# CityU-AIM-Group/SCAN

Hardware: AMD Instinct MI355X
Metric: train images/sec (whole node), VGG16 C2F 1024x2048 (higher is better)
Workload: dtype f32 (fp32 storage, fp32 multiply, fp32 accumulate -- the reference's arithmetic; the convolutions run it on the bf16 matrix cores as bf16x6: every fp32 operand cut into 3 bf16 pieces = all 24 significand bits, 6 bf16 MFMAs per product)

## Files before the change

### include/scan_hip.h

```cpp
#ifndef SCAN_HIP_H
#define SCAN_HIP_H

#include <stdint.h>

#ifdef __cplusplus
extern "C" {
#endif

#define SCAN_MAX_LEVELS 5

typedef struct {
  int32_t n_levels;
  int32_t n_images;
  int32_t h[SCAN_MAX_LEVELS];
  int32_t w[SCAN_MAX_LEVELS];
  int64_t row_off[SCAN_MAX_LEVELS + 1];
} scan_pyramid_t;

const char* scan_last_error(void);
int scan_abi_version(void);

#define SCAN_TUNE_UNKNOWN (-2147483647 - 1)
int scan_tune(const char* key, int value);
int scan_tune_get(const char* key);
int scan_tune_default(const char* key);
const char* scan_tune_key(int index);

int scan_mfma_sustained_bf16(double seconds, int32_t random, double* tflops, void* stream);

int scan_comm_standin(float* buf, int64_t n_floats, double traffic, int32_t wgs, double gbps, void* stream);

int scan_conv3x3_bf16x3_instance(const scan_pyramid_t* d, int32_t Nout);
int scan_conv1x1_bf16x6_instance(const scan_pyramid_t* yd, int32_t Nout, int32_t Csw);

int scan_sigmoid_focal_loss_forward(const float* logits, const int32_t* targets, int64_t M, int32_t C,
                                    float gamma, float alpha, float* losses, float* loss_sum, void* stream);
int scan_sigmoid_focal_loss_backward(const float* logits, const int32_t* targets, const float* d_losses,
                                     float d_scale, int64_t M, int32_t C, float gamma, float alpha,
                                     float* d_logits, void* stream);

int scan_iou_loss_forward(const float* pred, const float* target, const float* weight, int64_t P,
                          float* out2, void* stream);
int scan_iou_loss_backward(const float* pred, const float* target, const float* weight, int64_t P,
                           const float* g_num_dev, float* d_pred, void* stream);

int scan_bce_logits_forward(const float* logits, const float* targets, float const_target,
                            const float* weight, int64_t w_stride, int64_t M, float* out2, void* stream);
int scan_bce_logits_backward(const float* logits, const float* targets, float const_target,
                             const float* weight, int64_t w_stride, int64_t M, const float* g_dev,
                             float* d_logits, void* stream);

int scan_cka_bce_forward(const float* logits, const float* act, int64_t M, int32_t Cf, float target, float* out,
                         void* stream);
int scan_cka_bce_backward(const float* logits, const float* act, int64_t M, int32_t Cf, float target,
                          const float* g_dev, float* d_logits, void* stream);
int scan_cka_bce_forward_loss(const float* logits, const float* act, int64_t M, int32_t Cf, float target, float* out,
                              void* stream);
int scan_cka_bce_backward_loss(const float* logits, const float* act, int64_t M, int32_t Cf, float target,
                               const float* g_loss, const float* sums, float* d_logits, void* stream);

int scan_scale(const float* x, float alpha, float* y, int64_t n, void* stream);
int scan_copy_cols(const float* src, int32_t ld_src, float* dst, int32_t ld_dst, int64_t M, int32_t ncols, int32_t ztail,
                   void* stream);
int scan_paradigm_update(float* P, const float* pb, int32_t K, int32_t C, int32_t T, int32_t it, void* stream);

int scan_dynconv_softmax_forward(const float* feat, const float* kernels, int64_t M, int32_t C, int32_t K,
                                 float* logits, float* probs, void* stream);
int64_t scan_dynconv_ws_floats(int64_t M, int32_t C, int32_t K);
int scan_dynconv_softmax_backward(const float* feat, const float* kernels, const float* probs,
                                  const float* d_logits_in, const float* d_probs, int64_t M, int32_t C,
                                  int32_t K, float* d_feat, float* d_kernels, float* ws, void* stream);

int scan_softmax_focal_forward(const float* logits, const int64_t* labels, int64_t M, int32_t K, float gamma,
                               float* loss_sum, void* stream);
int scan_softmax_focal_backward(const float* logits, const int64_t* labels, int64_t M, int32_t K, float gamma,
                                float d_scale, float* d_logits, void* stream);

#define SCAN_NMS_PANEL 8192
#define SCAN_NMS_MAX 262144
int64_t scan_nms_ws_bytes(int64_t n);
int scan_nms(const float* dets, const float* scores, const float* labels, int64_t n, float thr, int32_t rule_ge,
             int64_t* keep_out, int32_t* num_keep_out, void* workspace, void* stream);

int scan_conv2d_forward(const float* x, const scan_pyramid_t* xd, int32_t Cin_s, const float* w, const float* bias,
                        float* y, const scan_pyramid_t* yd, int32_t Cout, int32_t Cout_s, int32_t ksize,
                        int32_t stride, int32_t relu, void* stream);
int scan_conv2d_dgrad(const float* dy, const scan_pyramid_t* yd, int32_t Cout_s, const float* wt, float* dx,
                      const scan_pyramid_t* xd, int32_t Cin, int32_t Cin_s, int32_t ksize, int32_t stride,
                      const float* mask, void* stream);
int64_t scan_conv2d_wgrad_ws_floats(const scan_pyramid_t* yd, int32_t Cin_s, int32_t Cout, int32_t ksize);
int scan_conv2d_wgrad(const float* x, const scan_pyramid_t* xd, int32_t Cin_s, const float* dy,
                      const scan_pyramid_t* yd, int32_t Cout, int32_t Cout_s, int32_t ksize, int32_t stride,
                      float* dw, int32_t accumulate, float* ws, void* stream);
int scan_weight_split(const float* w, int32_t O, int32_t T, int32_t Cs, int32_t mode, void* wh, void* wl,
                      int32_t Csw, void* stream);
int scan_conv3x3_bf16x3(const float* x, const scan_pyramid_t* d, int32_t Cs, const void* wh, const void* wl,
                        int32_t Csw, const float* bias, const float* mask, float* y, int32_t Nout, int32_t Ns,
                        int32_t relu, void* stream);
int scan_conv1x1_bf16x3(const float* x, const scan_pyramid_t* xd, int32_t Cs, const void* wh, const void* wl,
                        int32_t Csw, const float* bias, const float* mask, float* y, const scan_pyramid_t* yd,
                        int32_t Nout, int32_t Ns, int32_t relu, int32_t map, void* stream);
int64_t scan_conv1x1_wgrad_bf16x3_ws_floats(const scan_pyramid_t* yd, int32_t Cs, int32_t Cout);
int scan_conv1x1_wgrad_bf16x3(const float* x, const scan_pyramid_t* xd, int32_t Cs, const float* dy,
                              const scan_pyramid_t* yd, int32_t Cout, int32_t Cout_s, int32_t stride, float* dw,
                              float* db, int32_t accumulate, float* ws, void* stream);
int scan_conv_smallcin_bf16x3(const float* x, int32_t N, int32_t H, int32_t W, const float* w, const float* bias,
                              float* y, int32_t Cout, int32_t Cout_s, int32_t ksize, int32_t stride, int32_t relu,
                              void* stream);
int scan_conv3x3_gn_bf16x3(const float* x, const scan_pyramid_t* d, int32_t Cs, const void* wh, const void* wl,
                           int32_t Csw, const float* bias, float* y, int32_t Nout, int32_t Ns, float* gn_ws,
                           void* stream);
int scan_conv3x3_gn_acc_bf16x3(const float* x, const scan_pyramid_t* d, int32_t Cs, const void* wh, const void* wl,
                               int32_t Csw, const float* bias, float* y, int32_t Nout, int32_t Ns, float* gn_ws,
                               void* stream);
int scan_groupnorm_stats_from_sums(const float* ws, const scan_pyramid_t* d, int32_t C, int32_t G, float eps,
                                   float* stats, void* stream);
int scan_conv3x3_pool2_bf16x3(const float* x, const scan_pyramid_t* d, int32_t Cs, const void* wh, const void* wl,
                              int32_t Csw, const float* bias, float* y, int32_t Nout, int32_t Ns, int32_t relu,
                              void* stream);
int64_t scan_conv3x3_wgrad_bf16x3_ws_floats(const scan_pyramid_t* d, int32_t Cs, int32_t Cout);
int scan_conv3x3_wgrad_bf16x3(const float* x, const scan_pyramid_t* d, int32_t Cs, const float* dy, int32_t Cout,
                              int32_t Cout_s, float* dw, float* db, int32_t accumulate, float* ws, void* stream);
int scan_weight_split3(const float* w, int32_t O, int32_t T, int32_t Cs, int32_t mode, void* wh, void* wm, void* wl,
                       int32_t Csw, void* stream);
int scan_conv3x3_bf16x6(const float* x, const scan_pyramid_t* d, int32_t Cs, const void* wh, const void* wm,
                        const void* wl, int32_t Csw, const float* bias, const float* mask, float* y, int32_t Nout,
                        int32_t Ns, int32_t relu, void* stream);
int scan_conv1x1_bf16x6(const float* x, const scan_pyramid_t* xd, int32_t Cs, const void* wh, const void* wm,
                        const void* wl, int32_t Csw, const float* bias, const float* mask, float* y,
                        const scan_pyramid_t* yd, int32_t Nout, int32_t Ns, int32_t relu, int32_t map, void* stream);
int scan_conv3x3_gn_bf16x6(const float* x, const scan_pyramid_t* d, int32_t Cs, const void* wh, const void* wm,
                           const void* wl, int32_t Csw, const float* bias, float* y, int32_t Nout, int32_t Ns,
                           float* gn_ws, int32_t clear, void* stream);
int scan_conv3x3_pool2_bf16x6(const float* x, const scan_pyramid_t* d, int32_t Cs, const void* wh, const void* wm,
                              const void* wl, int32_t Csw, const float* bias, float* y, int32_t Nout, int32_t Ns,
                              int32_t relu, void* stream);
int scan_conv_smallcin_bf16x6(const float* x, int32_t N, int32_t H, int32_t W, const float* w, const float* bias,
                              float* y, int32_t Cout, int32_t Cout_s, int32_t ksize, int32_t stride, int32_t relu,
                              void* stream);
int64_t scan_conv3x3_wgrad_bf16x6_ws_floats(const scan_pyramid_t* d, int32_t Cs, int32_t Cout);
int scan_conv3x3_wgrad_bf16x6(const float* x, const scan_pyramid_t* d, int32_t Cs, const float* dy, int32_t Cout,
                              int32_t Cout_s, float* dw, float* db, int32_t accumulate, float* ws, void* stream);
int64_t scan_conv1x1_wgrad_bf16x6_ws_floats(const scan_pyramid_t* yd, int32_t Cs, int32_t Cout);
int scan_conv1x1_wgrad_bf16x6(const float* x, const scan_pyramid_t* xd, int32_t Cs, const float* dy,
                              const scan_pyramid_t* yd, int32_t Cout, int32_t Cout_s, int32_t stride, float* dw,
                              float* db, int32_t accumulate, float* ws, void* stream);
int scan_conv3x3_bf16x6_instance(const scan_pyramid_t* d, int32_t Nout);
int scan_weight_transpose(const float* w, int32_t Cout, int32_t T, int32_t Cin_s, float* wt, int32_t Cout_s,
                          void* stream);
int64_t scan_colsum_ws_floats(int64_t M, int32_t C);
int scan_colsum(const float* dy, int64_t M, int32_t C, int32_t ld, float* db, int32_t accumulate, float* ws,
                void* stream);
int scan_relu_backward(const float* dy, const float* y, float* out, int64_t n, void* stream);

int scan_groupnorm_stats(const float* x, const scan_pyramid_t* d, int32_t C, int32_t G, float eps, float* stats,
                         float* ws, void* stream);
int scan_groupnorm_relu_forward(const float* x, const scan_pyramid_t* d, int32_t C, int32_t G, const float* stats,
                                const float* gamma, const float* beta, int32_t relu, float* y, void* stream);
int scan_groupnorm_relu_forward_from_sums(const float* x, const scan_pyramid_t* d, int32_t C, int32_t G,
                                          const float* sums, float eps, const float* gamma, const float* beta,
                                          int32_t relu, float* y, float* stats, void* stream);
int64_t scan_groupnorm_ws_floats(const scan_pyramid_t* d, int32_t C, int32_t G);
int scan_groupnorm_relu_backward(const float* x, const float* beta, const float* dy, const scan_pyramid_t* d, int32_t C,
                                 int32_t G, const float* stats, const float* gamma, int32_t relu, float* dx,
                                 float* dgamma, float* dbeta, int32_t accumulate, float* ws, void* stream);
int scan_groupnorm_relu_forward_ld(const float* x, const scan_pyramid_t* d, int32_t C, int32_t G, const float* stats,
                                   const float* gamma, const float* beta, int32_t relu, float* y, int32_t ldy,
                                   void* stream);
int scan_groupnorm_relu_forward_from_sums_ld(const float* x, const scan_pyramid_t* d, int32_t C, int32_t G,
                                             const float* sums, float eps, const float* gamma, const float* beta,
                                             int32_t relu, float* y, int32_t ldy, float* stats, void* stream);
int scan_groupnorm_relu_backward_ld(const float* x, const float* beta, const float* dy, int32_t lddy,
                                    const scan_pyramid_t* d, int32_t C, int32_t G, const float* stats, const float* gamma,
                                    int32_t relu, float* dx, float* dgamma, float* dbeta, int32_t accumulate, float* ws,
                                    void* stream);

int scan_fcos_assign(const scan_pyramid_t* d, const int32_t* strides, const float* soi, const float* boxes,
                     const int64_t* glabels, const int32_t* ng, int32_t G, int64_t* labels, int32_t* labels_i32,
                     float* reg, int32_t* level_pos, void* stream);
int scan_fcos_compact(const scan_pyramid_t* d, const int64_t* labels, int32_t* pos_list, int32_t* neg_list, void* stream);
int64_t scan_fcos_nodes_count(const scan_pyramid_t* d, const int32_t* level_pos);
int scan_fcos_nodes(const scan_pyramid_t* d, const int32_t* level_pos, const int64_t* labels, const float* reg,
                    const int32_t* pos_list, const int32_t* neg_list, int64_t* node_index, int64_t* node_labels,
                    int64_t* pos_inds, float* reg_pos, float* ctr_pos, void* stream);

int scan_upsample2x_add(const float* lat, const float* coarse, int32_t N, int32_t h, int32_t w, int32_t C, float* y,
                        void* stream);
int scan_downsample2x_sum(const float* g, int32_t N, int32_t h, int32_t w, int32_t C, float* d, void* stream);

int scan_maxpool2x2_forward(const float* x, int32_t N, int32_t H, int32_t W, int32_t C, float* y, void* stream);
int scan_maxpool2x2_backward(const float* x, const float* y, const float* dy, int32_t N, int32_t H, int32_t W,
                             int32_t C, float* dx, int32_t relu_mask, void* stream);

int scan_maxpool3x3s2_forward(const float* x, int32_t N, int32_t H, int32_t W, int32_t C, float* y, void* stream);
int scan_add_relu(const float* a, const float* b, float* y, int64_t n, void* stream);

#define SCAN_DBSCAN_MAX 1200000
int64_t scan_dbscan_ws_bytes(int64_t n);
int scan_dbscan_prepare(const float* pts, int64_t n, int32_t D, float eps, int32_t min_samples, void* ws,
                        int32_t* info, void* stream);
int scan_dbscan_bfs_step(int64_t n, void* ws, int32_t parity, int32_t* changed, void* stream);
int scan_dbscan_finish(int64_t n, void* ws, uint8_t* in_cluster0, void* stream);

int scan_sgd_momentum(float* p, const float* g, float* buf, int64_t n, float lr, float wd, float momentum,
                      int32_t first_step, void* stream);

#define SCAN_SGD_MAX_SEGMENTS 32
typedef struct {
  float* p;
  const float* g;
  float* buf;
  int64_t n;
  float lr;
  float wd;
  int32_t first_step;
  int32_t reserved;
} scan_sgd_segment_t;
int scan_sgd_momentum_multi(const scan_sgd_segment_t* segs, int32_t n_segs, float momentum, void* stream);

#define SCAN_SPLIT_JOB_WORDS 11
int64_t scan_weight_split_job_blocks(int32_t O, int32_t T, int32_t Cs, int32_t mode, int32_t Csw);
int scan_weight_split_batched(const int64_t* jobs, int32_t n_jobs, int32_t job_words, int64_t total_blocks, void* stream);

#define SCAN_CKA_MAX_CLASSES 16
typedef struct {
  const float* w0;
  const float* b0;
  const float* w2;
  const float* b2;
} scan_cka_branch_t;
int scan_cka_stack_weights(const scan_cka_branch_t* branches, int32_t Cf, int32_t C, int32_t H, int64_t s1o, int64_t s1c,
                           int64_t s1k, int64_t s2c, int64_t s2k, int32_t Cs1, int32_t Cs2, float* w1, float* b1,
                           float* w2, float* b2, void* stream);
int scan_cka_unstack_grads(const scan_cka_branch_t* grads, int32_t Cf, int32_t C, int32_t H, int64_t s1o, int64_t s1c,
                           int64_t s1k, int64_t s2c, int64_t s2k, int32_t Cs1, int32_t Cs2, const float* dw1,
                           const float* db1, const float* dw2, const float* db2, int32_t accumulate, void* stream);

int64_t scan_gconv3x3_to1_ws_floats(const scan_pyramid_t* d, int32_t G, int32_t Cg);
int scan_gconv3x3_to1_forward(const float* x, const scan_pyramid_t* d, int32_t G, int32_t Cg, const float* w,
                              const float* bias, float* y, int32_t Ns, float* ws, void* stream);
int scan_gconv3x3_to1_dgrad(const float* dy, int32_t Ns, const scan_pyramid_t* d, int32_t G, int32_t Cg, const float* w,
                            const float* mask, float* dx, void* stream);
int scan_gconv3x3_to1_wgrad(const float* x, const float* dy, int32_t Ns, const scan_pyramid_t* d, int32_t G, int32_t Cg,
                            float* dw, int32_t accumulate, float* ws, void* stream);
int scan_gconv3x3_to1_backward(const float* x, const float* dy, int32_t Ns, const scan_pyramid_t* d, int32_t G, int32_t Cg,
                               const float* w, int32_t relu_mask, float* dx, float* dw, int32_t accumulate, float* ws,
                               void* stream);
int scan_gconv3x3_to1_forward_bits(const float* x, const scan_pyramid_t* d, int32_t G, int32_t Cg, const float* w,
                                   const float* bias, float* y, int32_t Ns, float* ws, uint32_t* relu_bits, void* stream);
int scan_gconv3x3_to1_backward_bits(const float* x, const float* dy, int32_t Ns, const scan_pyramid_t* d, int32_t G,
                                    int32_t Cg, const float* w, const uint32_t* relu_bits, float* dx, float* dw,
                                    int32_t accumulate, float* ws, void* stream);

int scan_resize_bilinear_u8(const uint8_t* src, int32_t H, int32_t W, uint8_t* tmp, uint8_t* dst, int32_t OH, int32_t OW,
                            const int32_t* xbounds, const int32_t* xcoef, int32_t kx, const int32_t* ybounds,
                            const int32_t* ycoef, int32_t ky, void* stream);

int scan_normalize_image_u8(const uint8_t* src, int32_t H, int32_t W, int32_t flip, int32_t to_bgr255,
                            const float* mean3, const float* std3, float* dst, int32_t Hp, int32_t Wp, int32_t layout,
                            void* stream);

int scan_take_images_backward(const float* g, const scan_pyramid_t* d, int32_t i0, int32_t i1, int32_t C, float* out,
                              void* stream);

int scan_cond_rnn_forward(const float* x, int32_t K, int32_t T, const float* const* weights, float* h0, float* h1,
                          float* kernels, void* stream);
int64_t scan_cond_rnn_ws_floats(void);
int scan_cond_rnn_backward(const float* x, int32_t K, int32_t T, const float* const* weights, const float* h0,
                           const float* h1, const float* dkernels, float* const* grads, float* ws, void* stream);

#ifdef __cplusplus
}
#endif
#endif
```

### scan_amd/_lib.py

```python
import ctypes
import os

_HERE = os.path.dirname(os.path.abspath(__file__))
LIB_PATH = os.environ.get("SCAN_HIP_LIB") or os.path.join(_HERE, "libscan_hip.so")

MAX_LEVELS = 5
TUNE_UNKNOWN = -2 ** 31
NMS_PANEL = 8192
NMS_MAX = 262144

c_i32, c_i64, c_f32, c_vp = ctypes.c_int32, ctypes.c_int64, ctypes.c_float, ctypes.c_void_p


class PyramidDesc(ctypes.Structure):
    _fields_ = [("n_levels", c_i32), ("n_images", c_i32), ("h", c_i32 * MAX_LEVELS), ("w", c_i32 * MAX_LEVELS),
                ("row_off", c_i64 * (MAX_LEVELS + 1))]


_PD = ctypes.POINTER(PyramidDesc)


class SgdSegment(ctypes.Structure):
    _fields_ = [("p", c_vp), ("g", c_vp), ("buf", c_vp), ("n", c_i64), ("lr", c_f32), ("wd", c_f32),
                ("first_step", c_i32), ("reserved", c_i32)]


class CkaBranch(ctypes.Structure):
    _fields_ = [("w0", c_vp), ("b0", c_vp), ("w2", c_vp), ("b2", c_vp)]


SGD_MAX_SEGMENTS = 32
CKA_MAX_CLASSES = 16
SPLIT_JOB_WORDS = 11

SIGNATURES = {
    "scan_last_error": (ctypes.c_char_p, []),
    "scan_abi_version": (ctypes.c_int, []),
    "scan_comm_standin": (ctypes.c_int, [ctypes.c_void_p, ctypes.c_int64, ctypes.c_double, ctypes.c_int32, ctypes.c_double,
                                         ctypes.c_void_p]),
    "scan_tune": (ctypes.c_int, [ctypes.c_char_p, ctypes.c_int]),
    "scan_take_images_backward": (ctypes.c_int, [c_vp, _PD, c_i32, c_i32, c_i32, c_vp, c_vp]),
    "scan_cond_rnn_forward": (ctypes.c_int, [c_vp, c_i32, c_i32, c_vp, c_vp, c_vp, c_vp, c_vp]),
    "scan_cond_rnn_ws_floats": (ctypes.c_int64, []),
    "scan_cond_rnn_backward": (ctypes.c_int, [c_vp, c_i32, c_i32, c_vp, c_vp, c_vp, c_vp, c_vp, c_vp, c_vp]),
    "scan_tune_get": (ctypes.c_int, [ctypes.c_char_p]),
    "scan_tune_default": (ctypes.c_int, [ctypes.c_char_p]),
    "scan_tune_key": (ctypes.c_char_p, [ctypes.c_int]),
    "scan_mfma_sustained_bf16": (ctypes.c_int, [ctypes.c_double, c_i32, ctypes.POINTER(ctypes.c_double), c_vp]),
    "scan_conv3x3_bf16x3_instance": (ctypes.c_int, [_PD, c_i32]),
    "scan_conv1x1_bf16x6_instance": (ctypes.c_int, [_PD, c_i32, c_i32]),
    "scan_conv3x3_bf16x6_instance": (ctypes.c_int, [_PD, c_i32]),
    "scan_sigmoid_focal_loss_forward": (ctypes.c_int, [c_vp, c_vp, c_i64, c_i32, c_f32, c_f32, c_vp, c_vp, c_vp]),
    "scan_sigmoid_focal_loss_backward": (ctypes.c_int, [c_vp, c_vp, c_vp, c_f32, c_i64, c_i32, c_f32, c_f32, c_vp, c_vp]),
    "scan_iou_loss_forward": (ctypes.c_int, [c_vp, c_vp, c_vp, c_i64, c_vp, c_vp]),
    "scan_iou_loss_backward": (ctypes.c_int, [c_vp, c_vp, c_vp, c_i64, c_vp, c_vp, c_vp]),
    "scan_bce_logits_forward": (ctypes.c_int, [c_vp, c_vp, c_f32, c_vp, c_i64, c_i64, c_vp, c_vp]),
    "scan_bce_logits_backward": (ctypes.c_int, [c_vp, c_vp, c_f32, c_vp, c_i64, c_i64, c_vp, c_vp, c_vp]),
    "scan_cka_bce_forward": (ctypes.c_int, [c_vp, c_vp, c_i64, c_i32, c_f32, c_vp, c_vp]),
    "scan_cka_bce_backward": (ctypes.c_int, [c_vp, c_vp, c_i64, c_i32, c_f32, c_vp, c_vp, c_vp]),
    "scan_cka_bce_forward_loss": (ctypes.c_int, [c_vp, c_vp, c_i64, c_i32, c_f32, c_vp, c_vp]),
    "scan_cka_bce_backward_loss": (ctypes.c_int, [c_vp, c_vp, c_i64, c_i32, c_f32, c_vp, c_vp, c_vp, c_vp]),
    "scan_scale": (ctypes.c_int, [c_vp, c_f32, c_vp, c_i64, c_vp]),
    "scan_copy_cols": (ctypes.c_int, [c_vp, c_i32, c_vp, c_i32, c_i64, c_i32, c_i32, c_vp]),
    "scan_paradigm_update": (ctypes.c_int, [c_vp, c_vp, c_i32, c_i32, c_i32, c_i32, c_vp]),
    "scan_dynconv_softmax_forward": (ctypes.c_int, [c_vp, c_vp, c_i64, c_i32, c_i32, c_vp, c_vp, c_vp]),
    "scan_dynconv_ws_floats": (c_i64, [c_i64, c_i32, c_i32]),
    "scan_dynconv_softmax_backward": (ctypes.c_int, [c_vp, c_vp, c_vp, c_vp, c_vp, c_i64, c_i32, c_i32, c_vp, c_vp, c_vp, c_vp]),
    "scan_softmax_focal_forward": (ctypes.c_int, [c_vp, c_vp, c_i64, c_i32, c_f32, c_vp, c_vp]),
    "scan_softmax_focal_backward": (ctypes.c_int, [c_vp, c_vp, c_i64, c_i32, c_f32, c_f32, c_vp, c_vp]),
    "scan_nms_ws_bytes": (c_i64, [c_i64]),
    "scan_nms": (ctypes.c_int, [c_vp, c_vp, c_vp, c_i64, c_f32, c_i32, c_vp, c_vp, c_vp, c_vp]),
    "scan_conv2d_forward": (ctypes.c_int, [c_vp, _PD, c_i32, c_vp, c_vp, c_vp, _PD, c_i32, c_i32, c_i32, c_i32, c_i32, c_vp]),
    "scan_conv2d_dgrad": (ctypes.c_int, [c_vp, _PD, c_i32, c_vp, c_vp, _PD, c_i32, c_i32, c_i32, c_i32, c_vp, c_vp]),
    "scan_conv2d_wgrad_ws_floats": (c_i64, [_PD, c_i32, c_i32, c_i32]),
    "scan_conv2d_wgrad": (ctypes.c_int, [c_vp, _PD, c_i32, c_vp, _PD, c_i32, c_i32, c_i32, c_i32, c_vp, c_i32, c_vp, c_vp]),
    "scan_weight_split": (ctypes.c_int, [c_vp, c_i32, c_i32, c_i32, c_i32, c_vp, c_vp, c_i32, c_vp]),
    "scan_conv3x3_bf16x3": (ctypes.c_int, [c_vp, _PD, c_i32, c_vp, c_vp, c_i32, c_vp, c_vp, c_vp, c_i32, c_i32, c_i32, c_vp]),
    "scan_conv3x3_wgrad_bf16x3_ws_floats": (c_i64, [_PD, c_i32, c_i32]),
    "scan_dbscan_ws_bytes": (c_i64, [c_i64]),
    "scan_conv1x1_wgrad_bf16x3_ws_floats": (c_i64, [_PD, c_i32, c_i32]),
    "scan_conv3x3_wgrad_bf16x3": (ctypes.c_int, [c_vp, _PD, c_i32, c_vp, c_i32, c_i32, c_vp, c_vp, c_i32, c_vp, c_vp]),
    "scan_weight_transpose": (ctypes.c_int, [c_vp, c_i32, c_i32, c_i32, c_vp, c_i32, c_vp]),
    "scan_colsum_ws_floats": (c_i64, [c_i64, c_i32]),
    "scan_colsum": (ctypes.c_int, [c_vp, c_i64, c_i32, c_i32, c_vp, c_i32, c_vp, c_vp]),
    "scan_relu_backward": (ctypes.c_int, [c_vp, c_vp, c_vp, c_i64, c_vp]),
    "scan_groupnorm_stats": (ctypes.c_int, [c_vp, _PD, c_i32, c_i32, c_f32, c_vp, c_vp, c_vp]),
    "scan_groupnorm_relu_forward": (ctypes.c_int, [c_vp, _PD, c_i32, c_i32, c_vp, c_vp, c_vp, c_i32, c_vp, c_vp]),
    "scan_groupnorm_relu_forward_from_sums": (ctypes.c_int, [c_vp, _PD, c_i32, c_i32, c_vp, c_f32, c_vp, c_vp, c_i32, c_vp, c_vp, c_vp]),
    "scan_groupnorm_ws_floats": (c_i64, [_PD, c_i32, c_i32]),
    "scan_fcos_assign": (ctypes.c_int, [_PD, c_vp, c_vp, c_vp, c_vp, c_vp, c_i32, c_vp, c_vp, c_vp, c_vp, c_vp]),
    "scan_fcos_compact": (ctypes.c_int, [_PD, c_vp, c_vp, c_vp, c_vp]),
    "scan_fcos_nodes_count": (c_i64, [_PD, c_vp]),
    "scan_fcos_nodes": (ctypes.c_int, [_PD, c_vp, c_vp, c_vp, c_vp, c_vp, c_vp, c_vp, c_vp, c_vp, c_vp, c_vp]),
    "scan_groupnorm_relu_forward_ld": (ctypes.c_int, [c_vp, _PD, c_i32, c_i32, c_vp, c_vp, c_vp, c_i32, c_vp, c_i32, c_vp]),
    "scan_groupnorm_relu_forward_from_sums_ld": (ctypes.c_int, [c_vp, _PD, c_i32, c_i32, c_vp, c_f32, c_vp, c_vp, c_i32, c_vp,
                                                                c_i32, c_vp, c_vp]),
    "scan_groupnorm_relu_backward_ld": (ctypes.c_int, [c_vp, c_vp, c_vp, c_i32, _PD, c_i32, c_i32, c_vp, c_vp, c_i32, c_vp,
                                                       c_vp, c_vp, c_i32, c_vp, c_vp]),
    "scan_groupnorm_relu_backward": (ctypes.c_int, [c_vp, c_vp, c_vp, _PD, c_i32, c_i32, c_vp, c_vp, c_i32, c_vp, c_vp, c_vp, c_i32, c_vp, c_vp]),
    "scan_maxpool2x2_forward": (ctypes.c_int, [c_vp, c_i32, c_i32, c_i32, c_i32, c_vp, c_vp]),
    "scan_maxpool2x2_backward": (ctypes.c_int, [c_vp, c_vp, c_vp, c_i32, c_i32, c_i32, c_i32, c_vp, c_i32, c_vp]),
    "scan_conv3x3_gn_bf16x3": (ctypes.c_int, [c_vp, _PD, c_i32, c_vp, c_vp, c_i32, c_vp, c_vp, c_i32, c_i32, c_vp, c_vp]),
    "scan_conv3x3_gn_acc_bf16x3": (ctypes.c_int, [c_vp, _PD, c_i32, c_vp, c_vp, c_i32, c_vp, c_vp, c_i32, c_i32, c_vp, c_vp]),
    "scan_groupnorm_stats_from_sums": (ctypes.c_int, [c_vp, _PD, c_i32, c_i32, c_f32, c_vp, c_vp]),
    "scan_conv3x3_pool2_bf16x3": (ctypes.c_int, [c_vp, _PD, c_i32, c_vp, c_vp, c_i32, c_vp, c_vp, c_i32, c_i32, c_i32, c_vp]),
    "scan_conv1x1_bf16x3": (ctypes.c_int, [c_vp, _PD, c_i32, c_vp, c_vp, c_i32, c_vp, c_vp, c_vp, _PD, c_i32, c_i32, c_i32,
                                           c_i32, c_vp]),
    "scan_conv1x1_wgrad_bf16x3": (ctypes.c_int, [c_vp, _PD, c_i32, c_vp, _PD, c_i32, c_i32, c_i32, c_vp, c_vp, c_i32, c_vp,
                                                 c_vp]),
    "scan_conv_smallcin_bf16x3": (ctypes.c_int, [c_vp, c_i32, c_i32, c_i32, c_vp, c_vp, c_vp, c_i32, c_i32, c_i32, c_i32,
                                                 c_i32, c_vp]),
    "scan_weight_split3": (ctypes.c_int, [c_vp, c_i32, c_i32, c_i32, c_i32, c_vp, c_vp, c_vp, c_i32, c_vp]),
    "scan_conv3x3_bf16x6": (ctypes.c_int, [c_vp, _PD, c_i32, c_vp, c_vp, c_vp, c_i32, c_vp, c_vp, c_vp, c_i32, c_i32, c_i32, c_vp]),
    "scan_conv1x1_bf16x6": (ctypes.c_int, [c_vp, _PD, c_i32, c_vp, c_vp, c_vp, c_i32, c_vp, c_vp, c_vp, _PD, c_i32, c_i32, c_i32,
                                           c_i32, c_vp]),
    "scan_conv3x3_gn_bf16x6": (ctypes.c_int, [c_vp, _PD, c_i32, c_vp, c_vp, c_vp, c_i32, c_vp, c_vp, c_i32, c_i32, c_vp, c_i32,
                                              c_vp]),
    "scan_conv3x3_pool2_bf16x6": (ctypes.c_int, [c_vp, _PD, c_i32, c_vp, c_vp, c_vp, c_i32, c_vp, c_vp, c_i32, c_i32, c_i32,
                                                 c_vp]),
    "scan_conv3x3_wgrad_bf16x6_ws_floats": (c_i64, [_PD, c_i32, c_i32]),
    "scan_conv3x3_wgrad_bf16x6": (ctypes.c_int, [c_vp, _PD, c_i32, c_vp, c_i32, c_i32, c_vp, c_vp, c_i32, c_vp, c_vp]),
    "scan_conv1x1_wgrad_bf16x6_ws_floats": (c_i64, [_PD, c_i32, c_i32]),
    "scan_conv1x1_wgrad_bf16x6": (ctypes.c_int, [c_vp, _PD, c_i32, c_vp, _PD, c_i32, c_i32, c_i32, c_vp, c_vp, c_i32, c_vp,
                                                 c_vp]),
    "scan_conv_smallcin_bf16x6": (ctypes.c_int, [c_vp, c_i32, c_i32, c_i32, c_vp, c_vp, c_vp, c_i32, c_i32, c_i32, c_i32,
                                                 c_i32, c_vp]),
    "scan_maxpool3x3s2_forward": (ctypes.c_int, [c_vp, c_i32, c_i32, c_i32, c_i32, c_vp, c_vp]),
    "scan_upsample2x_add": (ctypes.c_int, [c_vp, c_vp, c_i32, c_i32, c_i32, c_i32, c_vp, c_vp]),
    "scan_downsample2x_sum": (ctypes.c_int, [c_vp, c_i32, c_i32, c_i32, c_i32, c_vp, c_vp]),
    "scan_add_relu": (ctypes.c_int, [c_vp, c_vp, c_vp, c_i64, c_vp]),
    "scan_dbscan_prepare": (ctypes.c_int, [c_vp, c_i64, c_i32, c_f32, c_i32, c_vp, c_vp, c_vp]),
    "scan_dbscan_bfs_step": (ctypes.c_int, [c_i64, c_vp, c_i32, c_vp, c_vp]),
    "scan_dbscan_finish": (ctypes.c_int, [c_i64, c_vp, c_vp, c_vp]),
    "scan_sgd_momentum": (ctypes.c_int, [c_vp, c_vp, c_vp, c_i64, c_f32, c_f32, c_f32, c_i32, c_vp]),
    "scan_sgd_momentum_multi": (ctypes.c_int, [ctypes.POINTER(SgdSegment), c_i32, c_f32, c_vp]),
    "scan_weight_split_job_blocks": (c_i64, [c_i32, c_i32, c_i32, c_i32, c_i32]),
    "scan_weight_split_batched": (ctypes.c_int, [c_vp, c_i32, c_i32, c_i64, c_vp]),
    "scan_cka_stack_weights": (ctypes.c_int, [ctypes.POINTER(CkaBranch), c_i32, c_i32, c_i32, c_i64, c_i64, c_i64, c_i64,
                                              c_i64, c_i32, c_i32, c_vp, c_vp, c_vp, c_vp, c_vp]),
    "scan_cka_unstack_grads": (ctypes.c_int, [ctypes.POINTER(CkaBranch), c_i32, c_i32, c_i32, c_i64, c_i64, c_i64, c_i64,
                                              c_i64, c_i32, c_i32, c_vp, c_vp, c_vp, c_vp, c_i32, c_vp]),
    "scan_gconv3x3_to1_ws_floats": (c_i64, [_PD, c_i32, c_i32]),
    "scan_gconv3x3_to1_forward": (ctypes.c_int, [c_vp, _PD, c_i32, c_i32, c_vp, c_vp, c_vp, c_i32, c_vp, c_vp]),
    "scan_gconv3x3_to1_dgrad": (ctypes.c_int, [c_vp, c_i32, _PD, c_i32, c_i32, c_vp, c_vp, c_vp, c_vp]),
    "scan_gconv3x3_to1_wgrad": (ctypes.c_int, [c_vp, c_vp, c_i32, _PD, c_i32, c_i32, c_vp, c_i32, c_vp, c_vp]),
    "scan_gconv3x3_to1_backward": (ctypes.c_int, [c_vp, c_vp, c_i32, _PD, c_i32, c_i32, c_vp, c_i32, c_vp, c_vp, c_i32, c_vp,
                                                  c_vp]),
    "scan_gconv3x3_to1_forward_bits": (ctypes.c_int, [c_vp, _PD, c_i32, c_i32, c_vp, c_vp, c_vp, c_i32, c_vp, c_vp, c_vp]),
    "scan_gconv3x3_to1_backward_bits": (ctypes.c_int, [c_vp, c_vp, c_i32, _PD, c_i32, c_i32, c_vp, c_vp, c_vp, c_vp, c_i32,
                                                       c_vp, c_vp]),
    "scan_resize_bilinear_u8": (ctypes.c_int, [c_vp, c_i32, c_i32, c_vp, c_vp, c_i32, c_i32, c_vp, c_vp, c_i32, c_vp, c_vp,
                                               c_i32, c_vp]),
    "scan_normalize_image_u8": (ctypes.c_int, [c_vp, c_i32, c_i32, c_i32, c_i32, ctypes.POINTER(c_f32),
                                               ctypes.POINTER(c_f32), c_vp, c_i32, c_i32, c_i32, c_vp]),
}

_lib = None


def lib():
    global _lib
    if _lib is None:
        if not os.path.exists(LIB_PATH):
            raise RuntimeError(
                "scan_amd: %s is missing -- build it with `python -c 'import __graft_entry__ as g; g.build()'` "
                "(hipcc --offload-arch=gfx950); there is no CPU fallback." % LIB_PATH)
        import torch
        L = ctypes.CDLL(LIB_PATH)
        for name, (res, args) in SIGNATURES.items():
            fn = getattr(L, name)
            fn.restype = res
            fn.argtypes = args
        for kv in filter(None, os.environ.get("SCAN_TUNE", "").split(",")):
            key, _, val = kv.partition("=")
            if L.scan_tune(key.strip().encode(), int(val)) == TUNE_UNKNOWN:
                raise RuntimeError("SCAN_TUNE: unknown key %r" % key)
        _lib = L
    return _lib


def tune_state():
    L, out, i = lib(), {}, 0
    while True:
        k = L.scan_tune_key(i)
        if k is None:
            return out
        out[k.decode()] = (L.scan_tune_get(k), L.scan_tune_default(k))
        i += 1


def lib_identity():
    import hashlib
    with open(LIB_PATH, "rb") as f:
        sha = hashlib.sha1(f.read()).hexdigest()
    product = os.path.realpath(LIB_PATH) == os.path.realpath(os.path.join(_HERE, "libscan_hip.so"))
    return {"lib": os.path.basename(LIB_PATH), "lib_sha1": sha, "product_library": product,
            "scan_tune_non_default": {k: v for k, (v, d) in tune_state().items() if v != d}}


def call(name, *args):
    rc = getattr(lib(), name)(*args)
    if rc != 0:
        raise RuntimeError("%s failed (%d): %s" % (name, rc, lib().scan_last_error().decode()))

# ... 4 lines not shown
```

### scan_amd/csrc/batched.hip

```cpp
#include "conv_split.h"

#define SPLIT_ELEMS_PER_BLOCK 2048
#define SPLIT_TILE 64

__device__ __forceinline__ void split8_store(const float (&v)[8], __bf16* __restrict__ w0, __bf16* __restrict__ w1,
                                             __bf16* __restrict__ w2, int64_t i) {
  bf16x8 q0, q1, q2;
#pragma unroll
  for (int k = 0; k < 8; ++k) {
    __bf16 q[3];
    split1_np<3>(v[k], q);
    q0[k] = q[0];
    q1[k] = q[1];
    q2[k] = q[2];
  }
  *reinterpret_cast<bf16x8*>(w0 + i) = q0;
  *reinterpret_cast<bf16x8*>(w1 + i) = q1;
  if (w2 != nullptr) *reinterpret_cast<bf16x8*>(w2 + i) = q2;
}

__global__ __launch_bounds__(256) void weight_split_batched_kernel(const int64_t* __restrict__ jobs, int n_jobs) {
  __shared__ float tile[SPLIT_TILE][SPLIT_TILE + 1];
  int j = 0;
  for (int i = 1; i < n_jobs; ++i)
    if ((int64_t)blockIdx.x >= jobs[(int64_t)i * SCAN_SPLIT_JOB_WORDS + 9]) j = i;
  const int64_t* job = jobs + (int64_t)j * SCAN_SPLIT_JOB_WORDS;
  const float* __restrict__ w = reinterpret_cast<const float*>(job[0]);
  __bf16* __restrict__ wh = reinterpret_cast<__bf16*>(job[1]);
  __bf16* __restrict__ wl = reinterpret_cast<__bf16*>(job[2]);
  __bf16* __restrict__ w2 = reinterpret_cast<__bf16*>(job[10]);
  const int O = (int)job[3], T = (int)job[4], Cs = (int)job[5], mode = (int)job[6], rows = (int)job[7],
            Csw = (int)job[8];
  const int64_t blk = (int64_t)blockIdx.x - job[9];
  const int tid = threadIdx.x;
  if (mode == 0) {
    const int64_t total = (int64_t)rows * T * Csw;
    const int64_t i = blk * SPLIT_ELEMS_PER_BLOCK + (int64_t)tid * 8;
    if (i >= total) return;
    const int col = (int)(i % Csw);
    const int64_t rt = i / Csw;
    const float* src = w + rt * Cs + col;
    float v[8];
    if (col + 8 <= Cs && (Cs & 3) == 0) {
      const float4 a = *reinterpret_cast<const float4*>(src);
      const float4 b = *reinterpret_cast<const float4*>(src + 4);
      v[0] = a.x; v[1] = a.y; v[2] = a.z; v[3] = a.w;
      v[4] = b.x; v[5] = b.y; v[6] = b.z; v[7] = b.w;
    } else {
#pragma unroll
      for (int k = 0; k < 8; ++k) v[k] = (col + k < Cs) ? src[k] : 0.f;
    }
    split8_store(v, wh, wl, w2, i);
    return;
  }
  const int tiles_o = (Csw + SPLIT_TILE - 1) / SPLIT_TILE, tiles_c = (rows + SPLIT_TILE - 1) / SPLIT_TILE;
  const int to = (int)(blk % tiles_o);
  const int tc = (int)((blk / tiles_o) % tiles_c);
  const int tt = (int)(blk / ((int64_t)tiles_o * tiles_c));
  const int o0 = to * SPLIT_TILE, c0 = tc * SPLIT_TILE;
  {
    const int cl = (tid & 15) * 4, ol = tid >> 4;
#pragma unroll
    for (int p = 0; p < SPLIT_TILE / 16; ++p) {
      const int o = o0 + ol + 16 * p, c = c0 + cl;
      float4 a = make_float4(0.f, 0.f, 0.f, 0.f);
      if (o < O && c < Cs) {
        const float* src = w + ((int64_t)o * T + (T - 1 - tt)) * Cs + c;
        if (c + 4 <= Cs && (Cs & 3) == 0) {
          a = *reinterpret_cast<const float4*>(src);
        } else {
          a.x = src[0];
          if (c + 1 < Cs) a.y = src[1];
          if (c + 2 < Cs) a.z = src[2];
          if (c + 3 < Cs) a.w = src[3];
        }
      }
      float* t = &tile[ol + 16 * p][cl];
      t[0] = a.x; t[1] = a.y; t[2] = a.z; t[3] = a.w;
    }
  }
  __syncthreads();
  {
    const int o8 = (tid & 7) * 8, cl = tid >> 3;
#pragma unroll
    for (int p = 0; p < SPLIT_TILE / 32; ++p) {
      const int c = c0 + cl + 32 * p, o = o0 + o8;
      if (c < rows && o < Csw) {
        float v[8];
#pragma unroll
        for (int k = 0; k < 8; ++k) v[k] = tile[o8 + k][cl + 32 * p];
        split8_store(v, wh, wl, w2, ((int64_t)c * T + tt) * Csw + o);
      }
    }
  }
}

extern "C" int64_t scan_weight_split_job_blocks(int32_t O, int32_t T, int32_t Cs, int32_t mode, int32_t Csw) {
  if (mode == 0) return ((int64_t)O * T * Csw + SPLIT_ELEMS_PER_BLOCK - 1) / SPLIT_ELEMS_PER_BLOCK;
  const int64_t tiles_o = (Csw + SPLIT_TILE - 1) / SPLIT_TILE, tiles_c = (Cs + SPLIT_TILE - 1) / SPLIT_TILE;
  return tiles_o * tiles_c * T;
}

extern "C" int scan_weight_split_batched(const int64_t* jobs, int32_t n_jobs, int32_t job_words, int64_t total_blocks,
                                         void* stream) {
  SCAN_CHECK_ARG(job_words == SCAN_SPLIT_JOB_WORDS, "weight_split_batched: records of %d words, this library reads %d",
                 job_words, SCAN_SPLIT_JOB_WORDS);
  SCAN_CHECK_ARG(jobs && n_jobs > 0 && total_blocks > 0 && total_blocks < (1ll << 31),
                 "weight_split_batched: bad arguments (n_jobs=%d)", n_jobs);
  hipLaunchKernelGGL(weight_split_batched_kernel, dim3((unsigned)total_blocks), dim3(256), 0, as_stream(stream), jobs,
                     n_jobs);
  SCAN_LAUNCH_CHECK("weight_split_batched");
  return 0;
}

struct SgdSegs {
  scan_sgd_segment_t s[SCAN_SGD_MAX_SEGMENTS];
  int64_t first_block[SCAN_SGD_MAX_SEGMENTS + 1];
  int n;
};
#define SGD_ELEMS_PER_BLOCK 4096

__global__ __launch_bounds__(256) void sgd_multi_kernel(SgdSegs t, float momentum) {
  int j = 0;
#pragma unroll
  for (int i = 1; i < SCAN_SGD_MAX_SEGMENTS; ++i)
    if (i < t.n && (int64_t)blockIdx.x >= t.first_block[i]) j = i;
  const scan_sgd_segment_t sg = t.s[j];
  const int64_t base = ((int64_t)blockIdx.x - t.first_block[j]) * SGD_ELEMS_PER_BLOCK;
  float* __restrict__ p = sg.p;
  const float* __restrict__ g = sg.g;
  float* __restrict__ buf = sg.buf;
#pragma unroll 4
  for (int k = 0; k < SGD_ELEMS_PER_BLOCK / 256; ++k) {
    const int64_t i = base + k * 256 + threadIdx.x;
    if (i >= sg.n) break;
    const float w = p[i];
    const float gg = g[i] + sg.wd * w;
    const float b = sg.first_step ? gg : momentum * buf[i] + gg;
    buf[i] = b;
    p[i] = w - sg.lr * b;
  }
}

extern "C" int scan_sgd_momentum_multi(const scan_sgd_segment_t* segs, int32_t n_segs, float momentum, void* stream) {
  SCAN_CHECK_ARG(segs && n_segs > 0 && n_segs <= SCAN_SGD_MAX_SEGMENTS, "sgd_momentum_multi: n_segs=%d out of 1..%d", n_segs,
                 SCAN_SGD_MAX_SEGMENTS);
  SgdSegs t;
  t.n = 0;
  int64_t blocks = 0;
  for (int i = 0; i < n_segs; ++i) {
    SCAN_CHECK_ARG(segs[i].n >= 0, "sgd_momentum_multi: segment %d has n < 0", i);
    if (segs[i].n == 0) continue;
    SCAN_CHECK_ARG(segs[i].p && segs[i].g && segs[i].buf, "sgd_momentum_multi: null pointer in segment %d", i);
    t.s[t.n] = segs[i];
    t.first_block[t.n] = blocks;
    blocks += (segs[i].n + SGD_ELEMS_PER_BLOCK - 1) / SGD_ELEMS_PER_BLOCK;
    ++t.n;
  }
  if (t.n == 0) return 0;
  t.first_block[t.n] = blocks;
  SCAN_CHECK_ARG(blocks < (1ll << 31), "sgd_momentum_multi: too many elements");
  hipLaunchKernelGGL(sgd_multi_kernel, dim3((unsigned)blocks), dim3(256), 0, as_stream(stream), t, momentum);
  SCAN_LAUNCH_CHECK("sgd_momentum_multi");
  return 0;
}

struct CkaPtrs {
  scan_cka_branch_t b[SCAN_CKA_MAX_CLASSES];
};

__global__ __launch_bounds__(256) void cka_stack_kernel(CkaPtrs P, int Cf, int C, int H, int64_t s1o, int64_t s1c,
                                                        int64_t s1k, int64_t s2c, int64_t s2k, int Cs1, int Cs2,
                                                        float* __restrict__ w1, float* __restrict__ b1,
                                                        float* __restrict__ w2, float* __restrict__ b2) {
  const int64_t n1 = (int64_t)Cf * H * 9 * Cs1;
  const int64_t n2 = (int64_t)Cf * 9 * Cs2;
  const int64_t nb = (int64_t)Cf * H + Cf;
  for (int64_t i = (int64_t)blockIdx.x * blockDim.x + threadIdx.x; i < n1 + n2 + nb;
       i += (int64_t)gridDim.x * blockDim.x) {
    if (i < n1) {
      const int col = (int)(i % Cs1);
      const int64_t r = i / Cs1;
      const int k = (int)(r % 9);
      const int row = (int)(r / 9);
      const int c = row / H, o = row - c * H;
      float v = 0.f;
      if (col < C) v = P.b[c].w0[o * s1o + col * s1c + k * s1k];
      else if (col == C + c) v = P.b[c].w0[o * s1o + C * s1c + k * s1k];
      w1[i] = v;
    } else if (i < n1 + n2) {
      const int64_t q = i - n1;
      const int col = (int)(q % Cs2);
      const int64_t r = q / Cs2;
      const int k = (int)(r % 9);
      const int c = (int)(r / 9);
      float v = 0.f;
      if (col >= c * H && col < (c + 1) * H) v = P.b[c].w2[(col - c * H) * s2c + k * s2k];
      w2[q] = v;
    } else {
      const int q = (int)(i - n1 - n2);
      if (q < Cf * H) b1[q] = P.b[q / H].b0[q % H];
      else b2[q - Cf * H] = P.b[q - Cf * H].b2[0];
    }
  }
}

__global__ __launch_bounds__(256) void cka_unstack_kernel(CkaPtrs G, int Cf, int C, int H, int64_t s1o, int64_t s1c,
                                                          int64_t s1k, int64_t s2c, int64_t s2k, int Cs1, int Cs2,
                                                          const float* __restrict__ dw1, const float* __restrict__ db1,
                                                          const float* __restrict__ dw2, const float* __restrict__ db2,
                                                          int accumulate) {
  const int64_t n1 = (int64_t)Cf * H * 9 * (C + 1);
  const int64_t n2 = (int64_t)Cf * 9 * H;
  const int64_t nb = (int64_t)Cf * H + Cf;
  for (int64_t i = (int64_t)blockIdx.x * blockDim.x + threadIdx.x; i < n1 + n2 + nb;
       i += (int64_t)gridDim.x * blockDim.x) {
    if (i < n1) {
      const int col = (int)(i % (C + 1));
      const int64_t r = i / (C + 1);
      const int k = (int)(r % 9);
      const int row = (int)(r / 9);
      const int c = row / H, o = row - c * H;
      if (dw1 != nullptr) {
        const float v = dw1[((int64_t)row * 9 + k) * Cs1 + (col < C ? col : C + c)];
        float* dst = const_cast<float*>(G.b[c].w0) + o * s1o + col * s1c + k * s1k;
        *dst = accumulate ? *dst + v : v;
      }
    } else if (i < n1 + n2) {
      const int64_t q = i - n1;
      const int h = (int)(q % H);
      const int64_t r = q / H;
      const int k = (int)(r % 9);
      const int c = (int)(r / 9);
      if (dw2 != nullptr) {
        const float v = dw2[((int64_t)c * 9 + k) * Cs2 + c * H + h];
        float* dst = const_cast<float*>(G.b[c].w2) + h * s2c + k * s2k;
        *dst = accumulate ? *dst + v : v;
      }
    } else {
      const int q = (int)(i - n1 - n2);
      if (q < Cf * H) {
        if (db1 != nullptr) {
          float* dst = const_cast<float*>(G.b[q / H].b0) + q % H;
          *dst = accumulate ? *dst + db1[q] : db1[q];
        }
      } else if (db2 != nullptr) {
        float* dst = const_cast<float*>(G.b[q - Cf * H].b2);
        *dst = accumulate ? *dst + db2[q - Cf * H] : db2[q - Cf * H];
      }
    }
  }
}

// ... 36 lines not shown
```

### scan_amd/csrc/capi.cpp

```cpp
#include <stdarg.h>
#include <stdio.h>
#include <string.h>

#include "../../include/scan_hip.h"

static thread_local char g_err[512] = "";

extern "C" void scan_set_error(const char* fmt, ...) {
  va_list ap;
  va_start(ap, fmt);
  vsnprintf(g_err, sizeof(g_err), fmt, ap);
  va_end(ap);
}

extern "C" const char* scan_last_error(void) { return g_err; }
extern "C" int scan_abi_version(void) { return 1; }

extern int g_scan_conv_bn256;
extern int g_scan_conv_v2;
extern int g_scan_conv_wg1024;
extern int g_scan_conv_w8;
extern int g_scan_conv_tpb3;
extern int g_scan_conv_bn64_th16;
extern int g_scan_conv_glds;
extern int g_scan_conv1x1;
extern int g_scan_wgrad_v6;
extern int g_scan_wgrad_prio;
extern int g_scan_wgrad_tile;
extern int g_scan_wgrad_wgs;
extern int g_scan_gconv_mfma;
extern int g_scan_dbscan_bf16x3;
extern int g_scan_reduce_blocks;

struct Knob {
  const char* key;
  int* slot;
  int dflt;
};
static Knob* knob_table(int* count) {
  static Knob knobs[] = {
      {"conv_bn256", &g_scan_conv_bn256, 0},   {"conv_v2", &g_scan_conv_v2, 0},         {"conv_wg1024", &g_scan_conv_wg1024, 0},
      {"conv_w8", &g_scan_conv_w8, 0},         {"conv_tpb3", &g_scan_conv_tpb3, 0},     {"conv_bn64_th16", &g_scan_conv_bn64_th16, 0},
      {"conv_glds", &g_scan_conv_glds, 0},     {"wgrad_v6", &g_scan_wgrad_v6, 0},       {"wgrad_prio", &g_scan_wgrad_prio, 0},
      {"wgrad_tile", &g_scan_wgrad_tile, 0},   {"wgrad_wgs", &g_scan_wgrad_wgs, 0},     {"gconv_mfma", &g_scan_gconv_mfma, 0},
      {"dbscan_bf16x3", &g_scan_dbscan_bf16x3, 0}, {"reduce_blocks", &g_scan_reduce_blocks, 0}, {"conv1x1", &g_scan_conv1x1, 0},
  };
  static bool init = false;
  if (!init) {
    for (auto& k : knobs) k.dflt = *k.slot;
    init = true;
  }
  *count = (int)(sizeof(knobs) / sizeof(knobs[0]));
  return knobs;
}
static Knob* find_knob(const char* key) {
  int n = 0;
  Knob* t = knob_table(&n);
  if (key == nullptr) return nullptr;
  for (int i = 0; i < n; ++i)
    if (strcmp(key, t[i].key) == 0) return &t[i];
  return nullptr;
}

extern "C" int scan_tune(const char* key, int value) {
  Knob* k = find_knob(key);
  if (k == nullptr) return SCAN_TUNE_UNKNOWN;
  const int old = *k->slot;
  *k->slot = value;
  return old;
}

extern "C" int scan_tune_get(const char* key) {
  const Knob* k = find_knob(key);
  return k == nullptr ? SCAN_TUNE_UNKNOWN : *k->slot;
}

extern "C" int scan_tune_default(const char* key) {
  const Knob* k = find_knob(key);
  return k == nullptr ? SCAN_TUNE_UNKNOWN : k->dflt;
}

extern "C" const char* scan_tune_key(int index) {
  int n = 0;
  const Knob* t = knob_table(&n);
  return (index >= 0 && index < n) ? t[index].key : nullptr;
}
```

### scan_amd/csrc/conv_bf16x3.hip

```cpp
#include "conv_split.h"

typedef float f32x16 __attribute__((ext_vector_type(16)));

#define SCAN_MMA(a, b, c) __builtin_amdgcn_mfma_f32_32x32x16_bf16(a, b, c, 0, 0, 0)

#define TW 16
#define PW (TW + 2)
#define CK 32
#define LROW 40
#define PPITCH 768

struct TileTab {
  int tile_off[SCAN_MAX_LEVELS + 1];
  int tiles_x[SCAN_MAX_LEVELS];
  int tiles_y[SCAN_MAX_LEVELS];
};

__device__ __forceinline__ int xcd_remap3(int orig, int nwg) {
  const int q = nwg / 8, r = nwg % 8, xcd = orig % 8;
  const int base = (xcd < r) ? xcd * (q + 1) : r * (q + 1) + (xcd - r) * q;
  return base + orig / 8;
}

__device__ __forceinline__ void split4(const float4 v, bf16x4& hi, bf16x4& lo) {
// ... 121 lines not shown
#pragma unroll
  for (int tm = 0; tm < TM; ++tm) {
    const int p = (wm * TM + tm) * 32 + lr;
    a_off[tm] = (p >> 4) * PPITCH + (p & 15) * LROW + 8 * lh;
  }
  const int b_off = (wn * 32 * TN + lr) * LROW + 8 * lh;

  f32x16 acc[TM][TN];
#pragma unroll
  for (int a = 0; a < TM; ++a)
#pragma unroll
    for (int b = 0; b < TN; ++b)
#pragma unroll
      for (int r = 0; r < 16; ++r) acc[a][b][r] = 0.f;

  load_a(0);
  load_b(0, 0);
  for (int cc = 0; cc < nchunks; ++cc) {
    __syncthreads();
    store_a();
    if (cc + 1 < nchunks) load_a(cc + 1);
#pragma unroll 1
    for (int tap = 0; tap < NTAPS; ++tap) {
      const int buf = (cc * NTAPS + tap) & 1;
      store_b(buf);
      if (tap < NTAPS - 1)
        load_b(cc, tap + 1);
      else if (cc + 1 < nchunks)
        load_b(cc + 1, 0);
      __syncthreads();
      const int ky = tap / KS, kx = tap - KS * ky;
      const int shift = ky * PPITCH + kx * LROW;
      const __bf16* bh = Bs + (buf * 2 + 0) * BN * LROW + b_off;
      const __bf16* bl = Bs + (buf * 2 + 1) * BN * LROW + b_off;
      if constexpr (TN > 2) {
#pragma unroll
        for (int s = 0; s < 2; ++s) {
          bf16x8 ah[TM], al[TM];
#pragma unroll
          for (int tm = 0; tm < TM; ++tm) {
            ah[tm] = *reinterpret_cast<const bf16x8*>(Ah + a_off[tm] + shift + 16 * s);
            al[tm] = *reinterpret_cast<const bf16x8*>(Al + a_off[tm] + shift + 16 * s);
          }
#pragma unroll
          for (int tn = 0; tn < TN; ++tn) {
            const bf16x8 bhv = *reinterpret_cast<const bf16x8*>(bh + tn * 32 * LROW + 16 * s);
            const bf16x8 blv = *reinterpret_cast<const bf16x8*>(bl + tn * 32 * LROW + 16 * s);
#pragma unroll
            for (int tm = 0; tm < TM; ++tm) {
              acc[tm][tn] = SCAN_MMA(al[tm], bhv, acc[tm][tn]);
              acc[tm][tn] = SCAN_MMA(ah[tm], blv, acc[tm][tn]);
              acc[tm][tn] = SCAN_MMA(ah[tm], bhv, acc[tm][tn]);
            }
          }
        }
        continue;
      }
#pragma unroll
      for (int s = 0; s < 2; ++s) {
        bf16x8 ah[TM], al[TM], bhv[TN], blv[TN];
#pragma unroll
        for (int tm = 0; tm < TM; ++tm) {
          ah[tm] = *reinterpret_cast<const bf16x8*>(Ah + a_off[tm] + shift + 16 * s);
          al[tm] = *reinterpret_cast<const bf16x8*>(Al + a_off[tm] + shift + 16 * s);
        }
#pragma unroll
        for (int tn = 0; tn < TN; ++tn) {
          bhv[tn] = *reinterpret_cast<const bf16x8*>(bh + tn * 32 * LROW + 16 * s);
          blv[tn] = *reinterpret_cast<const bf16x8*>(bl + tn * 32 * LROW + 16 * s);
        }
#pragma unroll
        for (int tm = 0; tm < TM; ++tm)
#pragma unroll
          for (int tn = 0; tn < TN; ++tn) {
            acc[tm][tn] = SCAN_MMA(al[tm], bhv[tn], acc[tm][tn]);
            acc[tm][tn] = SCAN_MMA(ah[tm], blv[tn], acc[tm][tn]);
            acc[tm][tn] = SCAN_MMA(ah[tm], bhv[tn], acc[tm][tn]);
          }
      }
    }
  }

#pragma unroll
  for (int tn = 0; tn < TN; ++tn) {
    const int o = n0 + wn * 32 * TN + tn * 32 + lr;
    const float bv = (bias != nullptr && o < Nout) ? bias[o] : 0.f;
    float gs = 0.f, gq = 0.f;
    if (relu & 2) {
      const int Hp = H >> 1, Wp = W >> 1;
#pragma unroll
      for (int tm = 0; tm < TM; ++tm)
#pragma unroll
        for (int q = 0; q < 4; ++q) {
          const int r = 2 * q;
          const int p = (wm * TM + tm) * 32 + (r & 3) + 8 * (r >> 2) + 4 * lh;
          const int y = ty0 + (p >> 4), x = tx0 + (p & 15);
          if (y < H && x < W && o < Nout) {
            float v = fmaxf(fmaxf(acc[tm][tn][r], acc[tm][tn][r + 1]), fmaxf(acc[tm][tn][r + 8], acc[tm][tn][r + 9])) + bv;
            if (relu & 1) v = fmaxf(v, 0.f);
            dst[((int64_t)img * Hp * Wp + (int64_t)(y >> 1) * Wp + (x >> 1)) * Ns + o] = v;
          }
        }
      continue;
    }
#pragma unroll
    for (int tm = 0; tm < TM; ++tm) {
      float mk[16];
      if (mask != nullptr) {
#pragma unroll
        for (int r = 0; r < 16; ++r) {
          const int p = (wm * TM + tm) * 32 + (r & 3) + 8 * (r >> 2) + 4 * lh;
          const int y = ty0 + (p >> 4), x = tx0 + (p & 15);
          const bool ok = y < H && x < W && o < Nout;
          mk[r] = ok ? mask[(rowbase + (int64_t)y * W + x) * Ns + o] : 0.f;
        }
      }
#pragma unroll
      for (int r = 0; r < 16; ++r) {
        const int p = (wm * TM + tm) * 32 + (r & 3) + 8 * (r >> 2) + 4 * lh;
        const int y = ty0 + (p >> 4), x = tx0 + (p & 15);
        if (y < H && x < W && o < Nout) {
          const int64_t m = rowbase + (int64_t)y * W + x;
          float v = acc[tm][tn][r] + bv;
          if (relu & 1) v = fmaxf(v, 0.f);
          if (mask != nullptr) v = (mk[r] > 0.f) ? v : 0.f;
          dst[m * Ns + o] = v;
          gs += v;
          gq += v * v;
        }
      }
    }
    if (gn_ws != nullptr) {
      double ds = (double)gs, dq = (double)gq;
#pragma unroll
      for (int sh = 1; sh <= 4; sh <<= 1) {
        ds += __shfl_xor(ds, sh, 64);
        dq += __shfl_xor(dq, sh, 64);
      }
      ds += __shfl_xor(ds, 32, 64);
      dq += __shfl_xor(dq, 32, 64);
      if ((lr & 7) == 0 && lh == 0 && o < Nout) {
        const int64_t slot = ((int64_t)(lvl * d.n_images + img) * 32 + (o >> 3)) * 2;
        atomicAdd(&gn_ws[slot], ds);
        atomicAdd(&gn_ws[slot + 1], dq);
      }
    }
  }
}


template <int NP>
__global__ void weight_split_kernel(const float* __restrict__ w, int O, int T, int Cs, int mode, int rows, int Csw,
                                    __bf16* __restrict__ w0, __bf16* __restrict__ w1, __bf16* __restrict__ w2) {
  const int64_t total = (int64_t)rows * T * Csw;
  for (int64_t i = (int64_t)blockIdx.x * blockDim.x + threadIdx.x; i < total; i += (int64_t)gridDim.x * blockDim.x) {
    const int col = (int)(i % Csw);
    const int64_t rt = i / Csw;
    const int tt = (int)(rt % T);
    const int row = (int)(rt / T);
    float v = 0.f;
    if (mode == 0) {
      if (col < Cs) v = w[((int64_t)row * T + tt) * Cs + col];
    } else {
      if (col < O) v = w[((int64_t)col * T + (T - 1 - tt)) * Cs + row];
    }
    __bf16 q[NP];
    split1_np<NP>(v, q);
    w0[i] = q[0];
    w1[i] = q[1];
    if constexpr (NP == 3) w2[i] = q[2];
  }
}

int g_scan_conv_v2 = 1;
extern int g_scan_conv_bn256;
int conv3x3_split_launch(int np, const float* x, const scan_pyramid_t* d, int32_t Cs, const void* w0, const void* w1,
                         const void* w2, int32_t Csw, const float* bias, const float* mask, float* y, int32_t Nout,
                         int32_t Ns, int32_t relu, void* stream, double* gn_ws);
int conv1x1_split_launch(int np, const float* x, const scan_pyramid_t* xd, int32_t Cs, const void* w0, const void* w1,
                         const void* w2, int32_t Csw, const float* bias, const float* mask, float* y,
                         const scan_pyramid_t* yd, int32_t Nout, int32_t Ns, int32_t relu, int32_t map, void* stream);
static inline bool v2_ok(const void* y, const void* mask, int32_t Ns) {
  return (Ns & 3) == 0 && (reinterpret_cast<uintptr_t>(y) & 15) == 0 && (reinterpret_cast<uintptr_t>(mask) & 15) == 0;
}

static void make_tiles(const scan_pyramid_t* d, TileTab* tt, int TH) {
  tt->tile_off[0] = 0;
  for (int l = 0; l < SCAN_MAX_LEVELS; ++l) {
    if (l < d->n_levels) {
      tt->tiles_x[l] = (d->w[l] + TW - 1) / TW;
      tt->tiles_y[l] = (d->h[l] + TH - 1) / TH;
      tt->tile_off[l + 1] = tt->tile_off[l] + d->n_images * tt->tiles_x[l] * tt->tiles_y[l];
    } else {
      tt->tiles_x[l] = tt->tiles_y[l] = 1;
      tt->tile_off[l + 1] = tt->tile_off[l];
    }
  }
}

static int weight_split_launch(int np, const float* w, int32_t O, int32_t T, int32_t Cs, int32_t mode, void* w0, void* w1,
                               void* w2, int32_t Csw, void* stream) {
  SCAN_CHECK_ARG(w && w0 && w1 && (np == 2 || w2) && O > 0 && T > 0 && Cs > 0, "weight_split: bad arguments");
  SCAN_CHECK_ARG(mode == 0 || mode == 1, "weight_split: mode must be 0 or 1");
  SCAN_CHECK_ARG(Csw % 8 == 0 && Csw >= (mode == 0 ? Cs : O), "weight_split: Csw=%d must be a multiple of 8 and cover the row",
                 Csw);
  const int rows = mode == 0 ? O : Cs;
  const int64_t total = (int64_t)rows * T * Csw;
  __bf16 *p0 = reinterpret_cast<__bf16*>(w0), *p1 = reinterpret_cast<__bf16*>(w1), *p2 = reinterpret_cast<__bf16*>(w2);
  if (np == 3)
    hipLaunchKernelGGL(weight_split_kernel<3>, dim3(grid_for(total, 256)), dim3(256), 0, as_stream(stream), w, O, T, Cs, mode,
                       rows, Csw, p0, p1, p2);
  else
    hipLaunchKernelGGL(weight_split_kernel<2>, dim3(grid_for(total, 256)), dim3(256), 0, as_stream(stream), w, O, T, Cs, mode,
                       rows, Csw, p0, p1, p2);
  SCAN_LAUNCH_CHECK("weight_split");
  return 0;
}

extern "C" int scan_weight_split(const float* w, int32_t O, int32_t T, int32_t Cs, int32_t mode, void* wh, void* wl,
                                 int32_t Csw, void* stream) {
  return weight_split_launch(2, w, O, T, Cs, mode, wh, wl, nullptr, Csw, stream);
}
extern "C" int scan_weight_split3(const float* w, int32_t O, int32_t T, int32_t Cs, int32_t mode, void* wh, void* wm,
                                  void* wl, int32_t Csw, void* stream) {
  return weight_split_launch(3, w, O, T, Cs, mode, wh, wm, wl, Csw, stream);
}

static int conv3x3_launch(int np, const float* x, const scan_pyramid_t* d, int32_t Cs, const void* w0, const void* w1,
                          const void* w2, int32_t Csw, const float* bias, const float* mask, float* y, int32_t Nout,
                          int32_t Ns, int32_t relu, void* stream, double* gn_ws = nullptr) {
  const char* name = np == 2 ? "conv3x3_bf16x3" : "conv3x3_bf16x6";
  SCAN_CHECK_ARG(d && d->n_levels >= 1 && d->n_levels <= SCAN_MAX_LEVELS && d->n_images >= 1, "%s: bad pyramid", name);
  SCAN_CHECK_ARG(Cs > 0 && Cs % 4 == 0, "%s: Cs=%d must be a positive multiple of 4", name, Cs);
  SCAN_CHECK_ARG(Csw % 8 == 0 && Csw >= Cs, "%s: Csw=%d must be a multiple of 8 and >= Cs", name, Csw);
  SCAN_CHECK_ARG(Nout > 0 && Ns >= Nout, "%s: Nout=%d Ns=%d", name, Nout, Ns);
  SCAN_CHECK_ARG(x && w0 && w1 && (np == 2 || w2) && y, "%s: null pointer", name);
  if (np == 3) {
    SCAN_CHECK_ARG(v2_ok(y, mask, Ns), "%s: y / mask must be 16-byte aligned and Ns a multiple of 4", name);
    return conv3x3_split_launch(3, x, d, Cs, w0, w1, w2, Csw, bias, mask, y, Nout, Ns, relu, stream, gn_ws);
  }
  if (g_scan_conv_v2 && v2_ok(y, mask, Ns))
    return conv3x3_split_launch(2, x, d, Cs, w0, w1, nullptr, Csw, bias, mask, y, Nout, Ns, relu, stream, gn_ws);
  TileTab tt;
  hipStream_t st = as_stream(stream);
  const __bf16* h = reinterpret_cast<const __bf16*>(w0);
  const __bf16* l = reinterpret_cast<const __bf16*>(w1);
  if (Nout > 64) {
    make_tiles(d, &tt, 16);
    const int tiles = tt.tile_off[d->n_levels];
    const bool wide = g_scan_conv_bn256 && Nout % 256 == 0 && (int64_t)tiles * (Nout / 256) >= 512;
    if (wide) {
      const int n_tiles = Nout / 256;
      const size_t sh = (size_t)(2 * 18 * PPITCH + 4 * 256 * LROW) * sizeof(__bf16);
      static bool done = false;
      if (!done) {
        hipFuncSetAttribute(reinterpret_cast<const void*>(conv3x3_bf16x3_kernel<256, 16, 512>),
                            hipFuncAttributeMaxDynamicSharedMemorySize, (int)sh);
        done = true;
      }
      hipLaunchKernelGGL((conv3x3_bf16x3_kernel<256, 16, 512>), dim3(tiles * n_tiles), dim3(512), sh, st, x, *d, Cs, h, l,
                         Csw, bias, mask, y, Nout, Ns, relu, tt, n_tiles, *d, 0, gn_ws);
      SCAN_LAUNCH_CHECK("conv3x3_bf16x3");
      return 0;
    }
    const int n_tiles = (Nout + 127) / 128;
    const size_t sh = (size_t)(2 * 18 * PPITCH + 4 * 128 * LROW) * sizeof(__bf16);
    static bool done = false;
    if (!done) {
      hipFuncSetAttribute(reinterpret_cast<const void*>(conv3x3_bf16x3_kernel<128, 16, 512>),
                          hipFuncAttributeMaxDynamicSharedMemorySize, (int)sh);
      done = true;
    }
    hipLaunchKernelGGL((conv3x3_bf16x3_kernel<128, 16, 512>), dim3(tiles * n_tiles), dim3(512), sh, st, x, *d, Cs, h, l,
                       Csw, bias, mask, y, Nout, Ns, relu, tt, n_tiles, *d, 0, gn_ws);
  } else {
    make_tiles(d, &tt, 8);
    const int tiles = tt.tile_off[d->n_levels];
    const size_t sh = (size_t)(2 * 10 * PPITCH + 4 * 64 * LROW) * sizeof(__bf16);
    hipLaunchKernelGGL((conv3x3_bf16x3_kernel<64, 8, 256>), dim3(tiles), dim3(256), sh, st, x, *d, Cs, h, l, Csw, bias,
                       mask, y, Nout, Ns, relu, tt, 1, *d, 0, gn_ws);
  }
  SCAN_LAUNCH_CHECK("conv3x3_bf16x3");
  return 0;
}

extern "C" int scan_conv3x3_bf16x3(const float* x, const scan_pyramid_t* d, int32_t Cs, const void* wh, const void* wl,
                                   int32_t Csw, const float* bias, const float* mask, float* y, int32_t Nout,
                                   int32_t Ns, int32_t relu, void* stream) {
  return conv3x3_launch(2, x, d, Cs, wh, wl, nullptr, Csw, bias, mask, y, Nout, Ns, relu ? 1 : 0, stream);
}
extern "C" int scan_conv3x3_bf16x6(const float* x, const scan_pyramid_t* d, int32_t Cs, const void* wh, const void* wm,
                                   const void* wl, int32_t Csw, const float* bias, const float* mask, float* y,
                                   int32_t Nout, int32_t Ns, int32_t relu, void* stream) {
  return conv3x3_launch(3, x, d, Cs, wh, wm, wl, Csw, bias, mask, y, Nout, Ns, relu ? 1 : 0, stream);
}

static int conv3x3_gn_launch(int np, int clear, const float* x, const scan_pyramid_t* d, int32_t Cs, const void* w0,
                             const void* w1, const void* w2, int32_t Csw, const float* bias, float* y, int32_t Nout,
                             int32_t Ns, float* gn_ws, void* stream) {
  SCAN_CHECK_ARG(Nout == 256 && gn_ws, "conv3x3_gn: needs Nout == 256 (GroupNorm(32, 256)) and a workspace");
  SCAN_CHECK_ARG(d && d->n_levels >= 1 && d->n_levels <= SCAN_MAX_LEVELS && d->n_images >= 1, "conv3x3_gn: bad pyramid");
  if (clear) {
    const size_t bytes = sizeof(double) * 2 * 32 * (size_t)d->n_levels * d->n_images;
    if (hipMemsetAsync(gn_ws, 0, bytes, as_stream(stream)) != hipSuccess) {
      scan_set_error("conv3x3_gn: memset failed");
      return -2;
    }
  }
  return conv3x3_launch(np, x, d, Cs, w0, w1, w2, Csw, bias, nullptr, y, Nout, Ns, 0, stream, reinterpret_cast<double*>(gn_ws));
}
extern "C" int scan_conv3x3_gn_bf16x3(const float* x, const scan_pyramid_t* d, int32_t Cs, const void* wh, const void* wl,
                                      int32_t Csw, const float* bias, float* y, int32_t Nout, int32_t Ns, float* gn_ws,
                                      void* stream) {
  return conv3x3_gn_launch(2, 1, x, d, Cs, wh, wl, nullptr, Csw, bias, y, Nout, Ns, gn_ws, stream);
}
extern "C" int scan_conv3x3_gn_acc_bf16x3(const float* x, const scan_pyramid_t* d, int32_t Cs, const void* wh, const void* wl,
                                          int32_t Csw, const float* bias, float* y, int32_t Nout, int32_t Ns, float* gn_ws,
                                          void* stream) {
  return conv3x3_gn_launch(2, 0, x, d, Cs, wh, wl, nullptr, Csw, bias, y, Nout, Ns, gn_ws, stream);
}
extern "C" int scan_conv3x3_gn_bf16x6(const float* x, const scan_pyramid_t* d, int32_t Cs, const void* wh, const void* wm,
                                      const void* wl, int32_t Csw, const float* bias, float* y, int32_t Nout, int32_t Ns,
                                      float* gn_ws, int32_t clear, void* stream) {
  return conv3x3_gn_launch(3, clear, x, d, Cs, wh, wm, wl, Csw, bias, y, Nout, Ns, gn_ws, stream);
}

extern "C" int scan_conv3x3_pool2_bf16x3(const float* x, const scan_pyramid_t* d, int32_t Cs, const void* wh,
                                         const void* wl, int32_t Csw, const float* bias, float* y, int32_t Nout,
                                         int32_t Ns, int32_t relu, void* stream) {
  SCAN_CHECK_ARG(d && d->n_levels == 1 && (d->h[0] & 1) == 0 && (d->w[0] & 1) == 0,
                 "conv3x3_pool2_bf16x3: needs a single-level pyramid with even H and W");
  return conv3x3_launch(2, x, d, Cs, wh, wl, nullptr, Csw, bias, nullptr, y, Nout, Ns, (relu ? 1 : 0) | 2, stream);
}
extern "C" int scan_conv3x3_pool2_bf16x6(const float* x, const scan_pyramid_t* d, int32_t Cs, const void* wh,
                                         const void* wm, const void* wl, int32_t Csw, const float* bias, float* y,
                                         int32_t Nout, int32_t Ns, int32_t relu, void* stream) {
  SCAN_CHECK_ARG(d && d->n_levels == 1 && (d->h[0] & 1) == 0 && (d->w[0] & 1) == 0,
                 "conv3x3_pool2_bf16x6: needs a single-level pyramid with even H and W");
  return conv3x3_launch(3, x, d, Cs, wh, wm, wl, Csw, bias, nullptr, y, Nout, Ns, (relu ? 1 : 0) | 2, stream);
}

static int conv1x1_launch(int np, const float* x, const scan_pyramid_t* xd, int32_t Cs, const void* w0, const void* w1,
                          const void* w2, int32_t Csw, const float* bias, const float* mask, float* y,
                          const scan_pyramid_t* yd, int32_t Nout, int32_t Ns, int32_t relu, int32_t map, void* stream) {
  const char* name = np == 2 ? "conv1x1_bf16x3" : "conv1x1_bf16x6";
  SCAN_CHECK_ARG(xd && yd && yd->n_levels >= 1 && yd->n_levels <= SCAN_MAX_LEVELS && yd->n_images >= 1 &&
                     xd->n_levels == yd->n_levels && xd->n_images == yd->n_images,
                 "%s: bad pyramids", name);
  SCAN_CHECK_ARG(map >= 0 && map <= 2, "%s: map=%d must be 0, 1 or 2", name, map);
  SCAN_CHECK_ARG(Cs > 0 && Cs % 4 == 0, "%s: Cs=%d must be a positive multiple of 4", name, Cs);
  SCAN_CHECK_ARG(Csw % 8 == 0 && Csw >= Cs, "%s: Csw=%d must be a multiple of 8 and >= Cs", name, Csw);
  SCAN_CHECK_ARG(Nout > 0 && Ns >= Nout, "%s: Nout=%d Ns=%d", name, Nout, Ns);
  SCAN_CHECK_ARG(x && w0 && w1 && (np == 2 || w2) && y, "%s: null pointer", name);
  for (int l = 0; l < yd->n_levels; ++l) {
    const int eh = map == 0 ? xd->h[l] : map == 1 ? (xd->h[l] - 1) / 2 + 1 : yd->h[l];
    const int ew = map == 0 ? xd->w[l] : map == 1 ? (xd->w[l] - 1) / 2 + 1 : yd->w[l];
    SCAN_CHECK_ARG(eh == yd->h[l] && ew == yd->w[l] &&
                       (map != 2 || ((yd->h[l] - 1) / 2 + 1 == xd->h[l] && (yd->w[l] - 1) / 2 + 1 == xd->w[l])),
                   "%s: level %d sizes do not match map %d", name, l, map);
  }
  if (np == 3) {
    SCAN_CHECK_ARG(v2_ok(y, mask, Ns), "%s: y / mask must be 16-byte aligned and Ns a multiple of 4", name);
    return conv1x1_split_launch(3, x, xd, Cs, w0, w1, w2, Csw, bias, mask, y, yd, Nout, Ns, relu, map, stream);
  }
  if (g_scan_conv_v2 && v2_ok(y, mask, Ns))
    return conv1x1_split_launch(2, x, xd, Cs, w0, w1, nullptr, Csw, bias, mask, y, yd, Nout, Ns, relu, map, stream);
  TileTab tt;
  hipStream_t st = as_stream(stream);
  const __bf16* h = reinterpret_cast<const __bf16*>(w0);
  const __bf16* l = reinterpret_cast<const __bf16*>(w1);
  if (Nout > 64) {
    make_tiles(yd, &tt, 16);
    const int tiles = tt.tile_off[yd->n_levels];
    const int n_tiles = (Nout + 127) / 128;
    const size_t sh = (size_t)(2 * 16 * PPITCH + 4 * 128 * LROW) * sizeof(__bf16);
    static bool done = false;
    if (!done) {
      hipFuncSetAttribute(reinterpret_cast<const void*>(conv3x3_bf16x3_kernel<128, 16, 512, 1>),
                          hipFuncAttributeMaxDynamicSharedMemorySize, (int)sh);
      done = true;
    }
    hipLaunchKernelGGL((conv3x3_bf16x3_kernel<128, 16, 512, 1>), dim3(tiles * n_tiles), dim3(512), sh, st, x, *yd, Cs, h,
                       l, Csw, bias, mask, y, Nout, Ns, relu, tt, n_tiles, *xd, map, nullptr);
  } else {
    make_tiles(yd, &tt, 8);
    const int tiles = tt.tile_off[yd->n_levels];
    const size_t sh = (size_t)(2 * 8 * PPITCH + 4 * 64 * LROW) * sizeof(__bf16);
    hipLaunchKernelGGL((conv3x3_bf16x3_kernel<64, 8, 256, 1>), dim3(tiles), dim3(256), sh, st, x, *yd, Cs, h, l, Csw,
                       bias, mask, y, Nout, Ns, relu, tt, 1, *xd, map, nullptr);
  }
  SCAN_LAUNCH_CHECK("conv1x1_bf16x3");
  return 0;
}

extern "C" int scan_conv1x1_bf16x3(const float* x, const scan_pyramid_t* xd, int32_t Cs, const void* wh, const void* wl,
                                   int32_t Csw, const float* bias, const float* mask, float* y,
                                   const scan_pyramid_t* yd, int32_t Nout, int32_t Ns, int32_t relu, int32_t map,
                                   void* stream) {
  return conv1x1_launch(2, x, xd, Cs, wh, wl, nullptr, Csw, bias, mask, y, yd, Nout, Ns, relu, map, stream);
}
extern "C" int scan_conv1x1_bf16x6(const float* x, const scan_pyramid_t* xd, int32_t Cs, const void* wh, const void* wm,
                                   const void* wl, int32_t Csw, const float* bias, const float* mask, float* y,
                                   const scan_pyramid_t* yd, int32_t Nout, int32_t Ns, int32_t relu, int32_t map,
                                   void* stream) {
  return conv1x1_launch(3, x, xd, Cs, wh, wm, wl, Csw, bias, mask, y, yd, Nout, Ns, relu, map, stream);
}
```

### scan_amd/csrc/conv_fwd.hip

```cpp
#include "conv_split.h"

#define V2_TW 16
#ifndef SCAN_CONV_MID
#define SCAN_CONV_MID 0
#endif
#ifndef SCAN_CONV_PFA
#define SCAN_CONV_PFA 1
#endif
#define V2_CK 32

struct TileTab2 {
  int tile_off[SCAN_MAX_LEVELS + 1];
  int tiles_x[SCAN_MAX_LEVELS];
  int tiles_y[SCAN_MAX_LEVELS];
};

__device__ __forceinline__ int swz(int idx) { return (idx >> 1) & 2; }

template <int K>
__device__ __forceinline__ const __bf16* pick_plane(const __bf16* w0, const __bf16* w1, const __bf16* w2) {
  if constexpr (K == 0)
    return w0;
  else if constexpr (K == 1)
    return w1;
  else
    return w2;
}
template <int I, int NT, int PL, int NPL>
__device__ __forceinline__ const __bf16* slot_plane(int tid, const __bf16* w0, const __bf16* w1, const __bf16* w2) {
  constexpr int lo = (NT * I) / PL, hi = (NT * I + NT - 1) / PL;
  constexpr int lo_c = lo < NPL ? lo : NPL - 1, hi_c = hi < NPL ? hi : NPL - 1;
  static_assert(hi - lo <= 1, "a thread's slot spans at most two planes");
  if constexpr (lo_c == hi_c)
    return pick_plane<lo_c>(w0, w1, w2);
  else
    return (tid + NT * I) / PL == lo ? pick_plane<lo_c>(w0, w1, w2) : pick_plane<hi_c>(w0, w1, w2);
}
template <int NT, int PL, int NPL>
__device__ __forceinline__ const __bf16* slot_plane_i(int i, int tid, const __bf16* w0, const __bf16* w1, const __bf16* w2) {
  return i == 0   ? slot_plane<0, NT, PL, NPL>(tid, w0, w1, w2)
         : i == 1 ? slot_plane<1, NT, PL, NPL>(tid, w0, w1, w2)
         : i == 2 ? slot_plane<2, NT, PL, NPL>(tid, w0, w1, w2)
         : i == 3 ? slot_plane<3, NT, PL, NPL>(tid, w0, w1, w2)
         : i == 4 ? slot_plane<4, NT, PL, NPL>(tid, w0, w1, w2)
                  : slot_plane<5, NT, PL, NPL>(tid, w0, w1, w2);
}

template <int NP, int TM>
__device__ __forceinline__ void mma_pieces(const bf16x8 (&w)[NP], const bf16x8 (&p)[NP][TM], f32x4v (&acc)[TM]) {
#pragma unroll
  for (int s = NP - 1; s >= 0; --s)
#pragma unroll
    for (int i = 0; i <= s; ++i)
#pragma unroll
      for (int tm = 0; tm < TM; ++tm) acc[tm] = __builtin_amdgcn_mfma_f32_16x16x32_bf16(w[i], p[s - i][tm], acc[tm], 0, 0, 0);
}

template <int NP, int BN, int TH, int NT, int KS, int TPB = 1, bool GL = false>
__global__ __launch_bounds__(NT, NT == 1024 ? 4 : 2) void conv_split_kernel(
    const float* __restrict__ src, scan_pyramid_t d, int Cs, const __bf16* __restrict__ w0, const __bf16* __restrict__ w1,
    const __bf16* __restrict__ w2, int Csw, const float* __restrict__ bias, const float* __restrict__ mask,
    float* __restrict__ dst, int Nout, int Ns, int relu, TileTab2 tt, int n_tiles, scan_pyramid_t sd, int map,
    double* __restrict__ gn_ws) {
  constexpr int HALO = KS / 2, NTAPS = KS * KS;
  constexpr int PH = TH + 2 * HALO;
  constexpr int PWK = V2_TW + 2 * HALO;
  constexpr int NPATCH = PH * PWK;
  constexpr int WAVES = NT / 64;
  constexpr int WN_WAVES = BN >= 128 ? 2 : 1;
  constexpr int WM_WAVES = WAVES / WN_WAVES;
  constexpr int TM = TH / WM_WAVES;
  constexpr int TN = BN / (16 * WN_WAVES);
  constexpr int ASLOTS = (NPATCH * 8 + NT - 1) / NT;
  constexpr int BSLOTS = BN * 4 * NP;
  constexpr int BSEG = (BSLOTS + NT - 1) / NT;
  constexpr int NGRP = NTAPS / TPB;
  static_assert(NP == 2 || NP == 3, "two or three pieces per operand");
  static_assert(TM * WM_WAVES == TH && (TM % 2) == 0, "tile rows must split evenly (and pair up for the fused pool)");
  static_assert(NTAPS % TPB == 0, "taps per barrier must divide the tap count");
  static_assert(BSLOTS % 64 == 0, "a wave's 64 weight segments lie in one plane (and past the end only as a whole wave)");

  extern __shared__ __align__(16) unsigned char smem_raw[];
  __bf16* As = reinterpret_cast<__bf16*>(smem_raw);
  __bf16* Bs = As + NP * NPATCH * 32;

  const int tid = threadIdx.x, lane = tid & 63, wid = tid >> 6;
  const int bid = xcd_remap(blockIdx.x, gridDim.x);
  const int n_tile = bid % n_tiles;
  const int tile = bid / n_tiles;
  int lvl = 0;
#pragma unroll
  for (int i = 1; i < SCAN_MAX_LEVELS; ++i)
    if (i < d.n_levels && tile >= tt.tile_off[i]) lvl = i;
  const int H = d.h[lvl], W = d.w[lvl];
  int t = tile - tt.tile_off[lvl];
  const int per_img = tt.tiles_x[lvl] * tt.tiles_y[lvl];
  const int img = t / per_img;
  t -= img * per_img;
  const int ty0 = (t / tt.tiles_x[lvl]) * TH, tx0 = (t % tt.tiles_x[lvl]) * V2_TW;
  const int64_t rowbase = d.row_off[lvl] + (int64_t)img * H * W;
  const int n0 = n_tile * BN;
  const int nchunks = (Cs + V2_CK - 1) / V2_CK;

  constexpr unsigned BAD = 0x80000000u;
  unsigned voff[ASLOTS];
  const int c_tail = Cs - (nchunks - 1) * V2_CK;
  const bool tail_bad = 4 * (tid & 7) >= c_tail;
  __amdgpu_buffer_rsrc_t a_src;
  {
    const bool mapped = KS == 1 && map != 0;
    const int Hs = mapped ? sd.h[lvl] : H, Ws = mapped ? sd.w[lvl] : W;
    int64_t base_row;
    if (!mapped)
      base_row = rowbase + (int64_t)(ty0 - HALO) * W + (tx0 - HALO);
    else if (map == 1)
      base_row = sd.row_off[lvl] + ((int64_t)img * Hs + 2 * ty0) * Ws + 2 * tx0;
    else
      base_row = sd.row_off[lvl] + ((int64_t)img * Hs + (ty0 >> 1)) * Ws + (tx0 >> 1);
    a_src = uniform_rsrc_b(src + base_row * Cs, 0x7ffffff0);
#pragma unroll
    for (int i = 0; i < ASLOTS; ++i) {
      const int slot = tid + NT * i;
      const int q = slot >> 3, c4 = slot & 7;
      const int py = q / PWK, px = q - py * PWK;
      const int y = ty0 - HALO + py, x = tx0 - HALO + px;
      bool ok = (slot < NPATCH * 8) && y >= 0 && y < H && x >= 0 && x < W;
      int pix = py * W + px;
      if (mapped) {
        if (map == 1) {
          ok = ok && 2 * y < Hs && 2 * x < Ws;
          pix = 2 * py * Ws + 2 * px;
        } else {
          ok = ok && ((y | x) & 1) == 0 && (y >> 1) < Hs && (x >> 1) < Ws;
          pix = (py >> 1) * Ws + (px >> 1);
        }
      }
      voff[i] = ok ? (unsigned)((pix * Cs + 4 * c4) * 4) : BAD;
    }
  }
  float4 ra[ASLOTS];
  auto load_a = [&](int cc) {
    const int soff = cc * (V2_CK * 4);
    const bool kill = tail_bad && cc == nchunks - 1;
#pragma unroll
    for (int i = 0; i < ASLOTS; ++i)
      ra[i] = __builtin_bit_cast(float4, __builtin_amdgcn_raw_buffer_load_b128(a_src, (int)(kill ? BAD : voff[i]), soff, 0));
  };
  auto store_a = [&]() {
#pragma unroll
    for (int i = 0; i < ASLOTS; ++i) {
      const int slot = tid + NT * i;
      if (slot < NPATCH * 8) {
        const int q = slot >> 3, c4 = slot & 7;
        const int px = q % PWK;
        bf16x4 pc[NP];
        split4_np<NP>(ra[i], pc);
        const int off = q * 32 + (((c4 >> 1) ^ swz(px)) << 3) + ((c4 & 1) << 2);
#pragma unroll
        for (int p = 0; p < NP; ++p) *reinterpret_cast<bf16x4*>(As + p * NPATCH * 32 + off) = pc[p];
      }
    }
  };
  uint4 rb[TPB][BSEG];
  auto load_b = [&](int cc, int grp) {
#pragma unroll
    for (int tt = 0; tt < TPB; ++tt) {
      const int tap = grp * TPB + tt;
#pragma unroll
      for (int i = 0; i < BSEG; ++i) {
        const int slot = tid + NT * i;
        const int plane = slot / (BN * 4);
        const int rem = slot - plane * BN * 4;
        const int row = rem >> 2, seg = rem & 3;
        const int o = n0 + row, c = cc * V2_CK + 8 * seg;
        const __bf16* base = slot_plane_i<NT, BN * 4, NP>(i, tid, w0, w1, w2);
        rb[tt][i] = (slot < BSLOTS && o < Nout && c < Csw)
                        ? *reinterpret_cast<const uint4*>(base + ((int64_t)o * NTAPS + tap) * Csw + c)
                        : make_uint4(0u, 0u, 0u, 0u);
      }
    }
  };
  auto store_b = [&](int buf) {
#pragma unroll
    for (int tt = 0; tt < TPB; ++tt) {
#pragma unroll
      for (int i = 0; i < BSEG; ++i) {
        const int slot = tid + NT * i;
        const int plane = slot / (BN * 4);
        const int rem = slot - plane * BN * 4;
        const int row = rem >> 2, seg = rem & 3;
        if (slot < BSLOTS)
          *reinterpret_cast<uint4*>(Bs + (((buf * TPB + tt) * NP + plane) * BN + row) * 32 + ((seg ^ swz(row)) << 3)) = rb[tt][i];
      }
    }
  };

  static_assert(!GL || BSEG <= 6, "the LDS-DMA path keeps at most six descriptors");
  unsigned boff[BSEG];
#pragma unroll
  for (int i = 0; i < BSEG; ++i) {
    const int slot = tid + NT * i;
    const int plane = slot / (BN * 4);
    const int rem = slot - plane * BN * 4;
    const int row = rem >> 2, seg = (rem & 3) ^ swz(row);
    boff[i] = (unsigned)((((n0 + row) * NTAPS) * Csw + 8 * seg) * 2);
  }
  const int plane_bytes = Nout * NTAPS * Csw * 2;
  auto plane_rsrc = [&](int i) { return uniform_rsrc_b(slot_plane_i<NT, BN * 4, NP>(i, tid, w0, w1, w2), plane_bytes); };
  const __amdgpu_buffer_rsrc_t b_src0 = plane_rsrc(0), b_src1 = plane_rsrc(1), b_src2 = plane_rsrc(2),
                               b_src3 = plane_rsrc(3), b_src4 = plane_rsrc(4), b_src5 = plane_rsrc(5);
  auto issue_b = [&](int cc, int grp, int buf) {
#pragma unroll
    for (int tt = 0; tt < TPB; ++tt) {
      const int tap = grp * TPB + tt;
      const int soff = (tap * Csw + cc * V2_CK) * 2;
#pragma unroll
      for (int i = 0; i < BSEG; ++i) {
        const int slot = tid + NT * i;
        if (BSEG * NT != BSLOTS && slot - lane >= BSLOTS) continue;
        const int plane = slot / (BN * 4);
        const int rem = slot - plane * BN * 4;
        __bf16* dst_l = Bs + (((buf * TPB + tt) * NP + plane) * BN) * 32 + (rem - lane) * 8;
        __builtin_amdgcn_raw_ptr_buffer_load_lds(
            i == 0 ? b_src0 : i == 1 ? b_src1 : i == 2 ? b_src2 : i == 3 ? b_src3 : i == 4 ? b_src4 : b_src5, (lds_ptr_t)dst_l,
            16, (int)boff[i], soff, 0, 0);
      }
    }
  };

  const int wm = wid / WN_WAVES, wn = wid % WN_WAVES;
  const int lr = lane & 15, kg = lane >> 4;
  const int w_row0 = wn * 16 * TN + lr;
  const int w_off = w_row0 * 32 + ((kg ^ swz(w_row0)) << 3);

  f32x4v acc[TN][TM];
#pragma unroll
  for (int b = 0; b < TN; ++b)
#pragma unroll
    for (int a = 0; a < TM; ++a) acc[b][a] = f32x4v{0.f, 0.f, 0.f, 0.f};

  auto patch_off = [&](int tap) {
    const int ky = tap / KS, kx = tap - KS * ky;
    const int pxs = lr + kx;
    return ((wm * TM + ky) * PWK + pxs) * 32 + ((kg ^ swz(pxs)) << 3);
  };
  auto read_patch = [&](int tap, bf16x8 (&pf)[NP][TM]) {
    const int p_off = patch_off(tap);
#pragma unroll
    for (int p = 0; p < NP; ++p)
#pragma unroll
      for (int tm = 0; tm < TM; ++tm)
        pf[p][tm] = *reinterpret_cast<const bf16x8*>(As + p * NPATCH * 32 + p_off + tm * PWK * 32);
  };
  auto read_w = [&](const __bf16* bt, int tn, bf16x8 (&wf)[NP]) {
#pragma unroll
    for (int p = 0; p < NP; ++p) wf[p] = *reinterpret_cast<const bf16x8*>(bt + p * BN * 32 + tn * 16 * 32);
  };
  auto taps_mma = [&](int grp, int buf, auto&& mid) {
#pragma unroll
    for (int tt = 0; tt < TPB; ++tt) {
      const int tap = grp * TPB + tt;
      const __bf16* bt = Bs + ((buf * TPB + tt) * NP) * BN * 32 + w_off;
      bf16x8 pf[NP][TM];
      read_patch(tap, pf);
#pragma unroll
      for (int tn = 0; tn < TN; ++tn) {
        bf16x8 wf[NP];
        read_w(bt, tn, wf);
        mma_pieces<NP, TM>(wf, pf, acc[tn]);
#ifdef SCAN_EXP_MID_STAGGER
        if (tt == 0 && tn == ((wid >= WAVES / 2 && TN >= 8) ? SCAN_EXP_MID_STAGGER : SCAN_CONV_MID)) {
#else
        if (tt == 0 && tn == SCAN_CONV_MID) {
#endif
          __builtin_amdgcn_sched_barrier(0);
          mid();
          __builtin_amdgcn_sched_barrier(0);
        }
      }
    }
  };
  auto no_mid = []() {};

  constexpr bool PFA = GL && NT == 512 && TPB == 1 && NP == 2 && SCAN_CONV_PFA;
  bf16x8 npf[NP][TM];
  auto taps_mma_pf = [&](int grp, int buf, auto&& mid) {
    if constexpr (PFA) {
      const __bf16* bt = Bs + (buf * NP) * BN * 32 + w_off;
      if (grp == 0) read_patch(0, npf);
#pragma unroll
      for (int tn = 0; tn < TN - 1; ++tn) {
        bf16x8 wf[NP];
        read_w(bt, tn, wf);
        mma_pieces<NP, TM>(wf, npf, acc[tn]);
        if (tn == SCAN_CONV_MID) {
          __builtin_amdgcn_sched_barrier(0);
          mid();
          __builtin_amdgcn_sched_barrier(0);
        }
      }
      {
        constexpr int tn = TN - 1;
        bf16x8 wf[NP];
        read_w(bt, tn, wf);
        const bool more = grp < NGRP - 1;
        const int p_off = patch_off(more ? grp + 1 : grp);
#pragma unroll
        for (int tm = 0; tm < TM; ++tm) {
          acc[tn][tm] = __builtin_amdgcn_mfma_f32_16x16x32_bf16(wf[0], npf[1][tm], acc[tn][tm], 0, 0, 0);
          acc[tn][tm] = __builtin_amdgcn_mfma_f32_16x16x32_bf16(wf[1], npf[0][tm], acc[tn][tm], 0, 0, 0);
          acc[tn][tm] = __builtin_amdgcn_mfma_f32_16x16x32_bf16(wf[0], npf[0][tm], acc[tn][tm], 0, 0, 0);
          npf[0][tm] = *reinterpret_cast<const bf16x8*>(As + p_off + tm * PWK * 32);
          npf[1][tm] = *reinterpret_cast<const bf16x8*>(As + NPATCH * 32 + p_off + tm * PWK * 32);
        }
      }
    }
  };

  load_a(0);
  if constexpr (GL) {
    issue_b(0, 0, 0);
    for (int cc = 0; cc < nchunks; ++cc) {
      __syncthreads();
#ifdef SCAN_EXP_FWD_NOFEED
      if (cc == 0 || !(SCAN_EXP_FWD_NOFEED & 2))
#endif
      store_a();
      if (NGRP == 1 && cc + 1 < nchunks) load_a(cc + 1);
#pragma unroll 1
      for (int grp = 0; grp < NGRP; ++grp) {
        const int buf = (cc * NGRP + grp) & 1;
        asm volatile("s_waitcnt vmcnt(0)" ::: "memory");
        __syncthreads();
        auto feed = [&]() {
#ifdef SCAN_EXP_FWD_NOFEED
          if ((SCAN_EXP_FWD_NOFEED & 1) && !(SCAN_EXP_FWD_NOFEED & 2)) {
            if (NGRP > 1 && grp == NGRP - 2 && cc + 1 < nchunks) load_a(cc + 1);
            return;
          }
          if ((SCAN_EXP_FWD_NOFEED & 3) == 3) return;
#endif
          if (grp < NGRP - 1)
            issue_b(cc, grp + 1, buf ^ 1);
          else if (cc + 1 < nchunks)
            issue_b(cc + 1, 0, buf ^ 1);
          if (NGRP > 1 && grp == NGRP - 2 && cc + 1 < nchunks) load_a(cc + 1);
        };
        if constexpr (PFA) {
          taps_mma_pf(grp, buf, feed);
        } else if (SCAN_CONV_MID >= 0) {
          taps_mma(grp, buf, feed);
        } else {
          feed();
          taps_mma(grp, buf, no_mid);
        }
      }
    }
  } else {
    load_b(0, 0);
    for (int cc = 0; cc < nchunks; ++cc) {
      __syncthreads();
      store_a();
      if (cc + 1 < nchunks) load_a(cc + 1);
#pragma unroll 1
      for (int grp = 0; grp < NGRP; ++grp) {
        const int buf = (cc * NGRP + grp) & 1;
        store_b(buf);
        if (grp < NGRP - 1)
          load_b(cc, grp + 1);
        else if (cc + 1 < nchunks)
          load_b(cc + 1, 0);
        __syncthreads();
        taps_mma(grp, buf, no_mid);
      }
    }
  }

  const int x = tx0 + lr;
  double* gn_red = reinterpret_cast<double*>(smem_raw);
  if (gn_ws != nullptr) __syncthreads();
#pragma unroll
  for (int tn = 0; tn < TN; ++tn) {
    const int o4 = n0 + wn * 16 * TN + tn * 16 + 4 * kg;
    float4 bv = make_float4(0.f, 0.f, 0.f, 0.f);
    if (bias != nullptr) {
      bv.x = o4 + 0 < Nout ? bias[o4 + 0] : 0.f;
      bv.y = o4 + 1 < Nout ? bias[o4 + 1] : 0.f;
      bv.z = o4 + 2 < Nout ? bias[o4 + 2] : 0.f;
      bv.w = o4 + 3 < Nout ? bias[o4 + 3] : 0.f;
    }
    if (relu & 2) {
      const int Hp = H >> 1, Wp = W >> 1;
#pragma unroll
      for (int tm = 0; tm < TM; tm += 2) {
        const int y = ty0 + wm * TM + tm;
        float v[4];
#pragma unroll
        for (int r = 0; r < 4; ++r) {
          const float m = fmaxf(acc[tn][tm][r], acc[tn][tm + 1][r]);
          v[r] = fmaxf(m, __shfl_xor(m, 1, 64));
        }
        if ((lr & 1) == 0 && y < H && x < W && o4 < Nout) {
          float4 o = make_float4(v[0] + bv.x, v[1] + bv.y, v[2] + bv.z, v[3] + bv.w);
          if (relu & 1) {
            o.x = fmaxf(o.x, 0.f);
            o.y = fmaxf(o.y, 0.f);
            o.z = fmaxf(o.z, 0.f);
            o.w = fmaxf(o.w, 0.f);
          }
          *reinterpret_cast<float4*>(dst + ((int64_t)img * Hp * Wp + (int64_t)(y >> 1) * Wp + (x >> 1)) * Ns + o4) = o;
        }
      }
      continue;
    }
    float4 mk[TM];
    if (mask != nullptr) {
#pragma unroll
      for (int tm = 0; tm < TM; ++tm) {
        const int y = ty0 + wm * TM + tm;
        const bool ok = y < H && x < W && o4 < Nout;
        mk[tm] = ok ? *reinterpret_cast<const float4*>(mask + (rowbase + (int64_t)y * W + x) * Ns + o4)
                    : make_float4(0.f, 0.f, 0.f, 0.f);
      }
    }
    double ds = 0.0, dq = 0.0;
#pragma unroll
    for (int tm = 0; tm < TM; ++tm) {
      const int y = ty0 + wm * TM + tm;
      if (y < H && x < W && o4 < Nout) {
        float4 o = make_float4(acc[tn][tm][0] + bv.x, acc[tn][tm][1] + bv.y, acc[tn][tm][2] + bv.z,
                               acc[tn][tm][3] + bv.w);
        if (relu & 1) {
          o.x = fmaxf(o.x, 0.f);
          o.y = fmaxf(o.y, 0.f);
          o.z = fmaxf(o.z, 0.f);
          o.w = fmaxf(o.w, 0.f);
        }
        if (mask != nullptr) {
          o.x = (mk[tm].x > 0.f) ? o.x : 0.f;
          o.y = (mk[tm].y > 0.f) ? o.y : 0.f;
          o.z = (mk[tm].z > 0.f) ? o.z : 0.f;
          o.w = (mk[tm].w > 0.f) ? o.w : 0.f;
        }
#ifdef SCAN_EXP_FWD_NOSTORE
        if (o.x == 1.2345e30f)
#endif
        *reinterpret_cast<float4*>(dst + (rowbase + (int64_t)y * W + x) * Ns + o4) = o;
        ds += (double)((o.x + o.y) + (o.z + o.w));
        dq += (double)((o.x * o.x + o.y * o.y) + (o.z * o.z + o.w * o.w));
      }
    }
    if (gn_ws != nullptr) {
#pragma unroll
      for (int sh = 1; sh <= 16; sh <<= 1) {
        ds += __shfl_xor(ds, sh, 64);
        dq += __shfl_xor(dq, sh, 64);
      }
      if (lr == 0 && (kg & 1) == 0) {
        double* r = gn_red + (wm * (BN / 8) + ((o4 - n0) >> 3)) * 2;
        r[0] = ds;
        r[1] = dq;
      }
    }
  }
  if (gn_ws != nullptr) {
    __syncthreads();
    if (tid < BN / 8 * 2) {
      const int g = n0 / 8 + (tid >> 1);
      double v = 0.0;
#pragma unroll
      for (int w = 0; w < WM_WAVES; ++w) v += gn_red[w * (BN / 8) * 2 + tid];
      if (g * 8 < Nout) atomicAdd(&gn_ws[((int64_t)(lvl * d.n_images + img) * 32 + g) * 2 + (tid & 1)], v);
    }
  }
}

static void make_tiles_v2(const scan_pyramid_t* d, TileTab2* tt, int TH) {
  tt->tile_off[0] = 0;
  for (int l = 0; l < SCAN_MAX_LEVELS; ++l) {
    if (l < d->n_levels) {
      tt->tiles_x[l] = (d->w[l] + V2_TW - 1) / V2_TW;
      tt->tiles_y[l] = (d->h[l] + TH - 1) / TH;
      tt->tile_off[l + 1] = tt->tile_off[l] + d->n_images * tt->tiles_x[l] * tt->tiles_y[l];
    } else {
      tt->tiles_x[l] = tt->tiles_y[l] = 1;
      tt->tile_off[l + 1] = tt->tile_off[l];
    }
  }
}

struct ConvArgs {
  const float* x;
  const scan_pyramid_t* od;
  const scan_pyramid_t* sd;
  int32_t Cs;
  const __bf16* w[3];
  int32_t Csw;
  const float* bias;
  const float* mask;
  float* y;
  int32_t Nout, Ns, relu, map;
  hipStream_t st;
  double* gn_ws;
};

template <int NP, int BN, int TH, int NT, int KS, int TPB = 1, bool GL = false>
static void launch_v2(const ConvArgs& a) {
  constexpr int HALO = KS / 2;
  TileTab2 tt;
  make_tiles_v2(a.od, &tt, TH);
  const int tiles = tt.tile_off[a.od->n_levels];
  const int n_tiles = (a.Nout + BN - 1) / BN;
  constexpr size_t sh = (size_t)(NP * (TH + 2 * HALO) * (V2_TW + 2 * HALO) * 32 + 2 * NP * TPB * BN * 32) * sizeof(__bf16);
  static_assert(sh <= 160 * 1024, "LDS: 160 KB per CU");
  static bool done = false;
  if (!done) {
    hipFuncSetAttribute(reinterpret_cast<const void*>(conv_split_kernel<NP, BN, TH, NT, KS, TPB, GL>),
                        hipFuncAttributeMaxDynamicSharedMemorySize, (int)sh);
    done = true;
  }
  hipLaunchKernelGGL((conv_split_kernel<NP, BN, TH, NT, KS, TPB, GL>), dim3(tiles * n_tiles), dim3(NT), sh, a.st, a.x, *a.od,
                     a.Cs, a.w[0], a.w[1], a.w[2], a.Csw, a.bias, a.mask, a.y, a.Nout, a.Ns, a.relu, tt, n_tiles, *a.sd,
                     a.map, a.gn_ws);
}

int g_scan_conv_bn256 = 2;
int g_scan_conv_wg1024 = 1;
int g_scan_conv_w8 = 1;
int g_scan_conv_tpb3 = 1;
int g_scan_conv_glds = 1;
int g_scan_conv_bn64_th16 = 2;
static int v2_instance(const scan_pyramid_t* od, int32_t Nout) {
  if (Nout <= 64) return 64;
  TileTab2 tt;
  make_tiles_v2(od, &tt, 16);
  const int64_t tiles = tt.tile_off[od->n_levels];
  if (g_scan_conv_bn256 == 1 && Nout % 256 == 0 && tiles * (Nout / 256) >= 512) return 256;
  if (g_scan_conv_bn256 == 2 && Nout % 256 == 0) {
    const int64_t r256 = (tiles * (Nout / 256) + 255) / 256 * 2, r128 = (tiles * (Nout / 128) + 255) / 256;
    if (r256 * 97 <= r128 * 100) return 256;
  }
  return 128;
}

int conv3x3_split_launch(int np, const float* x, const scan_pyramid_t* d, int32_t Cs, const void* w0, const void* w1,
                         const void* w2, int32_t Csw, const float* bias, const float* mask, float* y, int32_t Nout,
                         int32_t Ns, int32_t relu, void* stream, double* gn_ws) {
  ConvArgs a{x, d, d, Cs, {reinterpret_cast<const __bf16*>(w0), reinterpret_cast<const __bf16*>(w1),
                           reinterpret_cast<const __bf16*>(w2)}, Csw, bias, mask, y, Nout, Ns, relu, 0, as_stream(stream), gn_ws};
  const bool whole = g_scan_conv_glds && Csw % 32 == 0;
  const bool th16 = g_scan_conv_bn64_th16 && d->n_levels == 1 && d->h[0] % 16 == 0 && d->w[0] % 16 == 0;
  if (np == 3) {
    switch (v2_instance(d, Nout)) {
      case 64:
        if (whole && th16 && g_scan_conv_bn64_th16 == 2 && d->h[0] % 32 == 0)
          launch_v2<3, 64, 32, 512, 3, 1, true>(a);
        else if (whole && th16)
          launch_v2<3, 64, 16, 512, 3, 1, true>(a);
        else if (whole)
          launch_v2<3, 64, 8, 256, 3, 1, true>(a);
        else if (th16)
          launch_v2<3, 64, 16, 512, 3>(a);
        else
          launch_v2<3, 64, 8, 256, 3>(a);
        break;
      case 256:
        if (whole)
          launch_v2<3, 256, 16, 512, 3, 1, true>(a);
        else
          launch_v2<3, 256, 16, 512, 3>(a);
        break;
      default:
        if (whole)
          launch_v2<3, 128, 16, 512, 3, 1, true>(a);
        else
          launch_v2<3, 128, 16, 512, 3>(a);
        break;
    }
    SCAN_LAUNCH_CHECK("conv3x3_bf16x6");
    return 0;
  }
  switch (v2_instance(d, Nout)) {
    case 64:
      if (th16)
        launch_v2<2, 64, 16, 256, 3>(a);
      else if (g_scan_conv_tpb3 & 2)
        launch_v2<2, 64, 8, 256, 3, 3>(a);
      else
        launch_v2<2, 64, 8, 256, 3>(a);
      break;
    case 256:
      if (g_scan_conv_w8 && g_scan_conv_wg1024 == 1 && whole)
        launch_v2<2, 256, 16, 512, 3, 1, true>(a);
      else if ((g_scan_conv_wg1024 == 1 || (g_scan_conv_wg1024 == 2 && d->n_levels > 1)) && whole)
        launch_v2<2, 256, 16, 1024, 3, 1, true>(a);
      else if (g_scan_conv_wg1024 == 1 || (g_scan_conv_wg1024 == 2 && d->n_levels > 1))
        launch_v2<2, 256, 16, 1024, 3>(a);
      else
        launch_v2<2, 256, 16, 512, 3>(a);
      break;
    default:
      if (g_scan_conv_wg1024 == 1 && (g_scan_conv_tpb3 & 1) && whole && Nout % 128 == 0)
        launch_v2<2, 128, 16, 1024, 3, 3, true>(a);
      else if (g_scan_conv_wg1024 == 1 && (g_scan_conv_tpb3 & 1))
        launch_v2<2, 128, 16, 1024, 3, 3>(a);
      else if (g_scan_conv_wg1024 == 1 && whole && Nout % 128 == 0)
        launch_v2<2, 128, 16, 1024, 3, 1, true>(a);
      else if (g_scan_conv_wg1024 == 1)
        launch_v2<2, 128, 16, 1024, 3>(a);
      else if (g_scan_conv_tpb3 & 1)
        launch_v2<2, 128, 16, 512, 3, 3>(a);
      else
        launch_v2<2, 128, 16, 512, 3>(a);
      break;
  }
  SCAN_LAUNCH_CHECK("conv3x3_bf16x3");
  return 0;
}

static int conv1x1_instance3(const scan_pyramid_t* yd, int32_t Nout, int32_t Csw);
int g_scan_conv1x1 = 3;
static int conv1x1_instance3(const scan_pyramid_t* yd, int32_t Nout, int32_t Csw) {
  if (Nout <= 64) return 64;
  if (!((g_scan_conv1x1 & 1) && Csw % 32 == 0)) return 128;
  if ((g_scan_conv1x1 & 2) && Nout % 256 == 0) {
    TileTab2 tt;
    make_tiles_v2(yd, &tt, 16);
    const int64_t tiles = tt.tile_off[yd->n_levels];
    const int64_t r256 = (tiles * (Nout / 256) + 255) / 256 * 2, r128 = (tiles * (Nout / 128) + 255) / 256;
    if (r256 * 97 <= r128 * 100) return 1256;
  }
  return 1128;
}
extern "C" int scan_conv1x1_bf16x6_instance(const scan_pyramid_t* yd, int32_t Nout, int32_t Csw) {
  return yd ? conv1x1_instance3(yd, Nout, Csw) : -1;
}

int conv1x1_split_launch(int np, const float* x, const scan_pyramid_t* xd, int32_t Cs, const void* w0, const void* w1,
                         const void* w2, int32_t Csw, const float* bias, const float* mask, float* y,
                         const scan_pyramid_t* yd, int32_t Nout, int32_t Ns, int32_t relu, int32_t map, void* stream) {
  ConvArgs a{x, yd, xd, Cs, {reinterpret_cast<const __bf16*>(w0), reinterpret_cast<const __bf16*>(w1),
                             reinterpret_cast<const __bf16*>(w2)}, Csw, bias, mask, y, Nout, Ns, relu, map, as_stream(stream), nullptr};
  const int inst = np == 3 ? conv1x1_instance3(yd, Nout, Csw) : (Nout <= 64 ? 64 : 128);
  const bool wide = inst == 1256, gl = inst >= 1000;
  if (np == 3) {
    if (Nout <= 64)
      launch_v2<3, 64, 8, 256, 1>(a);
    else if (wide)
      launch_v2<3, 256, 16, 512, 1, 1, true>(a);
    else if (gl)
      launch_v2<3, 128, 16, 512, 1, 1, true>(a);
    else
      launch_v2<3, 128, 16, 512, 1>(a);
  } else {
    if (Nout <= 64)
      launch_v2<2, 64, 8, 256, 1>(a);
    else
      launch_v2<2, 128, 16, 512, 1>(a);
  }
  SCAN_LAUNCH_CHECK("conv1x1_split");
  return 0;
}

extern "C" int scan_conv3x3_bf16x3_instance(const scan_pyramid_t* d, int32_t Nout) {
  if (!d) return -1;
  const int bn = v2_instance(d, Nout);
  if (bn == 256 && g_scan_conv_w8 && g_scan_conv_wg1024 == 1 && g_scan_conv_glds) return 2256;
  if (bn == 256 && (g_scan_conv_wg1024 == 1 || (g_scan_conv_wg1024 == 2 && d->n_levels > 1))) return 1256;
  if (bn == 128 && g_scan_conv_wg1024 == 1) return 1128;
  return bn;
}

extern "C" int scan_conv3x3_bf16x6_instance(const scan_pyramid_t* d, int32_t Nout) {
  if (!d) return -1;
  const int bn = v2_instance(d, Nout);
  if (bn == 64 && g_scan_conv_bn64_th16 && d->n_levels == 1 && d->h[0] % 16 == 0 && d->w[0] % 16 == 0)
    return (g_scan_conv_bn64_th16 == 2 && d->h[0] % 32 == 0) ? 2064 : 1064;
  return bn;
}
```

### scan_amd/csrc/conv_split.h

```cpp
#pragma once
#include "common.h"

typedef float f32x4v __attribute__((ext_vector_type(4)));
typedef __bf16 bf16x8 __attribute__((ext_vector_type(8)));
typedef __bf16 bf16x4 __attribute__((ext_vector_type(4)));

typedef float f32x2v __attribute__((ext_vector_type(2)));
typedef __bf16 bf16x2 __attribute__((ext_vector_type(2)));
template <int NP>
__device__ __forceinline__ void split4_np(const float4 v, bf16x4 (&q)[NP]) {
  f32x2v r0 = {v.x, v.y}, r1 = {v.z, v.w};
#pragma unroll
  for (int p = 0; p < NP; ++p) {
    const bf16x2 b0 = __builtin_convertvector(r0, bf16x2), b1 = __builtin_convertvector(r1, bf16x2);
    q[p][0] = b0[0];
    q[p][1] = b0[1];
    q[p][2] = b1[0];
    q[p][3] = b1[1];
    if (p + 1 < NP) {
      const unsigned u0 = __builtin_bit_cast(unsigned, b0), u1 = __builtin_bit_cast(unsigned, b1);
      const f32x2v f0 = {__builtin_bit_cast(float, u0 << 16), __builtin_bit_cast(float, u0 & 0xffff0000u)};
      const f32x2v f1 = {__builtin_bit_cast(float, u1 << 16), __builtin_bit_cast(float, u1 & 0xffff0000u)};
      r0 -= f0;
      r1 -= f1;
    }
  }
}

template <int NP>
__device__ __forceinline__ void split1_np(float v, __bf16 (&q)[NP]) {
#pragma unroll
  for (int p = 0; p < NP; ++p) {
    q[p] = (__bf16)v;
    if (p + 1 < NP) v -= (float)q[p];
  }
}

__device__ __forceinline__ __amdgpu_buffer_rsrc_t uniform_rsrc_b(const void* base, int bytes) {
  const unsigned long long a = reinterpret_cast<unsigned long long>(base);
  const unsigned lo = __builtin_amdgcn_readfirstlane((unsigned)a), hi = __builtin_amdgcn_readfirstlane((unsigned)(a >> 32));
  void* p = reinterpret_cast<void*>(((unsigned long long)hi << 32) | lo);
  return __builtin_amdgcn_make_buffer_rsrc(p, 0, __builtin_amdgcn_readfirstlane(bytes), 0x00020000);
}

__device__ __forceinline__ int xcd_remap(int orig, int nwg) {
  const int q = nwg / 8, r = nwg % 8, xcd = orig % 8;
  const int base = (xcd < r) ? xcd * (q + 1) : r * (q + 1) + (xcd - r) * q;
  return base + orig / 8;
}

typedef __attribute__((address_space(3))) void* lds_ptr_t;
```

### scan_amd/csrc/scan_ops_ext.cpp

```cpp
#include <ATen/ATen.h>
#include <ATen/hip/impl/HIPGuardImplMasqueradingAsCUDA.h>
#include <ATen/hip/impl/HIPStreamMasqueradingAsCUDA.h>
#include <torch/extension.h>

#include <map>
#include <utility>
#include <vector>

#include "../../include/scan_hip.h"

namespace {

using torch::autograd::AutogradContext;
using torch::autograd::variable_list;

void* cur_stream(const at::Tensor& t) { return c10::hip::getCurrentHIPStreamMasqueradingAsCUDA(t.device().index()).stream(); }
void check(int rc, const char* what) { TORCH_CHECK(rc == 0, what, " failed (", rc, "): ", scan_last_error()); }
int64_t pad4(int64_t c) { return (c + 3) / 4 * 4; }
int64_t round_up(int64_t c, int64_t m) { return (c + m - 1) / m * m; }

void require_gpu_f32(const at::Tensor& t, const char* who, const char* what) {
  TORCH_CHECK(t.is_cuda(), who, ": ", what, " must be a GPU tensor (the HIP kernels have no CPU fallback)");
  TORCH_CHECK(t.scalar_type() == at::kFloat, who, ": ", what, " must be float32");
}

scan_pyramid_t one_level(int64_t n, int64_t h, int64_t w) {
  scan_pyramid_t d{};
  d.n_levels = 1;
  d.n_images = (int32_t)n;
  d.h[0] = (int32_t)h;
  d.w[0] = (int32_t)w;
  d.row_off[0] = 0;
  d.row_off[1] = n * h * w;
  return d;
}

at::Tensor to_rows(const at::Tensor& x) {
  const int64_t n = x.size(0), c = x.size(1), h = x.size(2), w = x.size(3);
  at::Tensor r = x.permute({0, 2, 3, 1});
  if (c % 4 != 0) r = at::constant_pad_nd(r, {0, pad4(c) - c}, 0);
  return r.contiguous().view({n * h * w, pad4(c)});
}
at::Tensor to_nchw(const at::Tensor& rows, int64_t n, int64_t h, int64_t w, int64_t c) {
  return rows.view({n, h, w, rows.size(1)}).slice(3, 0, c).permute({0, 3, 1, 2});
}
at::Tensor pack_weight(const at::Tensor& w) {
  const int64_t o = w.size(0), i = w.size(1), t = w.size(2) * w.size(3);
  at::Tensor p = w.permute({0, 2, 3, 1});
  if (i % 4 != 0) p = at::constant_pad_nd(p, {0, pad4(i) - i}, 0);
  return p.contiguous().view({o, t, pad4(i)});
}
at::Tensor unpack_wgrad(const at::Tensor& dwp, int64_t i, int64_t k) {
  return dwp.view({dwp.size(0), k, k, dwp.size(2)}).slice(3, 0, i).permute({0, 3, 1, 2});
}

struct Planes {
  at::Tensor p[3];
  int64_t csw;
};

struct PlaneEntry {
  at::Tensor keep;
  uint32_t version;
  int64_t epoch;
  void* stream;
  int64_t o, t, cs;
  Planes pl;
};
int64_t g_plane_epoch = 0;
std::map<std::pair<const void*, int>, PlaneEntry>& plane_cache() {
  static std::map<std::pair<const void*, int>, PlaneEntry> c;
  return c;
}
void invalidate_weight_cache() {
  ++g_plane_epoch;
  plane_cache().clear();
}
Planes split3_uncached(const at::Tensor& wp, int mode, int64_t cs_src);
Planes split3(const at::Tensor& wp, int mode, int64_t cs_src, const at::Tensor& owner = at::Tensor()) {
  if (!owner.defined() || owner.data_ptr() != wp.data_ptr()) return split3_uncached(wp, mode, cs_src);
  const auto key = std::make_pair((const void*)wp.data_ptr(), mode);
  void* st = cur_stream(wp);
  auto& cache = plane_cache();
  auto it = cache.find(key);
  if (it != cache.end()) {
    const PlaneEntry& e = it->second;
    if (e.version == owner._version() && e.epoch == g_plane_epoch && e.stream == st && e.o == wp.size(0) && e.t == wp.size(1) &&
        e.cs == wp.size(2))
      return e.pl;
  }
  if (cache.size() > 512) cache.clear();
  PlaneEntry e{wp, owner._version(), g_plane_epoch, st, wp.size(0), wp.size(1), wp.size(2), split3_uncached(wp, mode, cs_src)};
  cache[key] = e;
  return e.pl;
}
Planes split3_uncached(const at::Tensor& wp, int mode, int64_t cs_src) {
  const int64_t o = wp.size(0), t = wp.size(1), cs = wp.size(2);
  const int64_t rnd = t == 9 ? 32 : 8;
  Planes pl;
  const int64_t rows = mode == 0 ? o : cs;
  pl.csw = round_up(mode == 0 ? cs : std::max(o, cs_src), rnd);
  for (auto& q : pl.p) q = at::empty({rows, t, pl.csw}, wp.options().dtype(at::kBFloat16));
  check(scan_weight_split3(wp.data_ptr<float>(), (int32_t)o, (int32_t)t, (int32_t)cs, mode, pl.p[0].data_ptr(), pl.p[1].data_ptr(),
                           pl.p[2].data_ptr(), (int32_t)pl.csw, cur_stream(wp)),
        "scan_weight_split3");
  return pl;
}

const float* opt_ptr(const at::Tensor& t) { return t.defined() ? t.data_ptr<float>() : nullptr; }

struct ConvGeom {
  int64_t n, cin, h, w, cout, k, stride, ho, wo, cs, ns;
};
ConvGeom geom(const at::Tensor& x, const at::Tensor& weight, int64_t stride, const char* who) {
  require_gpu_f32(x, who, "input");
  require_gpu_f32(weight, who, "weight");
  TORCH_CHECK(x.dim() == 4 && weight.dim() == 4, who, ": input [N, C, H, W] and weight [O, I, k, k]");
  TORCH_CHECK(weight.size(1) == x.size(1), who, ": weight expects ", weight.size(1), " input channels, got ", x.size(1));
  TORCH_CHECK(weight.size(2) == weight.size(3) && (weight.size(2) == 1 || weight.size(2) == 3), who,
              ": kernel size 1 or 3 (square), padding = k // 2 -- the convolutions the SCAN modules build");
  TORCH_CHECK(stride == 1 || stride == 2, who, ": stride 1 or 2");
  ConvGeom g;
  g.n = x.size(0), g.cin = x.size(1), g.h = x.size(2), g.w = x.size(3);
  g.cout = weight.size(0), g.k = weight.size(2), g.stride = stride;
  g.ho = (g.h - 1) / stride + 1, g.wo = (g.w - 1) / stride + 1;
  g.cs = pad4(g.cin), g.ns = pad4(g.cout);
  return g;
}

at::Tensor conv_rows_forward(const at::Tensor& xr, const at::Tensor& wp, const at::Tensor& bias, const ConvGeom& g, bool relu,
                             at::Tensor gn_sums, const at::Tensor& owner = at::Tensor()) {
  const scan_pyramid_t xd = one_level(g.n, g.h, g.w), yd = one_level(g.n, g.ho, g.wo);
  at::Tensor y = g.ns != g.cout ? at::zeros({yd.row_off[1], g.ns}, xr.options()) : at::empty({yd.row_off[1], g.ns}, xr.options());
  void* st = cur_stream(xr);
  if (g.k == 3 && g.stride == 2) {
    check(scan_conv2d_forward(xr.data_ptr<float>(), &xd, (int32_t)g.cs, wp.data_ptr<float>(), opt_ptr(bias), y.data_ptr<float>(), &yd,
                              (int32_t)g.cout, (int32_t)g.ns, 3, 2, relu ? 1 : 0, st),
          "scan_conv2d_forward");
    return y;
  }
  if (g.k == 3 && g.stride == 1 && g.cs == 4 && g.cout <= 64 && !gn_sums.defined()) {
    check(scan_conv_smallcin_bf16x6(xr.data_ptr<float>(), (int32_t)g.n, (int32_t)g.h, (int32_t)g.w, wp.data_ptr<float>(), opt_ptr(bias),
                                    y.data_ptr<float>(), (int32_t)g.cout, (int32_t)g.ns, 3, 1, relu ? 1 : 0, st),
          "scan_conv_smallcin_bf16x6");
    return y;
  }
  const Planes pl = split3(wp, 0, g.cs, owner);
  if (g.k == 3) {
    if (gn_sums.defined())
      check(scan_conv3x3_gn_bf16x6(xr.data_ptr<float>(), &xd, (int32_t)g.cs, pl.p[0].data_ptr(), pl.p[1].data_ptr(), pl.p[2].data_ptr(),
                                   (int32_t)pl.csw, opt_ptr(bias), y.data_ptr<float>(), (int32_t)g.cout, (int32_t)g.ns,
                                   reinterpret_cast<float*>(gn_sums.data_ptr()), 1, st),
            "scan_conv3x3_gn_bf16x6");
    else
      check(scan_conv3x3_bf16x6(xr.data_ptr<float>(), &xd, (int32_t)g.cs, pl.p[0].data_ptr(), pl.p[1].data_ptr(), pl.p[2].data_ptr(),
                                (int32_t)pl.csw, opt_ptr(bias), nullptr, y.data_ptr<float>(), (int32_t)g.cout, (int32_t)g.ns,
                                relu ? 1 : 0, st),
            "scan_conv3x3_bf16x6");
  } else {
    check(scan_conv1x1_bf16x6(xr.data_ptr<float>(), &xd, (int32_t)g.cs, pl.p[0].data_ptr(), pl.p[1].data_ptr(), pl.p[2].data_ptr(),
                              (int32_t)pl.csw, opt_ptr(bias), nullptr, y.data_ptr<float>(), &yd, (int32_t)g.cout, (int32_t)g.ns,
                              relu ? 1 : 0, g.stride == 2 ? 1 : 0, st),
          "scan_conv1x1_bf16x6");
  }
  return y;
}

std::vector<at::Tensor> conv_rows_backward(const at::Tensor& xr, const at::Tensor& wp, const at::Tensor& dyr, const ConvGeom& g,
                                           bool need_dx, bool need_dw, bool need_db, const at::Tensor& owner = at::Tensor()) {
  const scan_pyramid_t xd = one_level(g.n, g.h, g.w), yd = one_level(g.n, g.ho, g.wo);
  void* st = cur_stream(xr);
  const int64_t T = g.k * g.k;
  at::Tensor dx, dw, db;
  if (need_dx) {
    dx = at::empty({xd.row_off[1], g.cs}, xr.options());
    if (g.k == 3 && g.stride == 2) {
      at::Tensor wt = at::empty({g.cs, T, g.ns}, xr.options());
      check(scan_weight_transpose(wp.data_ptr<float>(), (int32_t)g.cout, (int32_t)T, (int32_t)g.cs, wt.data_ptr<float>(), (int32_t)g.ns, st),
            "scan_weight_transpose");
      check(scan_conv2d_dgrad(dyr.data_ptr<float>(), &yd, (int32_t)g.ns, wt.data_ptr<float>(), dx.data_ptr<float>(), &xd, (int32_t)g.cs,
                              (int32_t)g.cs, 3, 2, nullptr, st),
            "scan_conv2d_dgrad");
    } else {
      const Planes pl = split3(wp, 1, g.ns, owner);
      if (g.k == 3)
        check(scan_conv3x3_bf16x6(dyr.data_ptr<float>(), &yd, (int32_t)g.ns, pl.p[0].data_ptr(), pl.p[1].data_ptr(), pl.p[2].data_ptr(),
                                  (int32_t)pl.csw, nullptr, nullptr, dx.data_ptr<float>(), (int32_t)g.cs, (int32_t)g.cs, 0, st),
              "scan_conv3x3_bf16x6 (data gradient)");
      else
        check(scan_conv1x1_bf16x6(dyr.data_ptr<float>(), &yd, (int32_t)g.ns, pl.p[0].data_ptr(), pl.p[1].data_ptr(), pl.p[2].data_ptr(),
                                  (int32_t)pl.csw, nullptr, nullptr, dx.data_ptr<float>(), &xd, (int32_t)g.cs, (int32_t)g.cs, 0,
                                  g.stride == 2 ? 2 : 0, st),
              "scan_conv1x1_bf16x6 (data gradient)");
    }
  }
  if (need_dw || need_db) {
    dw = at::empty({g.cout, T, g.cs}, xr.options());
    if (need_db) db = at::empty({g.cout}, xr.options());
    if (g.k == 3 && g.stride == 1) {
      at::Tensor ws = at::empty({scan_conv3x3_wgrad_bf16x6_ws_floats(&xd, (int32_t)g.cs, (int32_t)g.cout)}, xr.options());
      check(scan_conv3x3_wgrad_bf16x6(xr.data_ptr<float>(), &xd, (int32_t)g.cs, dyr.data_ptr<float>(), (int32_t)g.cout, (int32_t)g.ns,
                                      dw.data_ptr<float>(), need_db ? db.data_ptr<float>() : nullptr, 0, ws.data_ptr<float>(), st),
            "scan_conv3x3_wgrad_bf16x6");
    } else if (g.k == 1) {
      at::Tensor ws = at::empty({scan_conv1x1_wgrad_bf16x6_ws_floats(&yd, (int32_t)g.cs, (int32_t)g.cout)}, xr.options());
      check(scan_conv1x1_wgrad_bf16x6(xr.data_ptr<float>(), &xd, (int32_t)g.cs, dyr.data_ptr<float>(), &yd, (int32_t)g.cout, (int32_t)g.ns,
                                      (int32_t)g.stride, dw.data_ptr<float>(), need_db ? db.data_ptr<float>() : nullptr, 0,
                                      ws.data_ptr<float>(), st),
            "scan_conv1x1_wgrad_bf16x6");
    } else {
      at::Tensor ws = at::empty({scan_conv2d_wgrad_ws_floats(&yd, (int32_t)g.cs, (int32_t)g.cout, 3)}, xr.options());
      check(scan_conv2d_wgrad(xr.data_ptr<float>(), &xd, (int32_t)g.cs, dyr.data_ptr<float>(), &yd, (int32_t)g.cout, (int32_t)g.ns, 3, 2,
                              dw.data_ptr<float>(), 0, ws.data_ptr<float>(), st),
            "scan_conv2d_wgrad");
      if (need_db) {
        at::Tensor cws = at::empty({scan_colsum_ws_floats(yd.row_off[1], (int32_t)g.cout)}, xr.options());
        check(scan_colsum(dyr.data_ptr<float>(), yd.row_off[1], (int32_t)g.cout, (int32_t)g.ns, db.data_ptr<float>(), 0,
                          cws.data_ptr<float>(), st),
              "scan_colsum");
      }
    }
  }
  return {dx, dw, db};
}

ConvGeom geom_of(const std::vector<int64_t>& v) { return ConvGeom{v[0], v[1], v[2], v[3], v[4], v[5], v[6], v[7], v[8], v[9], v[10]}; }
std::vector<int64_t> geom_vec(const ConvGeom& g) { return {g.n, g.cin, g.h, g.w, g.cout, g.k, g.stride, g.ho, g.wo, g.cs, g.ns}; }

struct Conv2dFn : public torch::autograd::Function<Conv2dFn> {
  static at::Tensor forward(AutogradContext* ctx, at::Tensor xr, at::Tensor weight, c10::optional<at::Tensor> bias_opt,
                            std::vector<int64_t> gv, bool relu) {
    const at::Tensor bias = bias_opt.has_value() ? *bias_opt : at::Tensor();
    const ConvGeom g = geom_of(gv);
    c10::hip::HIPGuardMasqueradingAsCUDA guard(xr.device());
    at::Tensor wp = pack_weight(weight);
    at::Tensor bc = bias.defined() ? bias.contiguous() : bias;
    const bool wp_view = wp.data_ptr() == weight.data_ptr();
    at::Tensor y = conv_rows_forward(xr, wp, bc, g, relu, at::Tensor(), wp_view ? wp : at::Tensor());
    ctx->save_for_backward({xr, wp, relu ? y : at::Tensor()});
    ctx->saved_data["wp_view"] = wp_view;
    ctx->saved_data["geom"] = gv;
    ctx->saved_data["relu"] = relu;
    ctx->saved_data["has_bias"] = bias.defined();
    return y;
  }
  static variable_list backward(AutogradContext* ctx, variable_list grads) {
    const auto saved = ctx->get_saved_variables();
    const at::Tensor xr = saved[0], wp = saved[1], y = saved[2];
    const ConvGeom g = geom_of(ctx->saved_data["geom"].toIntVector());
    c10::hip::HIPGuardMasqueradingAsCUDA guard(xr.device());
    at::Tensor dyr = grads[0].contiguous();
    if (ctx->saved_data["relu"].toBool()) {
      at::Tensor t = at::empty_like(dyr);
      check(scan_relu_backward(dyr.data_ptr<float>(), y.data_ptr<float>(), t.data_ptr<float>(), dyr.numel(), cur_stream(dyr)),
            "scan_relu_backward");
      dyr = t;
    }
    const bool has_bias = ctx->saved_data["has_bias"].toBool();
    auto r = conv_rows_backward(xr, wp, dyr, g, ctx->needs_input_grad(0), ctx->needs_input_grad(1),
                                has_bias && ctx->needs_input_grad(2), ctx->saved_data["wp_view"].toBool() ? wp : at::Tensor());
    at::Tensor dw = (r[1].defined() && ctx->needs_input_grad(1)) ? unpack_wgrad(r[1], g.cin, g.k) : at::Tensor();
    return {r[0], dw, r[2], at::Tensor(), at::Tensor()};
  }
};

constexpr int kGroups = 32;

at::Tensor gn_rows_backward(const at::Tensor& xr, const at::Tensor& gamma, const at::Tensor& beta, const at::Tensor& stats,
                            const at::Tensor& dyr, const scan_pyramid_t& d, bool relu, at::Tensor& dgamma, at::Tensor& dbeta) {
  const int32_t C = (int32_t)xr.size(1);
  at::Tensor dx = at::empty_like(xr);
  dgamma = at::empty({C}, xr.options());
  dbeta = at::empty({C}, xr.options());
  at::Tensor ws = at::empty({scan_groupnorm_ws_floats(&d, C, kGroups) / 2 + 1}, xr.options().dtype(at::kDouble));
  check(scan_groupnorm_relu_backward(xr.data_ptr<float>(), beta.data_ptr<float>(), dyr.data_ptr<float>(), &d, C, kGroups,
                                     stats.data_ptr<float>(), gamma.data_ptr<float>(), relu ? 1 : 0, dx.data_ptr<float>(),
                                     dgamma.data_ptr<float>(), dbeta.data_ptr<float>(), 0, reinterpret_cast<float*>(ws.data_ptr()),
                                     cur_stream(xr)),
        "scan_groupnorm_relu_backward");
  return dx;
}

struct GroupNormReluFn : public torch::autograd::Function<GroupNormReluFn> {
  static at::Tensor forward(AutogradContext* ctx, at::Tensor xr, at::Tensor gamma, at::Tensor beta, std::vector<int64_t> dims,
                            double eps, bool relu) {
    c10::hip::HIPGuardMasqueradingAsCUDA guard(xr.device());
    const int64_t n = dims[0], c = dims[1], h = dims[2], w = dims[3];
    const scan_pyramid_t d = one_level(n, h, w);
    at::Tensor gc = gamma.contiguous(), bc = beta.contiguous();
    at::Tensor stats = at::empty({n * kGroups * 2}, xr.options()), y = at::empty_like(xr);
    at::Tensor ws = at::empty({scan_groupnorm_ws_floats(&d, (int32_t)c, kGroups) / 2 + 1}, xr.options().dtype(at::kDouble));
    void* st = cur_stream(xr);
    check(scan_groupnorm_stats(xr.data_ptr<float>(), &d, (int32_t)c, kGroups, (float)eps, stats.data_ptr<float>(),
                               reinterpret_cast<float*>(ws.data_ptr()), st),
          "scan_groupnorm_stats");
    check(scan_groupnorm_relu_forward(xr.data_ptr<float>(), &d, (int32_t)c, kGroups, stats.data_ptr<float>(), gc.data_ptr<float>(),
                                      bc.data_ptr<float>(), relu ? 1 : 0, y.data_ptr<float>(), st),
          "scan_groupnorm_relu_forward");
    ctx->save_for_backward({xr, gc, bc, stats});
    ctx->saved_data["dims"] = dims;
    ctx->saved_data["relu"] = relu;
    return y;
  }
  static variable_list backward(AutogradContext* ctx, variable_list grads) {
    const auto s = ctx->get_saved_variables();
    const auto v = ctx->saved_data["dims"].toIntVector();
    c10::hip::HIPGuardMasqueradingAsCUDA guard(s[0].device());
    const scan_pyramid_t d = one_level(v[0], v[2], v[3]);
    at::Tensor dg, db;
    at::Tensor dx = gn_rows_backward(s[0], s[1], s[2], s[3], grads[0].contiguous(), d, ctx->saved_data["relu"].toBool(), dg, db);
    return {dx, dg, db, at::Tensor(), at::Tensor(), at::Tensor()};
  }
};

struct ConvGnReluFn : public torch::autograd::Function<ConvGnReluFn> {
  static at::Tensor forward(AutogradContext* ctx, at::Tensor xr, at::Tensor weight, c10::optional<at::Tensor> bias_opt, at::Tensor gamma,
                            at::Tensor beta, std::vector<int64_t> gv, double eps, bool relu) {
    const at::Tensor bias = bias_opt.has_value() ? *bias_opt : at::Tensor();
    const ConvGeom g = geom_of(gv);
    c10::hip::HIPGuardMasqueradingAsCUDA guard(xr.device());
    at::Tensor wp = pack_weight(weight), gc = gamma.contiguous(), bc = beta.contiguous();
    at::Tensor cb = bias.defined() ? bias.contiguous() : bias;
    const scan_pyramid_t d = one_level(g.n, g.h, g.w);
    at::Tensor sums = at::empty({g.n * kGroups * 2}, xr.options().dtype(at::kDouble));
    const bool wp_view = wp.data_ptr() == weight.data_ptr();
    at::Tensor c = conv_rows_forward(xr, wp, cb, g, false, sums, wp_view ? wp : at::Tensor());
    ctx->saved_data["wp_view"] = wp_view;
    at::Tensor stats = at::empty({g.n * kGroups * 2}, xr.options()), y = at::empty_like(c);
    check(scan_groupnorm_relu_forward_from_sums(c.data_ptr<float>(), &d, 256, kGroups, reinterpret_cast<float*>(sums.data_ptr()),
                                                (float)eps, gc.data_ptr<float>(), bc.data_ptr<float>(), relu ? 1 : 0, y.data_ptr<float>(),
                                                stats.data_ptr<float>(), cur_stream(xr)),
          "scan_groupnorm_relu_forward_from_sums");
    ctx->save_for_backward({xr, wp, c, gc, bc, stats});
    ctx->saved_data["geom"] = gv;
    ctx->saved_data["relu"] = relu;
    ctx->saved_data["has_bias"] = bias.defined();
    return y;
  }
// ... 101 lines not shown
```

### scan_amd/ops.py

```python
import contextlib
import ctypes
import os
import weakref

import torch

from . import _lib
from ._lib import PyramidDesc, call, query


def _ptr(t):
    return ctypes.c_void_p(t.data_ptr()) if t is not None else ctypes.c_void_p(0)


def _stream():
    return ctypes.c_void_p(torch._C._cuda_getCurrentRawStream(torch._C._cuda_getDevice()))


def _chk(*ts):
    for t in ts:
        if t is None:
            continue
        if not t.is_cuda:
            raise RuntimeError("scan_amd ops run only on the GPU (HIP) -- got a %s tensor; no CPU fallback" % t.device)
# ... 130 lines not shown
def _round8(c):
    return (c + 7) // 8 * 8


BATCHED = os.environ.get("SCAN_BATCHED", "1") != "0"
CAT_IN_PLACE = os.environ.get("SCAN_CAT_IN_PLACE", "1") != "0"
FPN_DIRECT = os.environ.get("SCAN_FPN_DIRECT", "1") != "0"
SIDE_STREAMS = []


def borrow_side_streams(n):
    while len(SIDE_STREAMS) < n:
        SIDE_STREAMS.append(torch.cuda.Stream())
    return SIDE_STREAMS[:n]


WGRAD_STREAM = None
HEAD_OUT_SPLIT = os.environ.get("SCAN_HEAD_OUT_SPLIT", "1") != "0"
SPLIT_EPOCH = None
_split_cache = {}
_epoch_counter = [0]
_active_plan = None


class SplitPlan:

    def __init__(self):
        self.jobs = {}
        self.table = None
        self.order = []
        self.blocks = 0
        self.dirty = True

    def add(self, key, param, O, T, cs_w, mode, rows, csw, planes):
        self.jobs[key] = (weakref.ref(param), O, T, cs_w, mode, rows, csw, planes)
        self.dirty = True

    def run(self):
        npc = split_pieces()
        dead = [k for k, j in self.jobs.items() if j[0]() is None or j[0]().data_ptr() != k[0] or (npc > 0 and k[3] != npc)]
        for k in dead:
            _split_cache.pop(k, None)
            del self.jobs[k]
        if dead:
            self.dirty = True
        if not self.jobs:
            return
        if self.dirty:
            rows, off = [], 0
            self.order = list(self.jobs.keys())
            for k in self.order:
                _, O, T, cs_w, mode, r, csw, planes = self.jobs[k]
                rows.append([k[0], planes[0].data_ptr(), planes[1].data_ptr(), O, T, cs_w, mode, r, csw, off,
                             planes[2].data_ptr() if len(planes) == 3 else 0])
                off += query("scan_weight_split_job_blocks", O, T, cs_w, mode, csw)
            dev = self.jobs[self.order[0]][7][0].device
            self.table = torch.tensor(rows, dtype=torch.int64).to(dev)
            self.blocks = off
            self.dirty = False
        call("scan_weight_split_batched", _ptr(self.table), len(self.order), int(self.table.shape[1]), self.blocks, _stream())
        ev = torch.cuda.Event()
        ev.record(torch.cuda.current_stream())
        for k in self.order:
            _split_cache[k] = (SPLIT_EPOCH, self.jobs[k][7], ev)


ZERO_POOL = os.environ.get("SCAN_ZERO_POOL", "1") != "0"
_zero_pool = {"buf": None, "off": 0, "active": False}
_ZERO_POOL_DOUBLES = 1 << 20


def _ws_f64(n, device):
    zp = _zero_pool
    n_al = (n + 31) // 32 * 32
    if ZERO_POOL and zp["active"] and zp["buf"] is not None and zp["buf"].device == device \
            and zp["off"] + n_al <= _ZERO_POOL_DOUBLES:
        out = zp["buf"][zp["off"]:zp["off"] + n]
        zp["off"] += n_al
        return out, True
    return torch.empty((n,), dtype=torch.float64, device=device), False


_loss_zero = {"buf": None, "off": 0}


def _zeros_f32(n, device):
    lz = _loss_zero
    n_al = (n + 15) // 16 * 16
    if ZERO_POOL and _zero_pool["active"] and lz["buf"] is not None and lz["buf"].device == device \
            and lz["off"] + n_al <= lz["buf"].numel():
        out = lz["buf"][lz["off"]:lz["off"] + n]
        lz["off"] += n_al
        return out
    return torch.zeros((n,), dtype=torch.float32, device=device)


def _reset_zero_pool(device):
    _loss_zero["buf"] = torch.zeros((1024,), dtype=torch.float32, device=device) \
        if ZERO_POOL and device is not None and device.type == "cuda" else None
    _loss_zero["off"] = 0
    zp = _zero_pool
    if not ZERO_POOL or device is None or device.type != "cuda":
        zp["active"] = False
        return
    if zp["buf"] is None or zp["buf"].device != device:
        zp["buf"] = torch.zeros((_ZERO_POOL_DOUBLES,), dtype=torch.float64, device=device)
    elif zp["off"] > 0:
        zp["buf"][:zp["off"]].zero_()
    zp["off"] = 0
    zp["active"] = True


CACHE_PLAIN_PARAMS = False


def begin_weight_epoch(plan=None, device=None):
    global SPLIT_EPOCH, _active_plan
    _epoch_counter[0] += 1
    SPLIT_EPOCH = _epoch_counter[0]
    _split_cache.clear()
    _active_plan = plan if BATCHED else None
    _reset_zero_pool(device)
    if _active_plan is not None:
        _active_plan.run()


def invalidate_weight_planes():
    global SPLIT_EPOCH, _active_plan
    SPLIT_EPOCH = None
    _active_plan = None
    _zero_pool["active"] = False
    _split_cache.clear()
    if _EXT_INVALIDATE is not None:
        _EXT_INVALIDATE()


_EXT_INVALIDATE = None


_gn_sums = {}


def _conv_split(x, shape, wp, cout, rows_out, cs_src, mode, bias, relu, ns, name, flops, cache_key=None,
                mask=None, dst_shape=None, cmap=0, pool=False, gn_sums=False, param=None, out=None, pieces=None):
    st = _stream()
    npc = pieces or split_pieces()
    sfx = "bf16x6" if npc == 3 else "bf16x3"
    O, T, cs_w = wp.shape
    rnd = _round32 if T == 9 else _round8
    if mode == 0:
        rows, csw, nout = O, rnd(cs_w), O
    else:
        rows, csw, nout = cs_w, rnd(max(O, cs_src)), cs_w
    hit = None
    if cache_key is not None and SPLIT_EPOCH is not None:
        key = (cache_key, mode, csw, npc)
        hit = _split_cache.get(key)
        if hit is not None and (hit[0] != SPLIT_EPOCH or tuple(hit[1][0].shape) != (rows, T, csw)):
            hit = None
    if hit is not None:
        planes = hit[1]
        torch.cuda.current_stream().wait_event(hit[2])
    else:
        planes = tuple(torch.empty((rows, T, csw), dtype=torch.bfloat16, device=x.device) for _ in range(npc))
        if npc == 3:
            call("scan_weight_split3", _ptr(wp), O, T, cs_w, mode, _ptr(planes[0]), _ptr(planes[1]), _ptr(planes[2]), csw, st)
        else:
            call("scan_weight_split", _ptr(wp), O, T, cs_w, mode, _ptr(planes[0]), _ptr(planes[1]), csw, st)
        if cache_key is not None and SPLIT_EPOCH is not None:
            ev = torch.cuda.Event()
            ev.record(torch.cuda.current_stream())
            _split_cache[(cache_key, mode, csw, npc)] = (SPLIT_EPOCH, planes, ev)
            if _active_plan is not None and param is not None and wp.data_ptr() == cache_key == param.data_ptr():
                _active_plan.add((cache_key, mode, csw, npc), param, O, T, cs_w, mode, rows, csw, planes)
    wptrs = [_ptr(t) for t in planes]
    y = out if out is not None else (x.new_zeros if ns != nout else x.new_empty)((rows_out, ns))
    if kernel_timer.enabled:
        if T == 9:
            inst = query("scan_conv3x3_%s_instance" % sfx, (dst_shape or shape).ref(), nout)
        elif npc == 3:
            inst = query("scan_conv1x1_bf16x6_instance", (dst_shape or shape).ref(), nout, csw)
        else:
            inst = 128 if nout > 64 else 64
        ev = kernel_timer.begin("%s_bn%d" % (name, inst), flops)
    else:
        ev = None
    if gn_sums:
        sums, cleared = _ws_f64(shape.n_levels * shape.n_images * 32 * 2, x.device)
        if npc == 3:
            call("scan_conv3x3_gn_bf16x6", _ptr(x), shape.ref(), cs_src, *wptrs, csw, _ptr(bias), _ptr(y), nout, ns,
                 _ptr(sums), 0 if cleared else 1, st)
        else:
            call("scan_conv3x3_gn_acc_bf16x3" if cleared else "scan_conv3x3_gn_bf16x3", _ptr(x), shape.ref(), cs_src, *wptrs, csw,
                 _ptr(bias), _ptr(y), nout, ns, _ptr(sums), st)
        _gn_sums.clear()
        _gn_sums[y.data_ptr()] = sums
    elif pool:
        call("scan_conv3x3_pool2_" + sfx, _ptr(x), shape.ref(), cs_src, *wptrs, csw, _ptr(bias), _ptr(y),
             nout, ns, int(bool(relu)), st)
    elif T == 1:
        call("scan_conv1x1_" + sfx, _ptr(x), shape.ref(), cs_src, *wptrs, csw, _ptr(bias), _ptr(mask),
             _ptr(y), (dst_shape or shape).ref(), nout, ns, int(bool(relu)), cmap, st)
    else:
        fn = "scan_conv3x3_" + sfx
        rem = nout % 128
        if nout > 128 and 0 < rem <= 64 and cs_src >= 512 and rows_out >= 100000:
            main = nout - rem

            def off(t, nbytes):
                return ctypes.c_void_p(t.data_ptr() + nbytes) if t is not None else ctypes.c_void_p(0)

            call(fn, _ptr(x), shape.ref(), cs_src, *wptrs, csw, _ptr(bias), _ptr(mask), _ptr(y), main, ns,
                 int(bool(relu)), st)
            call(fn, _ptr(x), shape.ref(), cs_src, *[off(t, main * T * csw * 2) for t in planes], csw, off(bias, main * 4),
                 off(mask, main * 4), off(y, main * 4), rem, ns, int(bool(relu)), st)
        else:
            call(fn, _ptr(x), shape.ref(), cs_src, *wptrs, csw, _ptr(bias), _ptr(mask), _ptr(y), nout, ns,
                 int(bool(relu)), st)
    kernel_timer.end(ev)
    return y


class _Conv2d(torch.autograd.Function):

    @staticmethod
    def forward(ctx, x, weight, bias, shape, ksize, stride, relu, cout_s, mask_dx=False, pool=False, gn_sums=False,
                out=None):
        _chk(x, bias)
        if not weight.is_cuda:
            raise RuntimeError("scan_amd ops run only on the GPU (HIP); no CPU fallback")
        cs = x.shape[1]
        assert x.shape[0] == shape.rows, (x.shape, shape)
        cout = weight.shape[0]
        cout_s = cout_s or pad4(cout)
        wp = pack_weight(weight, cs)
        oshape = shape.conv_out(ksize, stride)
        if out is not None:
            if pool or not (out.is_cuda and out.dtype == torch.float32 and out.is_contiguous()
                            and tuple(out.shape) == (oshape.rows, cout_s) and cout_s == cout):
                raise RuntimeError("conv2d(out=...): needs a contiguous fp32 [%d, %d] GPU block with Cout == Cout_s"
                                   % (oshape.rows, cout_s))
        fast = split_pieces() > 0 and ((ksize == 3 and stride == 1) or ksize == 1)
        tag = CONV_MODE
        flops = 2.0 * oshape.rows * cout * ksize * ksize * weight.shape[1]
        ckey = weight.data_ptr() if (getattr(weight, "_scan_flat", False)
                                     or (CACHE_PLAIN_PARAMS and isinstance(weight, torch.nn.Parameter))) else None
        first = split_pieces() > 0 and cs == 4 and cout <= 64 and (ksize, stride) in ((3, 1), (7, 2)) \
            and shape.n_levels == 1
        if first:
            (h, w_), n = shape.sizes[0], shape.n_images
            y = out if out is not None else (x.new_zeros if cout_s != cout else x.new_empty)((oshape.rows, cout_s))
            ev = kernel_timer.begin("conv_smallcin_" + tag, flops)
            call("scan_conv_smallcin_" + tag, _ptr(x), n, h, w_, _ptr(wp), _ptr(bias), _ptr(y), cout, cout_s, ksize,
                 stride, int(bool(relu)), _stream())
            kernel_timer.end(ev)
        elif fast:
            if pool:
                if ksize != 3 or shape.n_levels != 1:
                    raise RuntimeError("conv2d(pool=True) needs a 3x3 conv on a single-level pyramid")
                (h, w_) = shape.sizes[0]
                y = _conv_split(x, shape, wp, cout, shape.n_images * (h // 2) * (w_ // 2), cs, 0, bias, relu, cout_s,
                                    "conv3x3_%s_fwd" % tag, flops, cache_key=ckey, pool=True, param=weight)
            else:
                y = _conv_split(x, shape, wp, cout, oshape.rows, cs, 0, bias, relu, cout_s,
                                    ("conv3x3_%s_fwd" if ksize == 3 else "conv1x1_%s_fwd") % tag, flops,
                                    cache_key=ckey, dst_shape=oshape, cmap=stride - 1, param=weight,
                                    gn_sums=gn_sums and ksize == 3 and cout == 256 and cout_s == 256 and not relu,
                                    out=out)
        else:
            y = out if out is not None else (x.new_zeros if cout_s != cout else x.new_empty)((oshape.rows, cout_s))
            ev = kernel_timer.begin("conv_igemm_fwd", flops)
            call("scan_conv2d_forward", _ptr(x), shape.ref(), cs, _ptr(wp), _ptr(bias), _ptr(y), oshape.ref(), cout,
                 cout_s, ksize, stride, int(bool(relu)), _stream())
            kernel_timer.end(ev)
        ctx.save_for_backward(x, weight, y if relu is True else None)
        ctx.cfg = (shape, oshape, ksize, stride, relu, cout_s, bias is not None, fast)
        ctx.conv_mode = CONV_MODE
        ctx.mask_dx = mask_dx
        ctx.ckey = ckey
        ctx.wgrad_buf = ctx.bgrad_buf = None
        if getattr(weight, "_scan_flat", False) and weight.grad is not None and weight.shape[1] == cs \
                and weight.grad.permute(0, 2, 3, 1).is_contiguous():
            ctx.wgrad_buf = weight.grad
            if bias is not None and getattr(bias, "_scan_flat", False) and bias.grad is not None:
                ctx.bgrad_buf = bias.grad
        return y

    @staticmethod
    def backward(ctx, dy):
        x, weight, y = ctx.saved_tensors
        shape, oshape, ksize, stride, relu, cout_s, has_bias, fast = ctx.cfg
        cs = x.shape[1]
        cout, cin = weight.shape[0], weight.shape[1]
        T = ksize * ksize
        st = _stream()
        sfx = ctx.conv_mode if ctx.conv_mode in SPLIT_MODES else "bf16x3"
        dy = dy.contiguous()
        if relu is True:
            g = torch.empty_like(dy)
            call("scan_relu_backward", _ptr(dy), _ptr(y), _ptr(g), dy.numel(), st)
            dy = g
        dx = dw = db = None
        mask = x if ctx.mask_dx else None
        if ctx.needs_input_grad[0] and fast:
            dx = _conv_split(dy, oshape, pack_weight(weight, cs), cout, x.shape[0], cout_s, 1, None, False, cs,
                                 ("conv3x3_%s_dgrad" if ksize == 3 else "conv1x1_%s_dgrad") % sfx,
                                 2.0 * oshape.rows * cout * T * cin, cache_key=ctx.ckey, mask=mask, dst_shape=shape,
                                 cmap=0 if stride == 1 else 2, param=weight, pieces=SPLIT_MODES[sfx])
        elif ctx.needs_input_grad[0]:
            wp = pack_weight(weight, cs)
            wt = x.new_empty((cs, T, cout_s))
            call("scan_weight_transpose", _ptr(wp), cout, T, cs, _ptr(wt), cout_s, st)
            dx = torch.empty_like(x)
            ev = kernel_timer.begin("conv_igemm_dgrad", 2.0 * oshape.rows * cout * T * cin)
            call("scan_conv2d_dgrad", _ptr(dy), oshape.ref(), cout_s, _ptr(wt), _ptr(dx), shape.ref(), cs, cs, ksize,
                 stride, _ptr(mask), st)
            kernel_timer.end(ev)
        direct_w = ctx.wgrad_buf is not None
        direct_b = direct_w and ctx.bgrad_buf is not None
        db_done = False
        if ctx.needs_input_grad[1] and fast and ksize == 3:
            want_db = has_bias and ctx.needs_input_grad[2]
            side = WGRAD_STREAM if (direct_w and (direct_b or not want_db) and not kernel_timer.enabled) else None
            if side is not None:
                side.wait_stream(torch.cuda.current_stream())
                x.record_stream(side)
                dy.record_stream(side)
            with torch.cuda.stream(side) if side is not None else contextlib.nullcontext():
                ws = x.new_empty((query("scan_conv3x3_wgrad_%s_ws_floats" % sfx, shape.ref(), cs, cout),))
                dwp = ctx.wgrad_buf if direct_w else x.new_empty((cout, T, cs))
                ev = kernel_timer.begin("conv3x3_%s_wgrad" % sfx, 2.0 * oshape.rows * cout * T * cin)
                if want_db:
                    db = ctx.bgrad_buf if direct_b else x.new_empty((cout,))
                    db_done = True
                call("scan_conv3x3_wgrad_" + sfx, _ptr(x), shape.ref(), cs, _ptr(dy), cout, cout_s, _ptr(dwp),
                     _ptr(db) if want_db else None, int(direct_w), _ptr(ws), _stream())
                kernel_timer.end(ev)
            if want_db and direct_w and not direct_b:
                raise RuntimeError("conv2d: flat weight gradient without a flat bias gradient")
            dw = None if direct_w else unpack_weight_grad(dwp, weight)
            if direct_b:
                db = None
        elif ctx.needs_input_grad[1] and fast:
            ws = x.new_empty((query("scan_conv1x1_wgrad_%s_ws_floats" % sfx, oshape.ref(), cs, cout),))
            dwp = ctx.wgrad_buf if direct_w else x.new_empty((cout, T, cs))
            ev = kernel_timer.begin("conv1x1_%s_wgrad" % sfx, 2.0 * oshape.rows * cout * T * cin)
            want_db = has_bias and ctx.needs_input_grad[2]
            if want_db:
                db = ctx.bgrad_buf if direct_b else x.new_empty((cout,))
                db_done = True
            call("scan_conv1x1_wgrad_" + sfx, _ptr(x), shape.ref(), cs, _ptr(dy), oshape.ref(), cout, cout_s, stride,
                 _ptr(dwp), _ptr(db) if want_db else None, int(direct_w), _ptr(ws), st)
            kernel_timer.end(ev)
            if want_db and direct_w and not direct_b:
                raise RuntimeError("conv2d: flat weight gradient without a flat bias gradient")
            dw = None if direct_w else unpack_weight_grad(dwp, weight)
            if direct_b:
                db = None
        elif ctx.needs_input_grad[1]:
# ... 886 lines not shown
```

Baseline: 21.34.

## Add 1-D Winograd F(2,3) bf16x6 3x3 convolution for forward and data gradient

Adds a Winograd F(2,3) variant along the width axis for 3x3 convolutions. Each 3-tap row filter is transformed into 4 weight taps, so the kernel uses 12 transformed taps instead of 9 and produces two output columns per transformed input tile. The weight-split kernels gain modes 2 and 3 that apply the G transform, in double precision, before cutting each weight into three bf16 pieces. The Python and C++ dispatchers route forward, fused GroupNorm-sum, fused pool and data-gradient convolutions to the new kernel when the selector approves. The aim is to cut matrix-core multiplies per output by about a third. In exchange it adds an input transform inside the kernel, larger weight planes, and rounding error from the transformed weights.

```diff
diff --git a/include/scan_hip.h b/include/scan_hip.h
--- a/include/scan_hip.h
+++ b/include/scan_hip.h
@@ -146,6 +146,10 @@
                               const scan_pyramid_t* yd, int32_t Cout, int32_t Cout_s, int32_t stride, float* dw,
                               float* db, int32_t accumulate, float* ws, void* stream);
 int scan_conv3x3_bf16x6_instance(const scan_pyramid_t* d, int32_t Nout);
+int scan_conv3x3_wino_bf16x6(const float* x, const scan_pyramid_t* d, int32_t Cs, const void* wh, const void* wm,
+                             const void* wl, int32_t Csw, const float* bias, const float* mask, float* y, int32_t Nout,
+                             int32_t Ns, int32_t relu, float* gn_ws, int32_t clear, void* stream);
+int scan_conv3x3_bf16x6_wino(int32_t Nout, int32_t Csw);
 int scan_weight_transpose(const float* w, int32_t Cout, int32_t T, int32_t Cin_s, float* wt, int32_t Cout_s,
                           void* stream);
 int64_t scan_colsum_ws_floats(int64_t M, int32_t C);
diff --git a/scan_amd/_lib.py b/scan_amd/_lib.py
--- a/scan_amd/_lib.py
+++ b/scan_amd/_lib.py
@@ -50,6 +50,9 @@
     "scan_conv3x3_bf16x3_instance": (ctypes.c_int, [_PD, c_i32]),
     "scan_conv1x1_bf16x6_instance": (ctypes.c_int, [_PD, c_i32, c_i32]),
     "scan_conv3x3_bf16x6_instance": (ctypes.c_int, [_PD, c_i32]),
+    "scan_conv3x3_bf16x6_wino": (ctypes.c_int, [c_i32, c_i32]),
+    "scan_conv3x3_wino_bf16x6": (ctypes.c_int, [c_vp, _PD, c_i32, c_vp, c_vp, c_vp, c_i32, c_vp, c_vp, c_vp, c_i32, c_i32, c_i32,
+                                                c_vp, c_i32, c_vp]),
     "scan_sigmoid_focal_loss_forward": (ctypes.c_int, [c_vp, c_vp, c_i64, c_i32, c_f32, c_f32, c_vp, c_vp, c_vp]),
     "scan_sigmoid_focal_loss_backward": (ctypes.c_int, [c_vp, c_vp, c_vp, c_f32, c_i64, c_i32, c_f32, c_f32, c_vp, c_vp]),
     "scan_iou_loss_forward": (ctypes.c_int, [c_vp, c_vp, c_vp, c_i64, c_vp, c_vp]),
diff --git a/scan_amd/csrc/batched.hip b/scan_amd/csrc/batched.hip
--- a/scan_amd/csrc/batched.hip
+++ b/scan_amd/csrc/batched.hip
@@ -33,6 +33,24 @@
             Csw = (int)job[8];
   const int64_t blk = (int64_t)blockIdx.x - job[9];
   const int tid = threadIdx.x;
+  if (mode == 2) {
+    const int64_t total = (int64_t)rows * 12 * Csw;
+    const int64_t i = blk * SPLIT_ELEMS_PER_BLOCK + (int64_t)tid * 8;
+    if (i >= total) return;
+    const int col = (int)(i % Csw);
+    const int64_t rt = i / Csw;
+    const int tt = (int)(rt % 12), row = (int)(rt / 12);
+    const int j = tt / 3, ky = tt - 3 * j;
+    const float* src = w + ((int64_t)row * T + ky * 3) * Cs + col;
+    float v[8];
+#pragma unroll
+    for (int k = 0; k < 8; ++k) {
+      const bool in = col + k < Cs;
+      v[k] = wino_g(j, in ? src[k] : 0.f, in ? src[Cs + k] : 0.f, in ? src[2 * Cs + k] : 0.f);
+    }
+    split8_store(v, wh, wl, w2, i);
+    return;
+  }
   if (mode == 0) {
     const int64_t total = (int64_t)rows * T * Csw;
     const int64_t i = blk * SPLIT_ELEMS_PER_BLOCK + (int64_t)tid * 8;
@@ -57,6 +75,7 @@
   const int to = (int)(blk % tiles_o);
   const int tc = (int)((blk / tiles_o) % tiles_c);
   const int tt = (int)(blk / ((int64_t)tiles_o * tiles_c));
+  const int TO = mode == 3 ? 12 : T;
   const int o0 = to * SPLIT_TILE, c0 = tc * SPLIT_TILE;
   {
     const int cl = (tid & 15) * 4, ol = tid >> 4;
@@ -65,14 +84,26 @@
       const int o = o0 + ol + 16 * p, c = c0 + cl;
       float4 a = make_float4(0.f, 0.f, 0.f, 0.f);
       if (o < O && c < Cs) {
-        const float* src = w + ((int64_t)o * T + (T - 1 - tt)) * Cs + c;
-        if (c + 4 <= Cs && (Cs & 3) == 0) {
-          a = *reinterpret_cast<const float4*>(src);
+        auto read4 = [&](int t) {
+          const float* src = w + ((int64_t)o * T + t) * Cs + c;
+          float4 r = make_float4(0.f, 0.f, 0.f, 0.f);
+          if (c + 4 <= Cs && (Cs & 3) == 0) {
+            r = *reinterpret_cast<const float4*>(src);
+          } else {
+            r.x = src[0];
+            if (c + 1 < Cs) r.y = src[1];
+            if (c + 2 < Cs) r.z = src[2];
+            if (c + 3 < Cs) r.w = src[3];
+          }
+          return r;
+        };
+        if (mode == 1) {
+          a = read4(T - 1 - tt);
         } else {
-          a.x = src[0];
-          if (c + 1 < Cs) a.y = src[1];
-          if (c + 2 < Cs) a.z = src[2];
-          if (c + 3 < Cs) a.w = src[3];
+          const int j = tt / 3, ky = tt - 3 * j;
+          const float4 g0 = read4(8 - ky * 3), g1 = read4(7 - ky * 3), g2 = read4(6 - ky * 3);
+          a = make_float4(wino_g(j, g0.x, g1.x, g2.x), wino_g(j, g0.y, g1.y, g2.y), wino_g(j, g0.z, g1.z, g2.z),
+                          wino_g(j, g0.w, g1.w, g2.w));
         }
       }
       float* t = &tile[ol + 16 * p][cl];
@@ -89,16 +120,17 @@
         float v[8];
 #pragma unroll
         for (int k = 0; k < 8; ++k) v[k] = tile[o8 + k][cl + 32 * p];
-        split8_store(v, wh, wl, w2, ((int64_t)c * T + tt) * Csw + o);
+        split8_store(v, wh, wl, w2, ((int64_t)c * TO + tt) * Csw + o);
       }
     }
   }
 }
 
 extern "C" int64_t scan_weight_split_job_blocks(int32_t O, int32_t T, int32_t Cs, int32_t mode, int32_t Csw) {
-  if (mode == 0) return ((int64_t)O * T * Csw + SPLIT_ELEMS_PER_BLOCK - 1) / SPLIT_ELEMS_PER_BLOCK;
+  const int64_t TO = mode >= 2 ? 12 : T;
+  if (mode == 0 || mode == 2) return ((int64_t)O * TO * Csw + SPLIT_ELEMS_PER_BLOCK - 1) / SPLIT_ELEMS_PER_BLOCK;
   const int64_t tiles_o = (Csw + SPLIT_TILE - 1) / SPLIT_TILE, tiles_c = (Cs + SPLIT_TILE - 1) / SPLIT_TILE;
-  return tiles_o * tiles_c * T;
+  return tiles_o * tiles_c * TO;
 }
 
 extern "C" int scan_weight_split_batched(const int64_t* jobs, int32_t n_jobs, int32_t job_words, int64_t total_blocks,
diff --git a/scan_amd/csrc/capi.cpp b/scan_amd/csrc/capi.cpp
--- a/scan_amd/csrc/capi.cpp
+++ b/scan_amd/csrc/capi.cpp
@@ -24,6 +24,7 @@
 extern int g_scan_conv_bn64_th16;
 extern int g_scan_conv_glds;
 extern int g_scan_conv1x1;
+extern int g_scan_conv_wino;
 extern int g_scan_wgrad_v6;
 extern int g_scan_wgrad_prio;
 extern int g_scan_wgrad_tile;
@@ -44,6 +45,7 @@
       {"conv_glds", &g_scan_conv_glds, 0},     {"wgrad_v6", &g_scan_wgrad_v6, 0},       {"wgrad_prio", &g_scan_wgrad_prio, 0},
       {"wgrad_tile", &g_scan_wgrad_tile, 0},   {"wgrad_wgs", &g_scan_wgrad_wgs, 0},     {"gconv_mfma", &g_scan_gconv_mfma, 0},
       {"dbscan_bf16x3", &g_scan_dbscan_bf16x3, 0}, {"reduce_blocks", &g_scan_reduce_blocks, 0}, {"conv1x1", &g_scan_conv1x1, 0},
+      {"conv_wino", &g_scan_conv_wino, 0},
   };
   static bool init = false;
   if (!init) {
diff --git a/scan_amd/csrc/conv_bf16x3.hip b/scan_amd/csrc/conv_bf16x3.hip
--- a/scan_amd/csrc/conv_bf16x3.hip
+++ b/scan_amd/csrc/conv_bf16x3.hip
@@ -297,17 +297,27 @@
 template <int NP>
 __global__ void weight_split_kernel(const float* __restrict__ w, int O, int T, int Cs, int mode, int rows, int Csw,
                                     __bf16* __restrict__ w0, __bf16* __restrict__ w1, __bf16* __restrict__ w2) {
-  const int64_t total = (int64_t)rows * T * Csw;
+  const int TO = mode >= 2 ? 12 : T;
+  const int64_t total = (int64_t)rows * TO * Csw;
   for (int64_t i = (int64_t)blockIdx.x * blockDim.x + threadIdx.x; i < total; i += (int64_t)gridDim.x * blockDim.x) {
     const int col = (int)(i % Csw);
     const int64_t rt = i / Csw;
-    const int tt = (int)(rt % T);
-    const int row = (int)(rt / T);
+    const int tt = (int)(rt % TO);
+    const int row = (int)(rt / TO);
     float v = 0.f;
     if (mode == 0) {
       if (col < Cs) v = w[((int64_t)row * T + tt) * Cs + col];
+    } else if (mode == 1) {
+      if (col < O) v = w[((int64_t)col * T + (T - 1 - tt)) * Cs + row];
     } else {
-      if (col < O) v = w[((int64_t)col * T + (T - 1 - tt)) * Cs + row];
+      const int j = tt / 3, ky = tt - 3 * j;
+      double g[3] = {0.0, 0.0, 0.0};
+      for (int kx = 0; kx < 3; ++kx) {
+        const int t = ky * 3 + kx;
+        if (mode == 2 && col < Cs) g[kx] = w[((int64_t)row * T + t) * Cs + col];
+        if (mode == 3 && col < O) g[kx] = w[((int64_t)col * T + (T - 1 - t)) * Cs + row];
+      }
+      v = wino_g(j, g[0], g[1], g[2]);
     }
     __bf16 q[NP];
     split1_np<NP>(v, q);
@@ -346,11 +356,12 @@
 static int weight_split_launch(int np, const float* w, int32_t O, int32_t T, int32_t Cs, int32_t mode, void* w0, void* w1,
                                void* w2, int32_t Csw, void* stream) {
   SCAN_CHECK_ARG(w && w0 && w1 && (np == 2 || w2) && O > 0 && T > 0 && Cs > 0, "weight_split: bad arguments");
-  SCAN_CHECK_ARG(mode == 0 || mode == 1, "weight_split: mode must be 0 or 1");
-  SCAN_CHECK_ARG(Csw % 8 == 0 && Csw >= (mode == 0 ? Cs : O), "weight_split: Csw=%d must be a multiple of 8 and cover the row",
-                 Csw);
-  const int rows = mode == 0 ? O : Cs;
-  const int64_t total = (int64_t)rows * T * Csw;
+  SCAN_CHECK_ARG(mode >= 0 && mode <= 3, "weight_split: mode must be 0..3");
+  SCAN_CHECK_ARG(mode < 2 || (np == 3 && T == 9), "weight_split: the Winograd modes 2 / 3 take three pieces and T = 9");
+  SCAN_CHECK_ARG(Csw % 8 == 0 && Csw >= ((mode & 1) == 0 ? Cs : O),
+                 "weight_split: Csw=%d must be a multiple of 8 and cover the row", Csw);
+  const int rows = (mode & 1) == 0 ? O : Cs;
+  const int64_t total = (int64_t)rows * (mode >= 2 ? 12 : T) * Csw;
   __bf16 *p0 = reinterpret_cast<__bf16*>(w0), *p1 = reinterpret_cast<__bf16*>(w1), *p2 = reinterpret_cast<__bf16*>(w2);
   if (np == 3)
     hipLaunchKernelGGL(weight_split_kernel<3>, dim3(grid_for(total, 256)), dim3(256), 0, as_stream(stream), w, O, T, Cs, mode,
@@ -470,6 +481,32 @@
   return conv3x3_gn_launch(3, clear, x, d, Cs, wh, wm, wl, Csw, bias, y, Nout, Ns, gn_ws, stream);
 }
 
+int conv3x3_wino_launch(const float* x, const scan_pyramid_t* d, int32_t Cs, const void* w0, const void* w1, const void* w2,
+                        int32_t Csw, const float* bias, const float* mask, float* y, int32_t Nout, int32_t Ns, int32_t relu,
+                        void* stream, double* gn_ws);
+extern "C" int scan_conv3x3_wino_bf16x6(const float* x, const scan_pyramid_t* d, int32_t Cs, const void* wh, const void* wm,
+                                        const void* wl, int32_t Csw, const float* bias, const float* mask, float* y,
+                                        int32_t Nout, int32_t Ns, int32_t relu, float* gn_ws, int32_t clear, void* stream) {
+  SCAN_CHECK_ARG(x && d && wh && wm && wl && y && Cs > 0 && Cs % 4 == 0 && Csw >= Cs && Nout > 0 && Ns >= Nout &&
+                     d->n_levels >= 1 && d->n_levels <= SCAN_MAX_LEVELS && d->n_images >= 1 && v2_ok(y, mask, Ns),
+                 "conv3x3_wino_bf16x6: bad arguments");
+  if (gn_ws != nullptr) {
+    SCAN_CHECK_ARG(Nout == 256 && mask == nullptr && !relu, "conv3x3_wino_bf16x6: GroupNorm sums need Nout == 256, no mask, no ReLU");
+    if (clear) {
+      const size_t bytes = sizeof(double) * 2 * 32 * (size_t)d->n_levels * d->n_images;
+      if (hipMemsetAsync(gn_ws, 0, bytes, as_stream(stream)) != hipSuccess) {
+        scan_set_error("conv3x3_wino_bf16x6: memset failed");
+        return -2;
+      }
+    }
+  }
+  if (relu & 2)
+    SCAN_CHECK_ARG(d->n_levels == 1 && (d->h[0] & 1) == 0 && (d->w[0] & 1) == 0 && mask == nullptr && gn_ws == nullptr,
+                   "conv3x3_wino_bf16x6: the fused pool needs a single-level pyramid with even H and W, no mask, no sums");
+  return conv3x3_wino_launch(x, d, Cs, wh, wm, wl, Csw, bias, mask, y, Nout, Ns, relu & 3, stream,
+                             reinterpret_cast<double*>(gn_ws));
+}
+
 extern "C" int scan_conv3x3_pool2_bf16x3(const float* x, const scan_pyramid_t* d, int32_t Cs, const void* wh,
                                          const void* wl, int32_t Csw, const float* bias, float* y, int32_t Nout,
                                          int32_t Ns, int32_t relu, void* stream) {
diff --git a/scan_amd/csrc/conv_fwd.hip b/scan_amd/csrc/conv_fwd.hip
--- a/scan_amd/csrc/conv_fwd.hip
+++ b/scan_amd/csrc/conv_fwd.hip
@@ -16,6 +16,7 @@
 };
 
 __device__ __forceinline__ int swz(int idx) { return (idx >> 1) & 2; }
+__device__ __forceinline__ int wsw(int t, int r) { return ((t >> 1) & 2) ^ (r & 1); }
 
 template <int K>
 __device__ __forceinline__ const __bf16* pick_plane(const __bf16* w0, const __bf16* w1, const __bf16* w2) {
@@ -56,7 +57,7 @@
       for (int tm = 0; tm < TM; ++tm) acc[tm] = __builtin_amdgcn_mfma_f32_16x16x32_bf16(w[i], p[s - i][tm], acc[tm], 0, 0, 0);
 }
 
-template <int NP, int BN, int TH, int NT, int KS, int TPB = 1, bool GL = false>
+template <int NP, int BN, int TH, int NT, int KS, int TPB = 1, bool GL = false, bool WINO = false>
 __global__ __launch_bounds__(NT, NT == 1024 ? 4 : 2) void conv_split_kernel(
     const float* __restrict__ src, scan_pyramid_t d, int Cs, const __bf16* __restrict__ w0, const __bf16* __restrict__ w1,
     const __bf16* __restrict__ w2, int Csw, const float* __restrict__ bias, const float* __restrict__ mask,
@@ -64,21 +65,25 @@
     double* __restrict__ gn_ws) {
   constexpr int HALO = KS / 2, NTAPS = KS * KS;
   constexpr int PH = TH + 2 * HALO;
-  constexpr int PWK = V2_TW + 2 * HALO;
+  constexpr int PWK = WINO ? 32 : V2_TW + 2 * HALO;
   constexpr int NPATCH = PH * PWK;
+  constexpr int WTAPS = WINO ? 12 : NTAPS;
   constexpr int WAVES = NT / 64;
   constexpr int WN_WAVES = BN >= 128 ? 2 : 1;
   constexpr int WM_WAVES = WAVES / WN_WAVES;
   constexpr int TM = TH / WM_WAVES;
   constexpr int TN = BN / (16 * WN_WAVES);
-  constexpr int ASLOTS = (NPATCH * 8 + NT - 1) / NT;
+  constexpr int TMW = WINO ? TM / 2 : TM;
+  constexpr int ASLOTS = WINO ? (PH * 64 + NT - 1) / NT : (NPATCH * 8 + NT - 1) / NT;
+  constexpr int AK = WINO ? 4 : 1;
   constexpr int BSLOTS = BN * 4 * NP;
   constexpr int BSEG = (BSLOTS + NT - 1) / NT;
-  constexpr int NGRP = NTAPS / TPB;
+  constexpr int NGRP = WTAPS / TPB;
   static_assert(NP == 2 || NP == 3, "two or three pieces per operand");
   static_assert(TM * WM_WAVES == TH && (TM % 2) == 0, "tile rows must split evenly (and pair up for the fused pool)");
   static_assert(NTAPS % TPB == 0, "taps per barrier must divide the tap count");
   static_assert(BSLOTS % 64 == 0, "a wave's 64 weight segments lie in one plane (and past the end only as a whole wave)");
+  static_assert(!WINO || (GL && KS == 3 && TPB == 1 && NP == 3 && TM % 2 == 0), "Winograd: three pieces, 3x3, LDS-DMA weights");
 
   extern __shared__ __align__(16) unsigned char smem_raw[];
   __bf16* As = reinterpret_cast<__bf16*>(smem_raw);
@@ -104,6 +109,7 @@
 
   constexpr unsigned BAD = 0x80000000u;
   unsigned voff[ASLOTS];
+  unsigned vok = 0;
   const int c_tail = Cs - (nchunks - 1) * V2_CK;
   const bool tail_bad = 4 * (tid & 7) >= c_tail;
   __amdgpu_buffer_rsrc_t a_src;
@@ -118,35 +124,77 @@
     else
       base_row = sd.row_off[lvl] + ((int64_t)img * Hs + (ty0 >> 1)) * Ws + (tx0 >> 1);
     a_src = uniform_rsrc_b(src + base_row * Cs, 0x7ffffff0);
-#pragma unroll
-    for (int i = 0; i < ASLOTS; ++i) {
-      const int slot = tid + NT * i;
-      const int q = slot >> 3, c4 = slot & 7;
-      const int py = q / PWK, px = q - py * PWK;
-      const int y = ty0 - HALO + py, x = tx0 - HALO + px;
-      bool ok = (slot < NPATCH * 8) && y >= 0 && y < H && x >= 0 && x < W;
-      int pix = py * W + px;
-      if (mapped) {
-        if (map == 1) {
-          ok = ok && 2 * y < Hs && 2 * x < Ws;
-          pix = 2 * py * Ws + 2 * px;
-        } else {
-          ok = ok && ((y | x) & 1) == 0 && (y >> 1) < Hs && (x >> 1) < Ws;
-          pix = (py >> 1) * Ws + (px >> 1);
-        }
-      }
-      voff[i] = ok ? (unsigned)((pix * Cs + 4 * c4) * 4) : BAD;
-    }
-  }
-  float4 ra[ASLOTS];
+    if constexpr (WINO) {
+#pragma unroll
+      for (int i = 0; i < ASLOTS; ++i) {
+        const int slot = tid + NT * i;
+        const int c4 = slot & 7, t = (slot >> 3) & 7, py = slot >> 6;
+        voff[i] = (unsigned)(((py * W + 2 * t) * Cs + 4 * c4) * 4);
+#pragma unroll
+        for (int k = 0; k < 4; ++k) {
+          const int y = ty0 - HALO + py, x = tx0 - HALO + 2 * t + k;
+          if ((slot < PH * 64) && y >= 0 && y < H && x >= 0 && x < W) vok |= 1u << (4 * i + k);
+        }
+      }
+    } else {
+#pragma unroll
+      for (int i = 0; i < ASLOTS; ++i) {
+        const int slot = tid + NT * i;
+        const int q = slot >> 3, c4 = slot & 7;
+        const int py = q / PWK, px = q - py * PWK;
+        const int y = ty0 - HALO + py, x = tx0 - HALO + px;
+        bool ok = (slot < NPATCH * 8) && y >= 0 && y < H && x >= 0 && x < W;
+        int pix = py * W + px;
+        if (mapped) {
+          if (map == 1) {
+            ok = ok && 2 * y < Hs && 2 * x < Ws;
+            pix = 2 * py * Ws + 2 * px;
+          } else {
+            ok = ok && ((y | x) & 1) == 0 && (y >> 1) < Hs && (x >> 1) < Ws;
+            pix = (py >> 1) * Ws + (px >> 1);
+          }
+        }
+        voff[i] = ok ? (unsigned)((pix * Cs + 4 * c4) * 4) : BAD;
+      }
+    }
+  }
+  float4 ra[ASLOTS][AK];
   auto load_a = [&](int cc) {
     const int soff = cc * (V2_CK * 4);
     const bool kill = tail_bad && cc == nchunks - 1;
 #pragma unroll
     for (int i = 0; i < ASLOTS; ++i)
-      ra[i] = __builtin_bit_cast(float4, __builtin_amdgcn_raw_buffer_load_b128(a_src, (int)(kill ? BAD : voff[i]), soff, 0));
+#pragma unroll
+      for (int k = 0; k < AK; ++k) {
+        const unsigned off = !WINO ? voff[i] : ((vok >> (4 * i + k)) & 1) ? voff[i] + (unsigned)(k * Cs * 4) : BAD;
+        ra[i][k] = __builtin_bit_cast(float4, __builtin_amdgcn_raw_buffer_load_b128(a_src, (int)(kill ? BAD : off), soff, 0));
+      }
   };
   auto store_a = [&]() {
+    if constexpr (WINO) {
+#pragma unroll
+      for (int i = 0; i < ASLOTS; ++i) {
+        const int slot = tid + NT * i;
+        if (slot < PH * 64) {
+          const int c4 = slot & 7, t = (slot >> 3) & 7, py = slot >> 6;
+          const float4 d0 = ra[i][0], d1 = ra[i][1], d2 = ra[i][2], d3 = ra[i][3];
+          const float4 u[4] = {make_float4(d0.x - d2.x, d0.y - d2.y, d0.z - d2.z, d0.w - d2.w),
+                               make_float4(d1.x + d2.x, d1.y + d2.y, d1.z + d2.z, d1.w + d2.w),
+                               make_float4(d2.x - d1.x, d2.y - d1.y, d2.z - d1.z, d2.w - d1.w),
+                               make_float4(d1.x - d3.x, d1.y - d3.y, d1.z - d3.z, d1.w - d3.w)};
+          const int sl = (((c4 >> 1) ^ wsw(t, py)) << 3) + ((c4 & 1) << 2);
+#pragma unroll
+          for (int j = 0; j < 4; ++j) {
+            bf16x4 pc[NP];
+            split4_np<NP>(u[j], pc);
+            const int off = (py * PWK + j * 8 + t) * 32 + sl;
+#pragma unroll
+            for (int p = 0; p < NP; ++p) *reinterpret_cast<bf16x4*>(As + p * NPATCH * 32 + off) = pc[p];
+          }
+        }
+      }
+      return;
+    }
 #pragma unroll
     for (int i = 0; i < ASLOTS; ++i) {
       const int slot = tid + NT * i;
@@ -154,7 +202,7 @@
         const int q = slot >> 3, c4 = slot & 7;
         const int px = q % PWK;
         bf16x4 pc[NP];
-        split4_np<NP>(ra[i], pc);
+        split4_np<NP>(ra[i][0], pc);
         const int off = q * 32 + (((c4 >> 1) ^ swz(px)) << 3) + ((c4 & 1) << 2);
 #pragma unroll
         for (int p = 0; p < NP; ++p) *reinterpret_cast<bf16x4*>(As + p * NPATCH * 32 + off) = pc[p];
@@ -203,9 +251,9 @@
     const int plane = slot / (BN * 4);
     const int rem = slot - plane * BN * 4;
     const int row = rem >> 2, seg = (rem & 3) ^ swz(row);
-    boff[i] = (unsigned)((((n0 + row) * NTAPS) * Csw + 8 * seg) * 2);
-  }
-  const int plane_bytes = Nout * NTAPS * Csw * 2;
+    boff[i] = (unsigned)((((n0 + row) * WTAPS) * Csw + 8 * seg) * 2);
+  }
+  const int plane_bytes = Nout * WTAPS * Csw * 2;
   auto plane_rsrc = [&](int i) { return uniform_rsrc_b(slot_plane_i<NT, BN * 4, NP>(i, tid, w0, w1, w2), plane_bytes); };
   const __amdgpu_buffer_rsrc_t b_src0 = plane_rsrc(0), b_src1 = plane_rsrc(1), b_src2 = plane_rsrc(2),
                                b_src3 = plane_rsrc(3), b_src4 = plane_rsrc(4), b_src5 = plane_rsrc(5);
@@ -238,6 +286,13 @@
   for (int b = 0; b < TN; ++b)
 #pragma unroll
     for (int a = 0; a < TM; ++a) acc[b][a] = f32x4v{0.f, 0.f, 0.f, 0.f};
+  f32x4v wacc[WINO ? 4 : 1][WINO ? TN : 1][TMW];
+#pragma unroll
+  for (int j = 0; j < (WINO ? 4 : 1); ++j)
+#pragma unroll
+    for (int b = 0; b < (WINO ? TN : 1); ++b)
+#pragma unroll
+      for (int a = 0; a < TMW; ++a) wacc[j][b][a] = f32x4v{0.f, 0.f, 0.f, 0.f};
 
   auto patch_off = [&](int tap) {
     const int ky = tap / KS, kx = tap - KS * ky;
@@ -317,8 +372,57 @@
     }
   };
 
+  auto wino_mma = [&](int j, int ky, int buf, f32x4v (&aj)[WINO ? TN : 1][TMW], auto&& mid) {
+    const __bf16* bt = Bs + (buf * NP) * BN * 32 + w_off;
+    const int prow = wm * TM + (lr >> 3) + ky, t = lr & 7;
+    const int p_off = (prow * PWK + j * 8 + t) * 32 + ((kg ^ wsw(t, prow)) << 3);
+    bf16x8 pf[NP][TMW];
+#pragma unroll
+    for (int p = 0; p < NP; ++p)
+#pragma unroll
+      for (int tm = 0; tm < TMW; ++tm)
+        pf[p][tm] = *reinterpret_cast<const bf16x8*>(As + p * NPATCH * 32 + p_off + tm * 2 * PWK * 32);
+#pragma unroll
+    for (int tn = 0; tn < TN; ++tn) {
+      bf16x8 wf[NP];
+      read_w(bt, tn, wf);
+      mma_pieces<NP, TMW>(wf, pf, aj[tn]);
+      if (tn == (SCAN_CONV_MID >= 0 ? SCAN_CONV_MID : 0)) {
+        __builtin_amdgcn_sched_barrier(0);
+        mid();
+        __builtin_amdgcn_sched_barrier(0);
+      }
+    }
+  };
+
   load_a(0);
-  if constexpr (GL) {
+  if constexpr (WINO) {
+    issue_b(0, 0, 0);
+    for (int cc = 0; cc < nchunks; ++cc) {
+      __syncthreads();
+      store_a();
+      auto comp = [&](int j, f32x4v (&aj)[WINO ? TN : 1][TMW]) {
+#pragma unroll 1
+        for (int ky = 0; ky < 3; ++ky) {
+          const int grp = j * 3 + ky, buf = grp & 1;
+          asm volatile("s_waitcnt vmcnt(0)" ::: "memory");
+          __syncthreads();
+          auto feed = [&]() {
+            if (grp < NGRP - 1)
+              issue_b(cc, grp + 1, buf ^ 1);
+            else if (cc + 1 < nchunks)
+              issue_b(cc + 1, 0, buf ^ 1);
+            if (grp == NGRP - 2 && cc + 1 < nchunks) load_a(cc + 1);
+          };
+          wino_mma(j, ky, buf, aj, feed);
+        }
+      };
+      comp(0, wacc[0]);
+      comp(1, wacc[WINO ? 1 : 0]);
+      comp(2, wacc[WINO ? 2 : 0]);
+      comp(3, wacc[WINO ? 3 : 0]);
+    }
+  } else if constexpr (GL) {
     issue_b(0, 0, 0);
     for (int cc = 0; cc < nchunks; ++cc) {
       __syncthreads();
@@ -389,6 +493,91 @@
       bv.z = o4 + 2 < Nout ? bias[o4 + 2] : 0.f;
       bv.w = o4 + 3 < Nout ? bias[o4 + 3] : 0.f;
     }
+    if constexpr (WINO) {
+      const int xw = tx0 + 2 * (lr & 7);
+      if (relu & 2) {
+#pragma unroll
+        for (int tm = 0; tm < TMW; ++tm) {
+          const int y = ty0 + wm * TM + 2 * tm + (lr >> 3);
+          const f32x4v m0 = wacc[0][tn][tm], m1 = wacc[WINO ? 1 : 0][tn][tm], m2 = wacc[WINO ? 2 : 0][tn][tm],
+                       m3 = wacc[WINO ? 3 : 0][tn][tm];
+          const f32x4v y0 = m0 + (m1 + m2), y1 = (m1 - m2) - m3;
+          float v[4];
+#pragma unroll
+          for (int r = 0; r < 4; ++r) {
+            const float m = fmaxf(y0[r], y1[r]);
+            v[r] = fmaxf(m, __shfl_xor(m, 8, 64));
+          }
+          if ((lr >> 3) == 0 && y < H && xw < W && o4 < Nout) {
+            const int Hp = H >> 1, Wp = W >> 1;
+            float4 o = make_float4(v[0] + bv.x, v[1] + bv.y, v[2] + bv.z, v[3] + bv.w);
+            if (relu & 1) {
+              o.x = fmaxf(o.x, 0.f);
+              o.y = fmaxf(o.y, 0.f);
+              o.z = fmaxf(o.z, 0.f);
+              o.w = fmaxf(o.w, 0.f);
+            }
+            *reinterpret_cast<float4*>(dst + ((int64_t)img * Hp * Wp + (int64_t)(y >> 1) * Wp + (xw >> 1)) * Ns + o4) = o;
+          }
+        }
+        continue;
+      }
+      float4 mk[TMW][2];
+      if (mask != nullptr) {
+#pragma unroll
+        for (int tm = 0; tm < TMW; ++tm) {
+          const int y = ty0 + wm * TM + 2 * tm + (lr >> 3);
+#pragma unroll
+          for (int e = 0; e < 2; ++e) {
+            const bool ok = y < H && xw + e < W && o4 < Nout;
+            mk[tm][e] = ok ? *reinterpret_cast<const float4*>(mask + (rowbase + (int64_t)y * W + xw + e) * Ns + o4)
+                           : make_float4(0.f, 0.f, 0.f, 0.f);
+          }
+        }
+      }
+      double ds = 0.0, dq = 0.0;
+#pragma unroll
+      for (int tm = 0; tm < TMW; ++tm) {
+        const int y = ty0 + wm * TM + 2 * tm + (lr >> 3);
+        const f32x4v m0 = wacc[0][tn][tm], m1 = wacc[WINO ? 1 : 0][tn][tm], m2 = wacc[WINO ? 2 : 0][tn][tm],
+                     m3 = wacc[WINO ? 3 : 0][tn][tm];
+        const f32x4v yv[2] = {m0 + (m1 + m2), (m1 - m2) - m3};
+#pragma unroll
+        for (int e = 0; e < 2; ++e) {
+          if (y < H && xw + e < W && o4 < Nout) {
+            float4 o = make_float4(yv[e][0] + bv.x, yv[e][1] + bv.y, yv[e][2] + bv.z, yv[e][3] + bv.w);
+            if (relu & 1) {
+              o.x = fmaxf(o.x, 0.f);
+              o.y = fmaxf(o.y, 0.f);
+              o.z = fmaxf(o.z, 0.f);
+              o.w = fmaxf(o.w, 0.f);
+            }
+            if (mask != nullptr) {
+              o.x = (mk[tm][e].x > 0.f) ? o.x : 0.f;
+              o.y = (mk[tm][e].y > 0.f) ? o.y : 0.f;
+              o.z = (mk[tm][e].z > 0.f) ? o.z : 0.f;
+              o.w = (mk[tm][e].w > 0.f) ? o.w : 0.f;
+            }
+            *reinterpret_cast<float4*>(dst + (rowbase + (int64_t)y * W + xw + e) * Ns + o4) = o;
+            ds += (double)((o.x + o.y) + (o.z + o.w));
+            dq += (double)((o.x * o.x + o.y * o.y) + (o.z * o.z + o.w * o.w));
+          }
+        }
+      }
+      if (gn_ws != nullptr) {
+#pragma unroll
+        for (int sh = 1; sh <= 16; sh <<= 1) {
+          ds += __shfl_xor(ds, sh, 64);
+          dq += __shfl_xor(dq, sh, 64);
+        }
+        if (lr == 0 && (kg & 1) == 0) {
+          double* r = gn_red + (wm * (BN / 8) + ((o4 - n0) >> 3)) * 2;
+          r[0] = ds;
+          r[1] = dq;
+        }
+      }
+      continue;
+    }
     if (relu & 2) {
       const int Hp = H >> 1, Wp = W >> 1;
 #pragma unroll
@@ -504,22 +693,23 @@
   double* gn_ws;
 };
 
-template <int NP, int BN, int TH, int NT, int KS, int TPB = 1, bool GL = false>
+template <int NP, int BN, int TH, int NT, int KS, int TPB = 1, bool GL = false, bool WINO = false>
 static void launch_v2(const ConvArgs& a) {
   constexpr int HALO = KS / 2;
   TileTab2 tt;
   make_tiles_v2(a.od, &tt, TH);
   const int tiles = tt.tile_off[a.od->n_levels];
   const int n_tiles = (a.Nout + BN - 1) / BN;
-  constexpr size_t sh = (size_t)(NP * (TH + 2 * HALO) * (V2_TW + 2 * HALO) * 32 + 2 * NP * TPB * BN * 32) * sizeof(__bf16);
+  constexpr int PWK = WINO ? 32 : V2_TW + 2 * HALO;
+  constexpr size_t sh = (size_t)(NP * (TH + 2 * HALO) * PWK * 32 + 2 * NP * TPB * BN * 32) * sizeof(__bf16);
   static_assert(sh <= 160 * 1024, "LDS: 160 KB per CU");
   static bool done = false;
   if (!done) {
-    hipFuncSetAttribute(reinterpret_cast<const void*>(conv_split_kernel<NP, BN, TH, NT, KS, TPB, GL>),
+    hipFuncSetAttribute(reinterpret_cast<const void*>(conv_split_kernel<NP, BN, TH, NT, KS, TPB, GL, WINO>),
                         hipFuncAttributeMaxDynamicSharedMemorySize, (int)sh);
     done = true;
   }
-  hipLaunchKernelGGL((conv_split_kernel<NP, BN, TH, NT, KS, TPB, GL>), dim3(tiles * n_tiles), dim3(NT), sh, a.st, a.x, *a.od,
+  hipLaunchKernelGGL((conv_split_kernel<NP, BN, TH, NT, KS, TPB, GL, WINO>), dim3(tiles * n_tiles), dim3(NT), sh, a.st, a.x, *a.od,
                      a.Cs, a.w[0], a.w[1], a.w[2], a.Csw, a.bias, a.mask, a.y, a.Nout, a.Ns, a.relu, tt, n_tiles, *a.sd,
                      a.map, a.gn_ws);
 }
@@ -618,6 +808,20 @@
   return 0;
 }
 
+int g_scan_conv_wino = 1;
+extern "C" int scan_conv3x3_bf16x6_wino(int32_t Nout, int32_t Csw) { return g_scan_conv_wino && Nout > 64 && Csw % 32 == 0 ? 1 : 0; }
+
+int conv3x3_wino_launch(const float* x, const scan_pyramid_t* d, int32_t Cs, const void* w0, const void* w1, const void* w2,
+                        int32_t Csw, const float* bias, const float* mask, float* y, int32_t Nout, int32_t Ns, int32_t relu,
+                        void* stream, double* gn_ws) {
+  SCAN_CHECK_ARG(Nout > 64 && Csw % 32 == 0, "conv3x3_wino_bf16x6: needs Nout > 64 and Csw %% 32 == 0 (Nout=%d Csw=%d)", Nout, Csw);
+  ConvArgs a{x, d, d, Cs, {reinterpret_cast<const __bf16*>(w0), reinterpret_cast<const __bf16*>(w1),
+                           reinterpret_cast<const __bf16*>(w2)}, Csw, bias, mask, y, Nout, Ns, relu, 0, as_stream(stream), gn_ws};
+  launch_v2<3, 128, 16, 512, 3, 1, true, true>(a);
+  SCAN_LAUNCH_CHECK("conv3x3_wino_bf16x6");
+  return 0;
+}
+
 static int conv1x1_instance3(const scan_pyramid_t* yd, int32_t Nout, int32_t Csw);
 int g_scan_conv1x1 = 3;
 static int conv1x1_instance3(const scan_pyramid_t* yd, int32_t Nout, int32_t Csw) {
diff --git a/scan_amd/csrc/conv_split.h b/scan_amd/csrc/conv_split.h
--- a/scan_amd/csrc/conv_split.h
+++ b/scan_amd/csrc/conv_split.h
@@ -36,6 +36,13 @@
   }
 }
 
+__device__ __forceinline__ float wino_g(int j, double g0, double g1, double g2) {
+  const double v = j == 0 ? g0 : j == 1 ? 0.5 * (g0 + g1 + g2) : j == 2 ? 0.5 * (g0 - g1 + g2) : g2;
+  float f = (float)v;
+  asm("" : "+v"(f));
+  return f;
+}
+
 __device__ __forceinline__ __amdgpu_buffer_rsrc_t uniform_rsrc_b(const void* base, int bytes) {
   const unsigned long long a = reinterpret_cast<unsigned long long>(base);
   const unsigned lo = __builtin_amdgcn_readfirstlane((unsigned)a), hi = __builtin_amdgcn_readfirstlane((unsigned)(a >> 32));
diff --git a/scan_amd/csrc/scan_ops_ext.cpp b/scan_amd/csrc/scan_ops_ext.cpp
--- a/scan_amd/csrc/scan_ops_ext.cpp
+++ b/scan_amd/csrc/scan_ops_ext.cpp
@@ -98,9 +98,9 @@
   const int64_t o = wp.size(0), t = wp.size(1), cs = wp.size(2);
   const int64_t rnd = t == 9 ? 32 : 8;
   Planes pl;
-  const int64_t rows = mode == 0 ? o : cs;
-  pl.csw = round_up(mode == 0 ? cs : std::max(o, cs_src), rnd);
-  for (auto& q : pl.p) q = at::empty({rows, t, pl.csw}, wp.options().dtype(at::kBFloat16));
+  const int64_t rows = (mode & 1) == 0 ? o : cs;
+  pl.csw = round_up((mode & 1) == 0 ? cs : std::max(o, cs_src), rnd);
+  for (auto& q : pl.p) q = at::empty({rows, mode >= 2 ? 12 : t, pl.csw}, wp.options().dtype(at::kBFloat16));
   check(scan_weight_split3(wp.data_ptr<float>(), (int32_t)o, (int32_t)t, (int32_t)cs, mode, pl.p[0].data_ptr(), pl.p[1].data_ptr(),
                            pl.p[2].data_ptr(), (int32_t)pl.csw, cur_stream(wp)),
         "scan_weight_split3");
@@ -143,6 +143,14 @@
     check(scan_conv_smallcin_bf16x6(xr.data_ptr<float>(), (int32_t)g.n, (int32_t)g.h, (int32_t)g.w, wp.data_ptr<float>(), opt_ptr(bias),
                                     y.data_ptr<float>(), (int32_t)g.cout, (int32_t)g.ns, 3, 1, relu ? 1 : 0, st),
           "scan_conv_smallcin_bf16x6");
+    return y;
+  }
+  if (g.k == 3 && scan_conv3x3_bf16x6_wino((int32_t)g.cout, (int32_t)round_up(g.cs, 32))) {
+    const Planes pl = split3(wp, 2, g.cs, owner);
+    check(scan_conv3x3_wino_bf16x6(xr.data_ptr<float>(), &xd, (int32_t)g.cs, pl.p[0].data_ptr(), pl.p[1].data_ptr(), pl.p[2].data_ptr(),
+                                   (int32_t)pl.csw, opt_ptr(bias), nullptr, y.data_ptr<float>(), (int32_t)g.cout, (int32_t)g.ns,
+                                   relu ? 1 : 0, gn_sums.defined() ? reinterpret_cast<float*>(gn_sums.data_ptr()) : nullptr, 1, st),
+          "scan_conv3x3_wino_bf16x6");
     return y;
   }
   const Planes pl = split3(wp, 0, g.cs, owner);
@@ -182,8 +190,14 @@
                               (int32_t)g.cs, 3, 2, nullptr, st),
             "scan_conv2d_dgrad");
     } else {
-      const Planes pl = split3(wp, 1, g.ns, owner);
-      if (g.k == 3)
+      const bool wino = g.k == 3 && scan_conv3x3_bf16x6_wino((int32_t)g.cs, (int32_t)round_up(std::max(g.cout, g.ns), 32));
+      const Planes pl = split3(wp, wino ? 3 : 1, g.ns, owner);
+      if (wino)
+        check(scan_conv3x3_wino_bf16x6(dyr.data_ptr<float>(), &yd, (int32_t)g.ns, pl.p[0].data_ptr(), pl.p[1].data_ptr(), pl.p[2].data_ptr(),
+                                       (int32_t)pl.csw, nullptr, nullptr, dx.data_ptr<float>(), (int32_t)g.cs, (int32_t)g.cs, 0, nullptr, 0,
+                                       st),
+              "scan_conv3x3_wino_bf16x6 (data gradient)");
+      else if (g.k == 3)
         check(scan_conv3x3_bf16x6(dyr.data_ptr<float>(), &yd, (int32_t)g.ns, pl.p[0].data_ptr(), pl.p[1].data_ptr(), pl.p[2].data_ptr(),
                                   (int32_t)pl.csw, nullptr, nullptr, dx.data_ptr<float>(), (int32_t)g.cs, (int32_t)g.cs, 0, st),
               "scan_conv3x3_bf16x6 (data gradient)");
diff --git a/scan_amd/ops.py b/scan_amd/ops.py
--- a/scan_amd/ops.py
+++ b/scan_amd/ops.py
@@ -306,31 +306,37 @@
         rows, csw, nout = O, rnd(cs_w), O
     else:
         rows, csw, nout = cs_w, rnd(max(O, cs_src)), cs_w
+    rem = nout % 128
+    split_rem = T == 9 and not gn_sums and not pool and nout > 128 and 0 < rem <= 64 and cs_src >= 512 and rows_out >= 100000
+    wino = npc == 3 and T == 9 and not split_rem and query("scan_conv3x3_bf16x6_wino", nout, csw) == 1
+    smode, TP = (mode + 2, 12) if wino else (mode, T)
     hit = None
     if cache_key is not None and SPLIT_EPOCH is not None:
-        key = (cache_key, mode, csw, npc)
+        key = (cache_key, smode, csw, npc)
         hit = _split_cache.get(key)
-        if hit is not None and (hit[0] != SPLIT_EPOCH or tuple(hit[1][0].shape) != (rows, T, csw)):
+        if hit is not None and (hit[0] != SPLIT_EPOCH or tuple(hit[1][0].shape) != (rows, TP, csw)):
             hit = None
     if hit is not None:
         planes = hit[1]
         torch.cuda.current_stream().wait_event(hit[2])
     else:
-        planes = tuple(torch.empty((rows, T, csw), dtype=torch.bfloat16, device=x.device) for _ in range(npc))
+        planes = tuple(torch.empty((rows, TP, csw), dtype=torch.bfloat16, device=x.device) for _ in range(npc))
         if npc == 3:
-            call("scan_weight_split3", _ptr(wp), O, T, cs_w, mode, _ptr(planes[0]), _ptr(planes[1]), _ptr(planes[2]), csw, st)
+            call("scan_weight_split3", _ptr(wp), O, T, cs_w, smode, _ptr(planes[0]), _ptr(planes[1]), _ptr(planes[2]), csw, st)
         else:
             call("scan_weight_split", _ptr(wp), O, T, cs_w, mode, _ptr(planes[0]), _ptr(planes[1]), csw, st)
         if cache_key is not None and SPLIT_EPOCH is not None:
             ev = torch.cuda.Event()
             ev.record(torch.cuda.current_stream())
-            _split_cache[(cache_key, mode, csw, npc)] = (SPLIT_EPOCH, planes, ev)
+            _split_cache[(cache_key, smode, csw, npc)] = (SPLIT_EPOCH, planes, ev)
             if _active_plan is not None and param is not None and wp.data_ptr() == cache_key == param.data_ptr():
-                _active_plan.add((cache_key, mode, csw, npc), param, O, T, cs_w, mode, rows, csw, planes)
+                _active_plan.add((cache_key, smode, csw, npc), param, O, T, cs_w, smode, rows, csw, planes)
     wptrs = [_ptr(t) for t in planes]
     y = out if out is not None else (x.new_zeros if ns != nout else x.new_empty)((rows_out, ns))
     if kernel_timer.enabled:
-        if T == 9:
+        if wino:
+            inst = 3128
+        elif T == 9:
             inst = query("scan_conv3x3_%s_instance" % sfx, (dst_shape or shape).ref(), nout)
         elif npc == 3:
             inst = query("scan_conv1x1_bf16x6_instance", (dst_shape or shape).ref(), nout, csw)
@@ -339,7 +345,14 @@
         ev = kernel_timer.begin("%s_bn%d" % (name, inst), flops)
     else:
         ev = None
-    if gn_sums:
+    if wino:
+        if gn_sums:
+            sums, cleared = _ws_f64(shape.n_levels * shape.n_images * 32 * 2, x.device)
+            _gn_sums.clear()
+            _gn_sums[y.data_ptr()] = sums
+        call("scan_conv3x3_wino_bf16x6", _ptr(x), shape.ref(), cs_src, *wptrs, csw, _ptr(bias), _ptr(mask), _ptr(y), nout, ns,
+             int(bool(relu)) | (2 if pool else 0), _ptr(sums) if gn_sums else None, 0 if not gn_sums or cleared else 1, st)
+    elif gn_sums:
         sums, cleared = _ws_f64(shape.n_levels * shape.n_images * 32 * 2, x.device)
         if npc == 3:
             call("scan_conv3x3_gn_bf16x6", _ptr(x), shape.ref(), cs_src, *wptrs, csw, _ptr(bias), _ptr(y), nout, ns,
@@ -357,8 +370,7 @@
              _ptr(y), (dst_shape or shape).ref(), nout, ns, int(bool(relu)), cmap, st)
     else:
         fn = "scan_conv3x3_" + sfx
-        rem = nout % 128
-        if nout > 128 and 0 < rem <= 64 and cs_src >= 512 and rows_out >= 100000:
+        if split_rem:
             main = nout - rem
 
             def off(t, nbytes):
```

Result: faster. 22.75 (median of 6 runs) (+6.6%).
